# infancy/ky

Hardware: AMD Instinct MI355X
Metric: Msamples/s (paths*spp) (higher is better)
Workload: dtype f32

## Files before the change

include/kyhip.h:

```cpp
#ifndef KYHIP_H
#define KYHIP_H

#ifndef __HIPCC_RTC__
#include <stddef.h>
#include <stdint.h>
#endif

#ifdef __cplusplus
extern "C" {
#endif

#define KYHIP_ABI_VERSION 4


typedef enum ky_shape_kind {
    KY_SHAPE_DISK      = 0,
    KY_SHAPE_TRIANGLE  = 1,
    KY_SHAPE_RECTANGLE = 2,
    KY_SHAPE_SPHERE    = 3
} ky_shape_kind;

typedef struct ky_shape {
    int32_t kind;
    float   p[4][3];
// ... 32 lines not shown
    float   position[3];
    float   direction[3];
    float   world_radius;
} ky_light;

typedef struct ky_surface {
    int32_t shape;
    int32_t material;
    int32_t area_light;
} ky_surface;

typedef struct ky_camera {
    float position[3];
    float front[3];
    float right[3];
    float up[3];
    float resolution[2];
} ky_camera;

typedef struct ky_scene {
    const ky_shape*    shapes;    int32_t shape_count;
    const ky_material* materials; int32_t material_count;
    const ky_light*    lights;    int32_t light_count;
    const ky_surface*  surfaces;  int32_t surface_count;
    int32_t            environment_light;
    ky_camera          camera;
} ky_scene;

#define KYHIP_MAX_SHAPES    256
#define KYHIP_MAX_SURFACES  256
#define KYHIP_MAX_MATERIALS 64
#define KYHIP_MAX_LIGHTS    16


typedef enum ky_integrator_kind {
    KY_INTEGRATOR_POSITION               = 0,
    KY_INTEGRATOR_NORMAL                 = 1,
    KY_INTEGRATOR_BASECOLOR              = 2,
    KY_INTEGRATOR_DIRECT_LIGHTING        = 6,
    KY_INTEGRATOR_SIMPLE_PATH_TRACING_RECURSION   = 8,
    KY_INTEGRATOR_PATH_TRACING_RECURSION          = 9,
    KY_INTEGRATOR_PATH_TRACING_RECURSION_DEFERED  = 10,
    KY_INTEGRATOR_PATH_TRACING_ITERATION = 11
} ky_integrator_kind;

typedef enum ky_direct_sample {
    KY_DIRECT_IDLE      = 0,
    KY_DIRECT_BSDF      = 4,
    KY_DIRECT_LIGHT     = 8,
    KY_DIRECT_BSDF_MIS  = 16,
    KY_DIRECT_LIGHT_MIS = 32,
    KY_DIRECT_BOTH_MIS  = 48
} ky_direct_sample;

typedef enum ky_sampler_kind {
    KY_SAMPLER_DEBUG  = 0,
    KY_SAMPLER_RANDOM = 1
} ky_sampler_kind;

typedef struct ky_render_params {
    int32_t  integrator;
    int32_t  max_path_depth;
    int32_t  direct_sample;
    int32_t  samples_per_pixel;
    int32_t  sampler;
    uint32_t seed;
    int32_t  width, height;
    int32_t  tile_w, tile_h;
    int32_t  tile_first, tile_step;
} ky_render_params;

typedef enum ky_status {
    KY_OK                = 0,
    KY_ERR_INVALID_VALUE = -1,
    KY_ERR_LIMIT         = -2,
    KY_ERR_DEVICE        = -3,
    KY_ERR_NO_DEVICE     = -4
} ky_status;

const char* kyhip_last_error(void);
int         kyhip_set_engine(int engine);
int         kyhip_set_specialisation(int on);
int         kyhip_set_boxes(int on);
int         kyhip_set_shadow_queue(int mode);
int         kyhip_set_jit(int mode);
const char* kyhip_jit_status(void);
int         kyhip_jit_failures(void);
int64_t     kyhip_jit_compile(const char* name_expression);
uint64_t    kyhip_kernel_source_hash(void);
int         kyhip_abi_version(void);
int         kyhip_device_count(void);

int64_t kyhip_shard_tile_count(const ky_render_params* params);
int64_t kyhip_shard_float_count(const ky_render_params* params);
int64_t kyhip_film_term_limit(const ky_render_params* params, int n_lights, int engine, int deferred, float* limit);

int kyhip_render(int device, const ky_scene* scene, const ky_render_params* params,
                 float* film_rgb, size_t film_row_stride_px);

size_t kyhip_workspace_bytes(const ky_render_params* params);
int kyhip_render_tiles_device(int device, const ky_scene* scene, const ky_render_params* params,
                              float* d_tiles, void* d_workspace, size_t workspace_bytes, void* stream);
int kyhip_film_add_tiles_device(int device, const ky_render_params* params, const float* d_tiles,
                                float* d_film_rgb, size_t film_row_stride_px, void* stream);
int kyhip_film_add_gathered_device(int device, const ky_render_params* params, int world, const float* d_gathered,
                                   size_t rank_stride_floats, float* d_film_rgb, size_t film_row_stride_px, void* stream);

void*       kyhip_film_alloc(size_t bytes);
void        kyhip_film_free(void* film);
const char* kyhip_multi_status(int root_device);
int kyhip_seam_threads(void);
int kyhip_render_multi(const int* devices, int n_devices, const ky_scene* scene, const ky_render_params* params,
                       float* film_rgb, size_t film_row_stride_px);

float kyhip_kernel_ms(int device);
const char* kyhip_last_kernel(int device);


int kyhip_kat_intersect(int device, const ky_shape* shape, const float* rays7, int n, float* out8);

int kyhip_kat_camera(int device, const ky_camera* camera, const float* p_film2, int n, float* out6);

int kyhip_kat_bsdf(int device, const ky_material* material, const float* in12, int n, float* out13);

int kyhip_kat_light(int device, const ky_scene* scene, int light, const float* in11, int n, float* out11);

int kyhip_kat_scene_intersect(int device, const ky_scene* scene, const float* rays7, int n, float* out9);
int kyhip_kat_occluded(int device, const ky_scene* scene, const float* in9, int n, float* out1);
int kyhip_kat_any_pair(int device, const ky_scene* scene, const float* in13, int n, float* out2);
int kyhip_kat_occluded_between(int device, const ky_scene* scene, int light, const float* in9, int n, float* out1);
int kyhip_scene_non_occluders(const ky_scene* scene, int light, int* left_out, int n);
int kyhip_scene_boxes(const ky_scene* scene, int* box_face, int n);
int kyhip_scene_facts(const ky_scene* scene);

int kyhip_kat_li(int device, const ky_scene* scene, const ky_render_params* params,
                 int x, int y, int s0, int n, float* out3);

int kyhip_kat_nee(int device, const ky_scene* scene, int direct_sample, int light, const float* in15, int n, float* out6);

int kyhip_kat_li_trace(int device, const ky_scene* scene, const ky_render_params* params, int x, int y, int s,
                       float* rows26, int max_rows, float* li3);

enum ky_smallpt_refl { KY_SP_DIFF = 0, KY_SP_SPEC = 1, KY_SP_REFR = 2 };

typedef struct ky_smallpt_sphere {
    double rad;
    double p[3], e[3], c[3];
    int refl;
    int pad_;
} ky_smallpt_sphere;

enum ky_smallpt_variant { KY_SP_VARIANT_SMALLPT = 0, KY_SP_VARIANT_REWRITE = 1 };

typedef struct ky_smallpt_params {
    int width, height;
    int samps;
    uint32_t seed;
    int max_depth;
    int variant;
} ky_smallpt_params;

int kyhip_smallpt_scene(ky_smallpt_sphere* out);
int kyhip_smallpt_scene_rewrite(ky_smallpt_sphere* out);

int kyhip_smallpt_render(int device, const ky_smallpt_sphere* spheres, int n_spheres, const ky_smallpt_params* params,
                         double* image_rgb);

int kyhip_smallpt_kat_radiance(int device, const ky_smallpt_sphere* spheres, int n_spheres, const ky_smallpt_params* params,
                               int x, int y, int sx, int sy, int s0, int n, double* out3);

#ifdef __cplusplus
}
#endif
#endif
```

ky_amd/_abi.py:

```python
import ctypes as C
import os

_HERE = os.path.dirname(os.path.abspath(__file__))
LIB_DIR = os.path.join(_HERE, "lib")
REPO_ROOT = os.path.dirname(_HERE)

SHAPE_DISK, SHAPE_TRIANGLE, SHAPE_RECTANGLE, SHAPE_SPHERE = 0, 1, 2, 3
MATERIAL_MATTE, MATERIAL_MIRROR, MATERIAL_GLASS, MATERIAL_PLASTIC = 0, 1, 2, 3
LIGHT_POINT, LIGHT_DIRECTION, LIGHT_AREA, LIGHT_ENVIRONMENT = 0, 1, 2, 3
INTEGRATOR_POSITION, INTEGRATOR_NORMAL, INTEGRATOR_BASECOLOR = 0, 1, 2
INTEGRATOR_DIRECT_LIGHTING, INTEGRATOR_PATH_TRACING_ITERATION = 6, 11
INTEGRATOR_SIMPLE_PATH_TRACING_RECURSION, INTEGRATOR_PATH_TRACING_RECURSION, INTEGRATOR_PATH_TRACING_RECURSION_DEFERED = 8, 9, 10
DIRECT_IDLE, DIRECT_BSDF, DIRECT_LIGHT, DIRECT_BSDF_MIS, DIRECT_LIGHT_MIS, DIRECT_BOTH_MIS = 0, 4, 8, 16, 32, 48
SAMPLER_DEBUG, SAMPLER_RANDOM = 0, 1
SP_VARIANT_SMALLPT, SP_VARIANT_REWRITE = 0, 1
KY_OK, KY_ERR_INVALID_VALUE, KY_ERR_LIMIT, KY_ERR_DEVICE, KY_ERR_NO_DEVICE = 0, -1, -2, -3, -4
MAX_SHAPES, MAX_SURFACES, MAX_MATERIALS, MAX_LIGHTS = 256, 256, 64, 16

CB_LIGHT_AREA, CB_LIGHT_DIRECTION, CB_LIGHT_POINT, CB_LIGHT_ENVIRONMENT = 1, 2, 4, 8
CB_LARGE_MIRROR, CB_LARGE_GLASS, CB_SMALL_MIRROR, CB_SMALL_GLASS = 16, 32, 64, 128
CB_BOTH_SMALL_SPHERES = CB_SMALL_MIRROR | CB_SMALL_GLASS
CB_DEFAULT_SCENE = CB_BOTH_SMALL_SPHERES | CB_LIGHT_AREA

f3 = C.c_float * 3


class Shape(C.Structure):
    _fields_ = [("kind", C.c_int32), ("p", (C.c_float * 3) * 4), ("normal", f3), ("radius", C.c_float)]


class Material(C.Structure):
    _fields_ = [("kind", C.c_int32), ("color0", f3), ("color1", f3), ("eta", C.c_float), ("exponent", C.c_float),
                ("diffuse_probability", C.c_float), ("specular_probability", C.c_float)]


class Light(C.Structure):
    _fields_ = [("kind", C.c_int32), ("shape", C.c_int32), ("color", f3), ("position", f3), ("direction", f3),
                ("world_radius", C.c_float)]


class Surface(C.Structure):
    _fields_ = [("shape", C.c_int32), ("material", C.c_int32), ("area_light", C.c_int32)]


class Camera(C.Structure):
    _fields_ = [("position", f3), ("front", f3), ("right", f3), ("up", f3), ("resolution", C.c_float * 2)]


class Scene(C.Structure):
    _fields_ = [("shapes", C.POINTER(Shape)), ("shape_count", C.c_int32),
                ("materials", C.POINTER(Material)), ("material_count", C.c_int32),
                ("lights", C.POINTER(Light)), ("light_count", C.c_int32),
                ("surfaces", C.POINTER(Surface)), ("surface_count", C.c_int32),
                ("environment_light", C.c_int32), ("camera", Camera)]


class RenderParams(C.Structure):
    _fields_ = [("integrator", C.c_int32), ("max_path_depth", C.c_int32), ("direct_sample", C.c_int32),
                ("samples_per_pixel", C.c_int32), ("sampler", C.c_int32), ("seed", C.c_uint32),
                ("width", C.c_int32), ("height", C.c_int32), ("tile_w", C.c_int32), ("tile_h", C.c_int32),
                ("tile_first", C.c_int32), ("tile_step", C.c_int32)]


FP = C.POINTER(C.c_float)
SP = C.POINTER(Scene)
PP = C.POINTER(RenderParams)

class SmallptSphere(C.Structure):
    _fields_ = [("rad", C.c_double), ("p", C.c_double * 3), ("e", C.c_double * 3), ("c", C.c_double * 3), ("refl", C.c_int), ("pad_", C.c_int)]


class SmallptParams(C.Structure):
    _fields_ = [("width", C.c_int), ("height", C.c_int), ("samps", C.c_int), ("seed", C.c_uint32), ("max_depth", C.c_int),
                ("variant", C.c_int)]


SP_DIFF, SP_SPEC, SP_REFR = 0, 1, 2
SSP = C.POINTER(SmallptSphere)
SPP = C.POINTER(SmallptParams)

KYHIP_SYMBOLS = {
    "kyhip_last_error": (C.c_char_p, []),
    "kyhip_set_engine": (C.c_int, [C.c_int]),
    "kyhip_set_specialisation": (C.c_int, [C.c_int]),
    "kyhip_set_boxes": (C.c_int, [C.c_int]),
    "kyhip_set_shadow_queue": (C.c_int, [C.c_int]),
    "kyhip_set_jit": (C.c_int, [C.c_int]),
    "kyhip_jit_status": (C.c_char_p, []),
    "kyhip_jit_failures": (C.c_int, []),
    "kyhip_multi_status": (C.c_char_p, [C.c_int]),
    "kyhip_film_alloc": (C.c_void_p, [C.c_size_t]),
    "kyhip_film_free": (None, [C.c_void_p]),
    "kyhip_seam_threads": (C.c_int, []),
    "kyhip_jit_compile": (C.c_int64, [C.c_char_p]),
    "kyhip_kernel_source_hash": (C.c_uint64, []),
    "kyhip_abi_version": (C.c_int, []),
    "kyhip_device_count": (C.c_int, []),
    "kyhip_shard_tile_count": (C.c_int64, [PP]),
    "kyhip_shard_float_count": (C.c_int64, [PP]),
    "kyhip_film_term_limit": (C.c_int64, [PP, C.c_int, C.c_int, C.c_int, C.POINTER(C.c_float)]),
    "kyhip_render": (C.c_int, [C.c_int, SP, PP, C.c_void_p, C.c_size_t]),
    "kyhip_workspace_bytes": (C.c_size_t, [PP]),
    "kyhip_render_tiles_device": (C.c_int, [C.c_int, SP, PP, C.c_void_p, C.c_void_p, C.c_size_t, C.c_void_p]),
    "kyhip_film_add_tiles_device": (C.c_int, [C.c_int, PP, C.c_void_p, C.c_void_p, C.c_size_t, C.c_void_p]),
    "kyhip_film_add_gathered_device": (C.c_int, [C.c_int, PP, C.c_int, C.c_void_p, C.c_size_t, C.c_void_p, C.c_size_t, C.c_void_p]),
    "kyhip_render_multi": (C.c_int, [C.POINTER(C.c_int), C.c_int, SP, PP, C.c_void_p, C.c_size_t]),
    "kyhip_kernel_ms": (C.c_float, [C.c_int]),
    "kyhip_last_kernel": (C.c_char_p, [C.c_int]),
    "kyhip_kat_nee": (C.c_int, [C.c_int, SP, C.c_int, C.c_int, C.c_void_p, C.c_int, C.c_void_p]),
    "kyhip_kat_li_trace": (C.c_int, [C.c_int, SP, PP, C.c_int, C.c_int, C.c_int, C.c_void_p, C.c_int, C.c_void_p]),
    "kyhip_smallpt_scene": (C.c_int, [SSP]),
    "kyhip_smallpt_scene_rewrite": (C.c_int, [SSP]),
    "kyhip_smallpt_render": (C.c_int, [C.c_int, SSP, C.c_int, SPP, C.c_void_p]),
    "kyhip_smallpt_kat_radiance": (C.c_int, [C.c_int, SSP, C.c_int, SPP, C.c_int, C.c_int, C.c_int, C.c_int, C.c_int, C.c_int, C.c_void_p]),
    "kyhip_kat_intersect": (C.c_int, [C.c_int, C.POINTER(Shape), C.c_void_p, C.c_int, C.c_void_p]),
    "kyhip_kat_camera": (C.c_int, [C.c_int, C.POINTER(Camera), C.c_void_p, C.c_int, C.c_void_p]),
    "kyhip_kat_bsdf": (C.c_int, [C.c_int, C.POINTER(Material), C.c_void_p, C.c_int, C.c_void_p]),
    "kyhip_kat_light": (C.c_int, [C.c_int, SP, C.c_int, C.c_void_p, C.c_int, C.c_void_p]),
    "kyhip_kat_scene_intersect": (C.c_int, [C.c_int, SP, C.c_void_p, C.c_int, C.c_void_p]),
    "kyhip_kat_occluded": (C.c_int, [C.c_int, SP, C.c_void_p, C.c_int, C.c_void_p]),
    "kyhip_kat_any_pair": (C.c_int, [C.c_int, SP, C.c_void_p, C.c_int, C.c_void_p]),
    "kyhip_kat_occluded_between": (C.c_int, [C.c_int, SP, C.c_int, C.c_void_p, C.c_int, C.c_void_p]),
    "kyhip_scene_non_occluders": (C.c_int, [SP, C.c_int, C.c_void_p, C.c_int]),
    "kyhip_scene_boxes": (C.c_int, [SP, C.c_void_p, C.c_int]),
    "kyhip_scene_facts": (C.c_int, [SP]),
    "kyhip_kat_li": (C.c_int, [C.c_int, SP, PP, C.c_int, C.c_int, C.c_int, C.c_int, C.c_void_p]),
}

KYHOST_SYMBOLS = {
    "kyhost_last_error": (C.c_char_p, []),
    "kyhost_scene_create_cornell_box": (C.c_void_p, [C.c_int, C.c_float, C.c_float]),
    "kyhost_scene_create_mis": (C.c_void_p, [C.c_float, C.c_float]),
    "kyhost_scene_destroy": (None, [C.c_void_p]),
    "kyhost_scene_flatten": (SP, [C.c_void_p]),
    "kyhost_render": (C.c_int, [C.c_void_p, C.c_int, C.c_int, C.c_int, C.c_int, C.c_int, C.c_uint, C.c_int, C.c_int,
                                C.c_int, C.c_int, C.c_int, C.c_void_p, C.c_int]),
    "kyhost_debug_area": (C.c_int, [C.c_void_p, C.c_int, C.c_int, C.c_int, C.c_int, C.c_int, C.c_uint, C.c_int, C.c_int,
                                    C.c_void_p, C.c_int, C.c_int, C.c_int, C.c_int, C.c_int]),
    "kyhost_store_image": (C.c_int, [C.c_char_p, C.c_int, C.c_int, C.c_int, C.c_void_p]),
    "kyhost_gamma_encoding": (C.c_int, [C.c_float]),
}


SANITIZE = os.environ.get("KY_SANITIZE")
SAN_DIR = os.path.join(REPO_ROOT, "build", "san")

KYHOSTCHECK_SYMBOLS = {
    "kyhostcheck_pack": (C.c_int, [SP, C.POINTER(C.c_int), C.POINTER(C.c_uint64), C.POINTER(C.c_uint64), C.POINTER(C.c_int), C.POINTER(C.c_int)]),
    "kyhostcheck_chunks": (C.c_int, [C.c_int]),
    "kyhostcheck_shard": (C.c_longlong, [PP]),
    "kyhostcheck_add_rows": (C.c_int, [C.c_int, C.c_int, C.c_int, C.c_int, C.c_int]),
    "kyhostcheck_seam_stress": (C.c_int, [C.c_int]),
    "kyhostcheck_jit_stress": (C.c_int, [C.c_int, C.c_int]),
}


def _bind(lib, table, partial=False):
    for name, (res, args) in table.items():
        try:
            fn = getattr(lib, name)
        except AttributeError:
            if partial:
                continue
            raise
        fn.restype = res
        fn.argtypes = args
    return lib


_kyhip = None
_kyhost = None
_hiprt = None


def load_hip_runtime():
    global _hiprt
    if _hiprt is not None:
        return _hiprt
    candidates = []
    if os.environ.get("KYHIP_HIP_RUNTIME"):
        candidates.append(os.environ["KYHIP_HIP_RUNTIME"])
    else:
        try:
            import torch
            candidates.append(os.path.join(os.path.dirname(torch.__file__), "lib", "libamdhip64.so"))
        except Exception:
            pass
        candidates += ["/opt/rocm/lib/libamdhip64.so", "libamdhip64.so"]
    err = None
    for path in candidates:
        if os.path.isabs(path) and not os.path.exists(path):
            continue
        try:
            _hiprt = C.CDLL(path, mode=C.RTLD_GLOBAL)
            return _hiprt
        except OSError as e:
            err = e
    raise ImportError(f"no HIP runtime (libamdhip64.so) could be loaded: {err}")


def load_kyhip():
    global _kyhip
    if _kyhip is None and SANITIZE:
        path = os.path.join(SAN_DIR, "libkyhip_host_%s.so" % SANITIZE)
        if not os.path.exists(path):
            raise ImportError(f"{path} is missing: `make sanitize-build`")
        _kyhip = _bind(_bind(C.CDLL(path, mode=C.RTLD_GLOBAL), KYHIP_SYMBOLS, partial=True), KYHOSTCHECK_SYMBOLS)
    if _kyhip is None:
# ... 19 lines not shown
```

ky_amd/api.py:

```python
import ctypes as C

import numpy as np

from . import _abi as A


class KyError(RuntimeError):
    pass


def _check(rc, lib=None):
    if rc != A.KY_OK:
        lib = lib or A.load_kyhip()
        raise KyError(f"kyhip error {rc}: {lib.kyhip_last_error().decode()}")


def _fptr(a):
    assert a.dtype == np.float32 and a.flags["C_CONTIGUOUS"]
    return a.ctypes.data_as(C.c_void_p)


class SceneHandle:

    def __init__(self, ptr):
# ... 111 lines not shown

def kernel_ms(device=0):
    return float(A.load_kyhip().kyhip_kernel_ms(device))



def kat_intersect(shape, rays7, device=0):
    lib = A.load_kyhip()
    rays7 = np.ascontiguousarray(rays7, np.float32)
    out = np.zeros((rays7.shape[0], 8), np.float32)
    _check(lib.kyhip_kat_intersect(device, C.byref(shape), _fptr(rays7), rays7.shape[0], _fptr(out)))
    return out


def kat_camera(camera, p_film2, device=0):
    lib = A.load_kyhip()
    p_film2 = np.ascontiguousarray(p_film2, np.float32)
    out = np.zeros((p_film2.shape[0], 6), np.float32)
    _check(lib.kyhip_kat_camera(device, C.byref(camera), _fptr(p_film2), p_film2.shape[0], _fptr(out)))
    return out


def kat_bsdf(material, in12, device=0):
    lib = A.load_kyhip()
    in12 = np.ascontiguousarray(in12, np.float32)
    out = np.zeros((in12.shape[0], 13), np.float32)
    _check(lib.kyhip_kat_bsdf(device, C.byref(material), _fptr(in12), in12.shape[0], _fptr(out)))
    return out


def kat_light(scene, light, in11, device=0):
    lib = A.load_kyhip()
    in11 = np.ascontiguousarray(in11, np.float32)
    out = np.zeros((in11.shape[0], 11), np.float32)
    _check(lib.kyhip_kat_light(device, _scene_ptr(scene), light, _fptr(in11), in11.shape[0], _fptr(out)))
    return out


def kat_scene_intersect(scene, rays7, device=0):
    lib = A.load_kyhip()
    rays7 = np.ascontiguousarray(rays7, np.float32)
    out = np.zeros((rays7.shape[0], 9), np.float32)
    _check(lib.kyhip_kat_scene_intersect(device, _scene_ptr(scene), _fptr(rays7), rays7.shape[0], _fptr(out)))
    return out


def kat_any_pair(scene, in13, device=0):
    lib = A.load_kyhip()
    in13 = np.ascontiguousarray(in13, np.float32)
    out = np.zeros((in13.shape[0], 2), np.float32)
    _check(lib.kyhip_kat_any_pair(device, _scene_ptr(scene), _fptr(in13), in13.shape[0], _fptr(out)))
    return out


def kat_occluded(scene, in9, device=0, table=None):
    lib = A.load_kyhip()
    in9 = np.ascontiguousarray(in9, np.float32)
    out = np.zeros((in9.shape[0],), np.float32)
    if table is None:
        _check(lib.kyhip_kat_occluded(device, _scene_ptr(scene), _fptr(in9), in9.shape[0], _fptr(out)))
    else:
        _check(lib.kyhip_kat_occluded_between(device, _scene_ptr(scene), int(table), _fptr(in9), in9.shape[0], _fptr(out)))
    return out


def scene_non_occluders(scene, light=-1):
    lib = A.load_kyhip()
    n = _scene_ptr(scene).contents.surface_count
    out = np.zeros(max(1, n), np.int32)
    rc = lib.kyhip_scene_non_occluders(_scene_ptr(scene), int(light), out.ctypes.data_as(C.c_void_p), n)
    if rc < 0:
        _check(rc)
    return out[:n].copy()


def scene_facts(scene):
    lib = A.load_kyhip()
    rc = lib.kyhip_scene_facts(_scene_ptr(scene))
    if rc < 0:
        _check(rc)
    return rc


def scene_boxes(scene):
    lib = A.load_kyhip()
    n = _scene_ptr(scene).contents.surface_count
    out = np.zeros(max(1, n), np.int32)
    rc = lib.kyhip_scene_boxes(_scene_ptr(scene), out.ctypes.data_as(C.c_void_p), n)
    if rc < 0:
        _check(rc)
    return rc, out[:n].copy()


def kat_li(scene, params, x, y, s0, n, device=0):
    lib = A.load_kyhip()
    out = np.zeros((n, 3), np.float32)
    _check(lib.kyhip_kat_li(device, _scene_ptr(scene), C.byref(params), x, y, s0, n, _fptr(out)))
    return out


def kat_nee(scene, direct_sample, light, in15, device=0):
    lib = A.load_kyhip()
    in15 = np.ascontiguousarray(in15, np.float32)
    out = np.zeros((in15.shape[0], 6), np.float32)
    _check(lib.kyhip_kat_nee(device, _scene_ptr(scene), direct_sample, light, _fptr(in15), in15.shape[0], _fptr(out)))
    return out


def kat_li_trace(scene, params, x, y, s, max_rows=64, device=0):
    lib = A.load_kyhip()
    rows = np.zeros((max_rows, 26), np.float32)
    li = np.zeros(3, np.float32)
    n = lib.kyhip_kat_li_trace(device, _scene_ptr(scene), C.byref(params), x, y, s, _fptr(rows), max_rows, _fptr(li))
    if n < 0:
        _check(n, lib)
    return rows[:n], li



def smallpt_scene():
    spheres = (A.SmallptSphere * 9)()
    n = A.load_kyhip().kyhip_smallpt_scene(spheres)
    assert n == 9
    return spheres


def smallpt_scene_rewrite():
    spheres = (A.SmallptSphere * 9)()
    n = A.load_kyhip().kyhip_smallpt_scene_rewrite(spheres)
    assert n == 9
    return spheres


def smallpt_params(width, height, samps, seed=1234, max_depth=10, variant=A.SP_VARIANT_SMALLPT):
    return A.SmallptParams(width, height, samps, seed, max_depth, variant)


def smallpt_render(spheres, params, device=0):
    lib = A.load_kyhip()
    img = np.zeros((params.height, params.width, 3), np.float64)
    _check(lib.kyhip_smallpt_render(device, spheres, len(spheres), C.byref(params), img.ctypes.data_as(C.c_void_p)), lib)
    return img


def smallpt_kat_radiance(spheres, params, x, y, sx, sy, s0, n, device=0):
    lib = A.load_kyhip()
    out = np.zeros((n, 3), np.float64)
    _check(lib.kyhip_smallpt_kat_radiance(device, spheres, len(spheres), C.byref(params), x, y, sx, sy, s0, n,
                                          out.ctypes.data_as(C.c_void_p)), lib)
    return out


def store_image(filename, rgb, kind="bmp"):
    host = A.load_kyhost()
    rgb = np.ascontiguousarray(rgb, np.float32)
    k = {"ppm": 0, "bmp": 1, "hdr": 2}[kind]
    if host.kyhost_store_image(filename.encode(), k, rgb.shape[1], rgb.shape[0], _fptr(rgb)) != 0:
        raise KyError("store_image failed: " + host.kyhost_last_error().decode())
```

ky_amd/csrc/ky_device.hpp:

```cpp
#pragma once
#ifndef __HIPCC_RTC__
#include <hip/hip_runtime.h>
#include <stdint.h>
#endif

#include "ky_scene.hpp"

#define KY_DEV __device__ __forceinline__

#if defined(KY_PROFILE_LANES) || defined(KY_PROFILE_CLOCKS) || defined(KY_MARKS)
#include "ky_measure.hpp"
#else
#define KY_PROBE(k) do { } while (0)
#define KY_CLK(k) do { } while (0)
#endif

namespace kyd {

KY_DEV float rcp(float x) { return __builtin_amdgcn_rcpf(x); }
KY_DEV float rsq(float x) { return __builtin_amdgcn_rsqf(x); }
KY_DEV float fsqrt(float x) { return __builtin_amdgcn_sqrtf(x); }
KY_DEV float sin_rev(float x) { return __builtin_amdgcn_sinf(x); }
KY_DEV float cos_rev(float x) { return __builtin_amdgcn_cosf(x); }
KY_DEV float clamp01f(float x) { return __builtin_amdgcn_fmed3f(x, 0.f, 1.f); }
KY_DEV float any_f() { float x; asm volatile("" : "=v"(x)); return x; }
KY_DEV float any_reg() { return any_f(); }
KY_DEV unsigned any_reg_u() { unsigned x; asm volatile("" : "=v"(x)); return x; }
KY_DEV float mul_legacy(float a, float b) { float r; asm("s_nop 0\n\tv_mul_legacy_f32_e64 %0, %1, %2" : "=v"(r) : "v"(a), "v"(b)); return r; }
KY_DEV float pow_nonneg(float x, float n) {
    return __builtin_amdgcn_exp2f(mul_legacy(n, __builtin_amdgcn_logf(x)));
}

struct f3 {
    float x, y, z;
};
KY_DEV f3 mk3(float x, float y, float z) { return f3{x, y, z}; }
KY_DEV f3 any3() { return f3{any_f(), any_f(), any_f()}; }
KY_DEV f3 operator+(f3 a, f3 b) { return {a.x + b.x, a.y + b.y, a.z + b.z}; }
KY_DEV f3 operator-(f3 a, f3 b) { return {a.x - b.x, a.y - b.y, a.z - b.z}; }
KY_DEV f3 operator-(f3 a) { return {-a.x, -a.y, -a.z}; }
KY_DEV f3 operator*(f3 a, float s) { return {a.x * s, a.y * s, a.z * s}; }
KY_DEV f3 operator*(float s, f3 a) { return {a.x * s, a.y * s, a.z * s}; }
KY_DEV f3 operator*(f3 a, f3 b) { return {a.x * b.x, a.y * b.y, a.z * b.z}; }
KY_DEV float dot(f3 a, f3 b) { return a.x * b.x + a.y * b.y + a.z * b.z; }
KY_DEV f3 cross(f3 a, f3 b) { return {a.y * b.z - a.z * b.y, a.z * b.x - a.x * b.z, a.x * b.y - a.y * b.x}; }
KY_DEV float length_sq(f3 a) { return dot(a, a); }
KY_DEV f3 normalize(f3 a) { return a * rsq(dot(a, a)); }
KY_DEV float max3(f3 a) { return fmaxf(a.x, fmaxf(a.y, a.z)); }
KY_DEV bool is_black(f3 c) { return (c.x <= 0) && (c.y <= 0) && (c.z <= 0); }
KY_DEV bool is_black_bits(const float* c) {
    const int* b = (const int*)c;
    return (b[0] <= 0) & (b[1] <= 0) & (b[2] <= 0);
}

KY_DEV unsigned long long fixed_from_float(float a) {
    const float aa = fabsf(a);
    const float hi = __builtin_floorf(aa);
    const float lo = __builtin_rintf((aa - hi) * 4294967296.0f);
    const unsigned long long v = ((unsigned long long)(unsigned)hi << 32) | (unsigned long long)(unsigned)lo;
    return a < 0 ? 0ull - v : v;
}
KY_DEV float film_limit(const unsigned* counter) {
    return __uint_as_float(__hip_atomic_load(counter + 1, __ATOMIC_RELAXED, __HIP_MEMORY_SCOPE_AGENT));
}
KY_DEV float film_limit_for(const float* c, const unsigned* counter) {
    float limit = 1.f;
    if (!(fminf(fminf(c[0], c[1]), c[2]) >= 0.f && c[0] + c[1] + c[2] < 1.f)) limit = film_limit(counter);
    return limit;
}
KY_DEV unsigned long long film_fixed(float a, float limit, int ch, unsigned& flags) {
    const bool nan = a != a, pos = a >= limit, neg = a <= -limit;
    flags |= (nan ? 1u << ch : 0u) | (pos ? 8u << ch : 0u) | (neg ? 64u << ch : 0u);
    const float b = (nan | pos | neg) ? 0.f : a;
    return fixed_from_float(b);
}

constexpr float K_PI = 3.14159265358979323846f;
constexpr float K_INV_PI = 0.318309886183790671538f;
constexpr float K_INV_2PI = K_INV_PI / 2.f;
constexpr float K_SHAPE_EPS = 1e-3f;
constexpr float K_RAY_OFFSET = 1e-2f;
constexpr float K_INF = __builtin_huge_valf();

struct SceneRef {
    const DScene* p;
    bool general;
    int feat;
    bool large;
    __device__ __forceinline__ SceneRef(const DScene* p_) : p(p_), general(true), feat(0), large(true) {}
    __device__ __forceinline__ SceneRef(const DScene* p_, bool general_, int feat_ = 0, bool large_ = false) : p(p_), general(general_), feat(feat_), large(large_) {}
    __device__ __forceinline__ const DScene* operator->() const { return p; }
    __device__ __forceinline__ bool single_area() const { return (feat & KY_FEAT_SINGLE_AREA) != 0; }
    __device__ __forceinline__ bool single_light() const { return (feat & KY_FEAT_SINGLE_LIGHT) != 0; }
    __device__ __forceinline__ bool is_area(int kind) const {
        return (feat & (KY_FEAT_SINGLE_AREA | KY_FEAT_SPHERE_LIGHTS)) ? true : ((feat & (KY_FEAT_SINGLE_DELTA | KY_FEAT_SINGLE_ENV)) ? false : kind == KY_LIGHT_AREA);
    }
    __device__ __forceinline__ bool is_delta(int kind) const {
        return (feat & KY_FEAT_SINGLE_DELTA) ? true : ((feat & (KY_FEAT_SINGLE_AREA | KY_FEAT_SINGLE_ENV | KY_FEAT_SPHERE_LIGHTS)) ? false : (kind == KY_LIGHT_POINT || kind == KY_LIGHT_DIRECTION));
    }
    __device__ __forceinline__ bool is_env(int kind) const {
        return (feat & KY_FEAT_SINGLE_ENV) ? true : ((feat & (KY_FEAT_SINGLE_AREA | KY_FEAT_SINGLE_DELTA | KY_FEAT_SPHERE_LIGHTS)) ? false : kind == KY_LIGHT_ENVIRONMENT);
    }
    __device__ __forceinline__ bool may_have_env() const { return (feat & (KY_FEAT_SINGLE_AREA | KY_FEAT_SINGLE_DELTA | KY_FEAT_SPHERE_LIGHTS)) == 0; }
    __device__ __forceinline__ bool no_carried_light() const { return (feat & (KY_FEAT_SINGLE_DELTA | KY_FEAT_SINGLE_ENV)) != 0; }
    __device__ __forceinline__ bool x_planks() const { return (feat & KY_FEAT_X_PLANKS) != 0; }
    __device__ __forceinline__ bool sphere_lights() const { return (feat & KY_FEAT_SPHERE_LIGHTS) != 0; }
    __device__ __forceinline__ bool boxes() const { return (feat & KY_FEAT_BOXES) != 0; }
    __device__ __forceinline__ bool flat_phong() const { return (feat & KY_FEAT_FLAT_PHONG) != 0; }
    __device__ __forceinline__ bool no_par() const { return (feat & KY_FEAT_AXIS_ALIGNED) != 0; }
    __device__ __forceinline__ bool ipdf() const { return (feat & KY_FEAT_SPHERE_LIGHTS) != 0; }
};

struct LdsScene {
    const DHit* hit;
    const DMat* mat;
    const float (*light_color)[4];
};
template <int NS, int NM>
struct LdsSceneStaticT {
    DHit hit[NS];
    DMat mat[NM];
    float light_color[KYHIP_MAX_LIGHTS][4];
};
using LdsSceneStatic = LdsSceneStaticT<KY_LDS_SURFACES, KY_LDS_MATERIALS>;
extern __shared__ __attribute__((aligned(16))) unsigned char g_lds_scene[];

KY_DEV f3 ld3(const float* p) { return {p[0], p[1], p[2]}; }

template <bool LARGE, bool SMALL = false>
KY_DEV LdsScene stage_scene(SceneRef S) {
    const int tid = threadIdx.x, nt = blockDim.x;
    const int ns = S->n_surfaces, nm = S->n_materials, nl = S->n_lights;
    uint32_t *dst_h, *dst_m;
    float* dst_l;
    if (LARGE) {
        dst_h = reinterpret_cast<uint32_t*>(g_lds_scene);
        dst_m = reinterpret_cast<uint32_t*>(g_lds_scene + lds_scene_mat_offset(ns));
        dst_l = reinterpret_cast<float*>(g_lds_scene + lds_scene_light_offset(ns, nm));
    } else {
        __shared__ LdsSceneStaticT<SMALL ? KY_LDS_SURFACES_SMALL : KY_LDS_SURFACES, SMALL ? KY_LDS_MATERIALS_SMALL : KY_LDS_MATERIALS> L;
        dst_h = reinterpret_cast<uint32_t*>(L.hit);
        dst_m = reinterpret_cast<uint32_t*>(L.mat);
        dst_l = &L.light_color[0][0];
    }
    const uint32_t* src_h = reinterpret_cast<const uint32_t*>(S->hit);
    for (int i = tid; i < ns * (int)(sizeof(DHit) / 4); i += nt) dst_h[i] = src_h[i];
    const uint32_t* src_m = reinterpret_cast<const uint32_t*>(S->mat);
    for (int i = tid; i < nm * (int)(sizeof(DMat) / 4); i += nt) dst_m[i] = src_m[i];
    for (int i = tid; i < nl; i += nt) {
        dst_l[4 * i + 0] = S->light[i].color[0];
        dst_l[4 * i + 1] = S->light[i].color[1];
        dst_l[4 * i + 2] = S->light[i].color[2];
        dst_l[4 * i + 3] = 0.f;
    }
    __syncthreads();
    return LdsScene{reinterpret_cast<const DHit*>(dst_h), reinterpret_cast<const DMat*>(dst_m), reinterpret_cast<const float (*)[4]>(dst_l)};
}

KY_DEV uint32_t mix32(uint32_t x) {
    x ^= x >> 16; x *= 0x21f0aaadu;
    x ^= x >> 15; x *= 0x735a2d97u;
    x ^= x >> 15;
    return x;
}
struct Sampler {
    uint32_t s0, s1;
};
KY_DEV uint32_t sampler_pixel_key(uint32_t seed, uint32_t pixel_index) { return mix32(pixel_index ^ mix32(seed)); }
KY_DEV void sampler_start(Sampler& s, uint32_t h, uint32_t sample_index) {
    s.s0 = mix32(h + sample_index * 0x9E3779B9u);
    s.s1 = (__builtin_amdgcn_alignbit(s.s0, s.s0, 16) ^ h) | 1u;
}
KY_DEV uint32_t rotl32(uint32_t x, int k) { return __builtin_amdgcn_alignbit(x, x, 32 - k); }
// ... 239 lines not shown
}

KY_DEV float vmin(float a, float b) { float r; asm("v_min_f32_e32 %0, %1, %2" : "=v"(r) : "v"(a), "v"(b)); return r; }
KY_DEV float vmax(float a, float b) { float r; asm("v_max_f32_e32 %0, %1, %2" : "=v"(r) : "v"(a), "v"(b)); return r; }
KY_DEV float vmin3(float a, float b, float c) { float r; asm("v_min3_f32 %0, %1, %2, %3" : "=v"(r) : "v"(a), "v"(b), "v"(c)); return r; }
KY_DEV float vmax3(float a, float b, float c) { float r; asm("v_max3_f32 %0, %1, %2, %3" : "=v"(r) : "v"(a), "v"(b), "v"(c)); return r; }
KY_DEV float face_tag(float t, float surface_bits) { return __uint_as_float((__float_as_uint(t) & ~15u) | __float_as_uint(surface_bits)); }
KY_DEV void box_candidate(unsigned long long ex, float t_enter, float t_leave, float t, float& tmax, int& best) {
    unsigned long long tmp;
    const unsigned surface = __float_as_uint(t) & 15u;
    asm volatile(
        "v_cmpx_le_f32_e64 %[tmp], %[te], %[tl]\n\t"
        "v_cmpx_lt_f32_e64 %[tmp], %[eps], %[t]\n\t"
        "v_cmpx_lt_f32_e64 %[tmp], %[t], %[tmax]\n\t"
        "v_cmpx_ne_u32_e64 %[tmp], %[none], %[s]\n\t"
        "v_mov_b32_e32 %[tmax], %[t]\n\t"
        "v_mov_b32_e32 %[best], %[s]\n\t"
        "s_mov_b64 exec, %[ex]"
        : [tmax] "+v"(tmax), [best] "+v"(best), [tmp] "=&s"(tmp)
        : [te] "v"(t_enter), [tl] "v"(t_leave), [t] "v"(t), [s] "v"(surface), [eps] "s"(K_SHAPE_EPS), [none] "n"(KY_BOX_NO_FACE), [ex] "s"(ex));
}
KY_DEV void box_update_nearest(unsigned long long ex, const float4 q0, const float4 q1, const float4 q2, f3 o, f3 inv_c, float& tmax, int& best) {
    const float xl = face_tag((q0.x - o.x) * inv_c.x, q0.w), xh = face_tag((q1.x - o.x) * inv_c.x, q1.w);
    const float yl = face_tag((q0.y - o.y) * inv_c.y, q2.x), yh = face_tag((q1.y - o.y) * inv_c.y, q2.y);
    const float zl = face_tag((q0.z - o.z) * inv_c.z, q2.z), zh = face_tag((q1.z - o.z) * inv_c.z, q2.w);
    const float t_enter = vmax3(vmin(xl, xh), vmin(yl, yh), vmin(zl, zh));
    const float t_leave = vmin3(vmax(xl, xh), vmax(yl, yh), vmax(zl, zh));
    box_candidate(ex, t_enter, t_leave, t_enter, tmax, best);
    box_candidate(ex, t_enter, t_leave, t_leave, tmax, best);
}

KY_DEV void box_candidate_any(unsigned long long ex, float t_enter, float t_leave, float t, float tmax, unsigned& occ) {
    unsigned long long tmp;
    const unsigned surface = __float_as_uint(t) & 15u;
    asm volatile(
        "v_cmpx_le_f32_e64 %[tmp], %[te], %[tl]\n\t"
        "v_cmpx_lt_f32_e64 %[tmp], %[eps], %[t]\n\t"
        "v_cmpx_lt_f32_e64 %[tmp], %[t], %[tmax]\n\t"
        "v_cmpx_ne_u32_e64 %[tmp], %[none], %[s]\n\t"
        "v_mov_b32_e32 %[occ], 1\n\t"
        "s_mov_b64 exec, %[ex]"
        : [occ] "+v"(occ), [tmp] "=&s"(tmp)
        : [te] "v"(t_enter), [tl] "v"(t_leave), [t] "v"(t), [tmax] "v"(tmax), [s] "v"(surface), [eps] "s"(K_SHAPE_EPS), [none] "n"(KY_BOX_NO_FACE), [ex] "s"(ex));
}
KY_DEV void box_update_any(unsigned long long ex, const float4 q0, const float4 q1, const float4 q2, f3 o, f3 inv_c, float tmax, unsigned& occ) {
    const float xl = face_tag((q0.x - o.x) * inv_c.x, q0.w), xh = face_tag((q1.x - o.x) * inv_c.x, q1.w);
    const float yl = face_tag((q0.y - o.y) * inv_c.y, q2.x), yh = face_tag((q1.y - o.y) * inv_c.y, q2.y);
    const float zl = face_tag((q0.z - o.z) * inv_c.z, q2.z), zh = face_tag((q1.z - o.z) * inv_c.z, q2.w);
    const float t_enter = vmax3(vmin(xl, xh), vmin(yl, yh), vmin(zl, zh));
    const float t_leave = vmin3(vmax(xl, xh), vmax(yl, yh), vmax(zl, zh));
    box_candidate_any(ex, t_enter, t_leave, t_enter, tmax, occ);
    box_candidate_any(ex, t_enter, t_leave, t_leave, tmax, occ);
}
KY_DEV void box_candidate_any_unbounded(unsigned long long ex, float t_enter, float t_leave, float t, unsigned& occ) {
    unsigned long long tmp;
    const unsigned surface = __float_as_uint(t) & 15u;
    asm volatile(
        "v_cmpx_le_f32_e64 %[tmp], %[te], %[tl]\n\t"
        "v_cmpx_lt_f32_e64 %[tmp], %[eps], %[t]\n\t"
        "v_cmpx_ne_u32_e64 %[tmp], %[none], %[s]\n\t"
        "v_mov_b32_e32 %[occ], 1\n\t"
        "s_mov_b64 exec, %[ex]"
        : [occ] "+v"(occ), [tmp] "=&s"(tmp)
        : [te] "v"(t_enter), [tl] "v"(t_leave), [t] "v"(t), [s] "v"(surface), [eps] "s"(K_SHAPE_EPS), [none] "n"(KY_BOX_NO_FACE), [ex] "s"(ex));
}
KY_DEV void box_update_any_unbounded(unsigned long long ex, const float4 q0, const float4 q1, const float4 q2, f3 o, f3 inv_c, unsigned& occ) {
    const float xl = face_tag((q0.x - o.x) * inv_c.x, q0.w), xh = face_tag((q1.x - o.x) * inv_c.x, q1.w);
    const float yl = face_tag((q0.y - o.y) * inv_c.y, q2.x), yh = face_tag((q1.y - o.y) * inv_c.y, q2.y);
    const float zl = face_tag((q0.z - o.z) * inv_c.z, q2.z), zh = face_tag((q1.z - o.z) * inv_c.z, q2.w);
    const float t_enter = vmax3(vmin(xl, xh), vmin(yl, yh), vmin(zl, zh));
    const float t_leave = vmin3(vmax(xl, xh), vmax(yl, yh), vmax(zl, zh));
    box_candidate_any_unbounded(ex, t_enter, t_leave, t_enter, occ);
    box_candidate_any_unbounded(ex, t_enter, t_leave, t_leave, occ);
}

KY_DEV bool surf_hit(const DSurf& S, const DShapeFull* __restrict__ full, f3 o, f3 d, float tmax, float& t_out, bool general = true, bool sphere_only = false, bool sparse = true) {
    if (sphere_only) return sph_hit(make_float4(S.f[0], S.f[1], S.f[2], S.f[3]), o, d, tmax, t_out, sparse);
    if (S.kind == TK_PARALLELOGRAM)
        return par_hit(make_float4(S.f[0], S.f[1], S.f[2], S.f[3]), make_float4(S.f[4], S.f[5], S.f[6], S.f[7]), make_float4(S.f[8], S.f[9], S.f[10], S.f[11]), o, d, tmax, t_out);
    if (!general || S.kind == TK_SPHERE) return sph_hit(make_float4(S.f[0], S.f[1], S.f[2], S.f[3]), o, d, tmax, t_out);
    return full_shape_hit(full[S.full], o, d, tmax, t_out);
}

KY_DEV int trace_nearest(SceneRef S, f3 o, f3 d, float& tmax) {
    int best = -1;
    const unsigned t_off = opaque_off((unsigned)__builtin_offsetof(DScene, trav));
    const int4 head = scene_at<int4>(S, t_off), axis = scene_at<int4>(S, t_off + 16u);
    const int n_aar = head.x, n_par = S.no_par() ? 0 : head.y, n_sph = S->n_sph, n_gen = S->n_gen;
    if (S.boxes()) {
        const unsigned b_off = opaque_off((unsigned)__builtin_offsetof(DScene, boxtrav));
        const int4 bhead = scene_at<int4>(S, b_off), baxis = scene_at<int4>(S, b_off + 16u);
        const f3 inv_d = mk3(rcp(d.x), rcp(d.y), rcp(d.z));
        const f3 inv_c = mk3(__builtin_amdgcn_fmed3f(inv_d.x, -1e30f, 1e30f), __builtin_amdgcn_fmed3f(inv_d.y, -1e30f, 1e30f), __builtin_amdgcn_fmed3f(inv_d.z, -1e30f, 1e30f));
        const unsigned long long ex = __builtin_amdgcn_ballot_w64(true);
        unsigned off = b_off + (unsigned)__builtin_offsetof(DBoxTrav, box);
        for (int k = 0; k < bhead.x; ++k) {
            asm volatile("" : "+s"(off));
            const DBox& B = scene_at<DBox>(S, off);
            box_update_nearest(ex, B.q0, B.q1, B.q2, o, inv_c, tmax, best);
            off += (unsigned)sizeof(DBox);
        }
        if (bhead.y > 0) {
            unsigned unused = 0;
            const int n0 = baxis.x, n1 = baxis.y, n2 = baxis.z;
            const unsigned aar_off = b_off + (unsigned)__builtin_offsetof(DBoxTrav, aar);
            aar_scan<0, true>(S, aar_off, 0, n0, o, d, inv_d, tmax, best, unused);
            aar_scan<1, true>(S, aar_off, n0, n1, o, d, inv_d, tmax, best, unused);
            aar_scan<2, true>(S, aar_off, n0 + n1, n2, o, d, inv_d, tmax, best, unused);
        }
    } else
    if (n_aar > 0) {
        const f3 inv_d = mk3(rcp(d.x), rcp(d.y), rcp(d.z));
        unsigned unused = 0;
        const int n0 = axis.x, n1 = axis.y, n2 = axis.z;
        const unsigned aar_off = t_off + (unsigned)__builtin_offsetof(DTrav, aar);
        aar_scan<0, true>(S, aar_off, 0, n0, o, d, inv_d, tmax, best, unused);
        aar_scan<1, true>(S, aar_off, n0, n1, o, d, inv_d, tmax, best, unused);
        aar_scan<2, true>(S, aar_off, n0 + n1, n2, o, d, inv_d, tmax, best, unused);
    }
    if (n_par > 0) {
        unsigned off = t_off + (unsigned)__builtin_offsetof(DTrav, par);
        const unsigned long long ex = __builtin_amdgcn_ballot_w64(true);
        for (int i = 0; i < n_par; ++i) {
            asm volatile("" : "+s"(off));
            const DPar& r = scene_at<DPar>(S, off);
            float t, u, v;
            par_coords(r.q0, r.q1, r.q2, o, d, t, u, v);
            hit_update_nearest(ex, u, 0.5f, v, 0.5f, t, tmax, best, n_aar + i);
            off += (unsigned)sizeof(DPar);
        }
    }
    if (n_sph > 0) {
        unsigned off = scene_off(S, &S->sph[0]);
        const unsigned long long ex = __builtin_amdgcn_ballot_w64(true);
        for (int i = 0; i < n_sph; ++i) {
            asm volatile("" : "+s"(off));
            const float4 c = scene_at<DSph>(S, off).c;
            const f3 oc = mk3(c.x, c.y, c.z) - o;
            const float neg_b = dot(oc, d);
            const float discr = neg_b * neg_b - dot(oc, oc) + c.w;
            if (!S.sphere_lights() || __any(discr >= 0.f)) sph_update_nearest(ex, neg_b, discr, tmax, best, n_aar + n_par + i);
            off += (unsigned)sizeof(DSph);
        }
    }
    for (int i = 0; S.general && i < n_gen; ++i) {
        float t;
        if (full_shape_hit(S->full[S->gen[i].full], o, d, tmax, t)) {
            tmax = t;
            best = n_aar + n_par + n_sph + i;
        }
    }
    return best;
}

KY_DEV bool trace_any_planar(SceneRef S, const DTrav& T, f3 o, f3 d, float tmax) {
    unsigned occ = 0;
    const unsigned t_off = opaque_off(scene_off(S, &T));
    const int4 head = scene_at<int4>(S, t_off), axis = scene_at<int4>(S, t_off + 16u);
    const int n_aar = head.x, n_par = S.no_par() ? 0 : head.y;
    if (n_aar > 0) {
        const f3 inv_d = mk3(rcp(d.x), rcp(d.y), rcp(d.z));
        int unused = -1;
        const int n0 = axis.x, n1 = axis.y, n2 = axis.z;
        const unsigned aar_off = t_off + (unsigned)__builtin_offsetof(DTrav, aar);
        aar_scan<0, false>(S, aar_off, 0, n0, o, d, inv_d, tmax, unused, occ);
        aar_scan<1, false>(S, aar_off, n0, n1, o, d, inv_d, tmax, unused, occ);
        aar_scan<2, false>(S, aar_off, n0 + n1, n2, o, d, inv_d, tmax, unused, occ);
    }
    if (n_par > 0) {
        unsigned off = t_off + (unsigned)__builtin_offsetof(DTrav, par);
        const unsigned long long ex = __builtin_amdgcn_ballot_w64(true);
        for (int i = 0; i < n_par; ++i) {
            asm volatile("" : "+s"(off));
            const DPar& r = scene_at<DPar>(S, off);
            float t, u, v;
            par_coords(r.q0, r.q1, r.q2, o, d, t, u, v, S.x_planks());
            hit_update_any(ex, u, 0.5f, v, 0.5f, t, tmax, occ);
            off += (unsigned)sizeof(DPar);
        }
    }
    return occ != 0;
}
KY_DEV bool trace_any_round(SceneRef S, bool occ, f3 o, f3 d, float tmax) {
    const int n_sph = S->n_sph, n_gen = S->n_gen;
    float t;
    if (n_sph > 0) {
        unsigned off = scene_off(S, &S->sph[0]);
        const unsigned long long ex = __builtin_amdgcn_ballot_w64(true);
        unsigned occ_v = 0;
        for (int i = 0; i < n_sph; ++i) {
            asm volatile("" : "+s"(off));
            const float4 c = scene_at<DSph>(S, off).c;
            const f3 oc = mk3(c.x, c.y, c.z) - o;
            const float neg_b = dot(oc, d);
            const float discr = neg_b * neg_b - dot(oc, oc) + c.w;
            const float e = neg_b - tmax;
            if (!S.sphere_lights() || __any((discr >= 0.f) & ((e < 0.f) | (e * e < discr)))) sph_update_any(ex, neg_b, discr, tmax, occ_v);
            off += (unsigned)sizeof(DSph);
        }
        occ = occ | (occ_v != 0);
    }
    for (int i = 0; S.general && i < n_gen; ++i) occ = occ || full_shape_hit(S->full[S->gen[i].full], o, d, tmax, t);
    return occ;
}
KY_DEV bool trace_any(SceneRef S, const DTrav& T, f3 o, f3 d, float tmax) {
    return trace_any_round(S, trace_any_planar(S, T, o, d, tmax), o, d, tmax);
}
struct AnyRay {
    f3 o, d;
    float tmax;
};
template <int AXIS>
KY_DEV void aar_scan_any_pair(SceneRef S, unsigned long long ex, unsigned aar_off, int first, int n, const AnyRay& A, f3 iA, unsigned& occA, const AnyRay& B, f3 iB, unsigned& occB) {
    if (n <= 0) return;
    unsigned off = aar_off + (unsigned)first * (unsigned)sizeof(DAar);
    const float oaA = AXIS == 0 ? A.o.x : (AXIS == 1 ? A.o.y : A.o.z), iaA = AXIS == 0 ? iA.x : (AXIS == 1 ? iA.y : iA.z);
    const float ouA = AXIS == 0 ? A.o.y : (AXIS == 1 ? A.o.z : A.o.x), duA = AXIS == 0 ? A.d.y : (AXIS == 1 ? A.d.z : A.d.x);
    const float ovA = AXIS == 0 ? A.o.z : (AXIS == 1 ? A.o.x : A.o.y), dvA = AXIS == 0 ? A.d.z : (AXIS == 1 ? A.d.x : A.d.y);
    const float oaB = AXIS == 0 ? B.o.x : (AXIS == 1 ? B.o.y : B.o.z), iaB = AXIS == 0 ? iB.x : (AXIS == 1 ? iB.y : iB.z);
    const float ouB = AXIS == 0 ? B.o.y : (AXIS == 1 ? B.o.z : B.o.x), duB = AXIS == 0 ? B.d.y : (AXIS == 1 ? B.d.z : B.d.x);
    const float ovB = AXIS == 0 ? B.o.z : (AXIS == 1 ? B.o.x : B.o.y), dvB = AXIS == 0 ? B.d.z : (AXIS == 1 ? B.d.x : B.d.y);
    for (int i = 0; i < n; ++i) {
        asm volatile("" : "+s"(off));
        const DAar& r = scene_at<DAar>(S, off);
        const float4 q0 = r.q0;
        const float rv = r.q1.x;
        const float tA = (q0.x - oaA) * iaA, tB = (q0.x - oaB) * iaB;
        const float uA = (ouA + tA * duA) - q0.y, uB = (ouB + tB * duB) - q0.y;
        const float vA = (ovA + tA * dvA) - q0.w, vB = (ovB + tB * dvB) - q0.w;
        hit_update_any_unbounded(ex, uA, q0.z, vA, rv, tA, occA);
        hit_update_any(ex, uB, q0.z, vB, rv, tB, B.tmax, occB);
        off += (unsigned)sizeof(DAar);
    }
}
KY_DEV void trace_any_pair(SceneRef S, const AnyRay& A, const AnyRay& B, bool& occ_a, bool& occ_b) {
    unsigned occA = 0, occB = 0;
    const f3 iA = mk3(__builtin_amdgcn_fmed3f(rcp(A.d.x), -1e30f, 1e30f), __builtin_amdgcn_fmed3f(rcp(A.d.y), -1e30f, 1e30f), __builtin_amdgcn_fmed3f(rcp(A.d.z), -1e30f, 1e30f));
    const f3 iB = mk3(__builtin_amdgcn_fmed3f(rcp(B.d.x), -1e30f, 1e30f), __builtin_amdgcn_fmed3f(rcp(B.d.y), -1e30f, 1e30f), __builtin_amdgcn_fmed3f(rcp(B.d.z), -1e30f, 1e30f));
    const unsigned long long ex = __builtin_amdgcn_ballot_w64(true);
    const unsigned t_off = opaque_off((unsigned)__builtin_offsetof(DScene, trav));
    if (S.boxes()) {
        const unsigned b_off = opaque_off((unsigned)__builtin_offsetof(DScene, boxtrav));
        const int4 bhead = scene_at<int4>(S, b_off), baxis = scene_at<int4>(S, b_off + 16u);
        unsigned off = b_off + (unsigned)__builtin_offsetof(DBoxTrav, box);
        for (int k = 0; k < bhead.x; ++k) {
            asm volatile("" : "+s"(off));
            const DBox& Bx = scene_at<DBox>(S, off);
            const float4 q0 = Bx.q0, q1 = Bx.q1, q2 = Bx.q2;
            box_update_any_unbounded(ex, q0, q1, q2, A.o, iA, occA);
            box_update_any(ex, q0, q1, q2, B.o, iB, B.tmax, occB);
            off += (unsigned)sizeof(DBox);
        }
        if (bhead.y > 0) {
            const unsigned aar_off = b_off + (unsigned)__builtin_offsetof(DBoxTrav, aar);
            aar_scan_any_pair<0>(S, ex, aar_off, 0, baxis.x, A, iA, occA, B, iB, occB);
            aar_scan_any_pair<1>(S, ex, aar_off, baxis.x, baxis.y, A, iA, occA, B, iB, occB);
            aar_scan_any_pair<2>(S, ex, aar_off, baxis.x + baxis.y, baxis.z, A, iA, occA, B, iB, occB);
        }
    } else {
        const int4 head = scene_at<int4>(S, t_off), axis = scene_at<int4>(S, t_off + 16u);
        if (head.x > 0) {
            const unsigned aar_off = t_off + (unsigned)__builtin_offsetof(DTrav, aar);
            aar_scan_any_pair<0>(S, ex, aar_off, 0, axis.x, A, iA, occA, B, iB, occB);
            aar_scan_any_pair<1>(S, ex, aar_off, axis.x, axis.y, A, iA, occA, B, iB, occB);
            aar_scan_any_pair<2>(S, ex, aar_off, axis.x + axis.y, axis.z, A, iA, occA, B, iB, occB);
        }
    }
    const int n_par = S.no_par() ? 0 : S->trav.n_par;
    if (n_par > 0) {
        unsigned off = t_off + (unsigned)__builtin_offsetof(DTrav, par);
        for (int i = 0; i < n_par; ++i) {
            asm volatile("" : "+s"(off));
            const DPar& r = scene_at<DPar>(S, off);
            float t, u, v;
            par_coords(r.q0, r.q1, r.q2, A.o, A.d, t, u, v, S.x_planks());
            hit_update_any_unbounded(ex, u, 0.5f, v, 0.5f, t, occA);
            par_coords(r.q0, r.q1, r.q2, B.o, B.d, t, u, v, S.x_planks());
            hit_update_any(ex, u, 0.5f, v, 0.5f, t, B.tmax, occB);
            off += (unsigned)sizeof(DPar);
        }
    }
    const int n_sph = S->n_sph, n_gen = S->n_gen;
    if (n_sph > 0) {
        unsigned off = scene_off(S, &S->sph[0]);
        for (int i = 0; i < n_sph; ++i) {
            asm volatile("" : "+s"(off));
            const float4 c = scene_at<DSph>(S, off).c;
            const f3 ocA = mk3(c.x, c.y, c.z) - A.o, ocB = mk3(c.x, c.y, c.z) - B.o;
            const float nbA = dot(ocA, A.d), nbB = dot(ocB, B.d);
            sph_update_any_unbounded(ex, nbA, nbA * nbA - dot(ocA, ocA) + c.w, occA);
            sph_update_any(ex, nbB, nbB * nbB - dot(ocB, ocB) + c.w, B.tmax, occB);
            off += (unsigned)sizeof(DSph);
        }
    }
    occ_a = occA != 0;
    occ_b = occB != 0;
    float t;
    for (int i = 0; S.general && i < n_gen; ++i) {
        occ_a = occ_a || full_shape_hit(S->full[S->gen[i].full], A.o, A.d, A.tmax, t);
        occ_b = occ_b || full_shape_hit(S->full[S->gen[i].full], B.o, B.d, B.tmax, t);
    }
}

KY_DEV f3 hit_normal(const DHit& H, f3 position, f3 d) {
    const f3 n = ld3(H.n);
    if (H.kind == KY_SHAPE_SPHERE) return normalize(position - n);
    if (H.kind == KY_SHAPE_RECTANGLE) {
        const unsigned flip = dot(n, d) <= 0 ? 0u : 0x80000000u;
        return mk3(__uint_as_float(__float_as_uint(n.x) ^ flip), __uint_as_float(__float_as_uint(n.y) ^ flip), __uint_as_float(__float_as_uint(n.z) ^ flip));
    }
    return n;
}

struct Frame {
    f3 s, t, n;
};
KY_DEV Frame make_frame(f3 n) {
    Frame f;
// ... 676 lines not shown
    const float c[3] = {r.c.x, r.c.y, r.c.z};
    const int pix = (int)(r.tag >> 6), owner = (int)((threadIdx.x & ~63u) | (r.tag & 63u));
    const bool local = q.c_pix[owner] == pix;
    unsigned fl = 0;
    const float limit = film_limit_for(c, q.counter);
#pragma unroll
    for (int ch = 0; ch < 3; ++ch) {
        const unsigned long long fx = film_fixed(c[ch], limit, ch, fl);
        if (fx != 0) {
            if (local) atomicAdd(&q.c_def[ch * 256 + owner], fx);
            else atomicAdd(&q.accum[(size_t)pix * 3 + ch], fx);
        }
    }
    if (fl) atomicOr(&q.flags[pix], fl);
}
KY_DEV void sq_push(SceneRef S, ShadowQueue& q, bool push, SqRay r) {
    const unsigned long long m = __ballot(push);
    if (!m) return;
    const int k = __popcll(m);
    const int rank = (int)__builtin_amdgcn_mbcnt_hi((unsigned)(m >> 32), __builtin_amdgcn_mbcnt_lo((unsigned)m, 0u));
    if (q.n + k < KY_SQ_FLUSH_AT) {
        if (push) sq_store(KY_SQ_SLOT(q, q.n + rank), r);
        q.n += k;
        return;
    }
    asm volatile("" ::: "memory");
    const unsigned long long idle = ~m;
    const int idx = (int)__builtin_amdgcn_mbcnt_hi((unsigned)(idle >> 32), __builtin_amdgcn_mbcnt_lo((unsigned)idle, 0u));
    const bool pop = !push && idx < q.n;
    if (pop) r = sq_load(KY_SQ_SLOT(q, q.n - 1 - idx));
    q.n -= min(q.n, 64 - k);
    if (KY_SQ_FLUSH_AT == 64 || push || pop) sq_trace(S, q, r);
}
KY_DEV void sq_push_bsdf_query(SceneRef S, ShadowQueue& q, bool push, f3 o, f3 d, float tmax, f3 c, unsigned tag) {
    sq_push(S, q, push, SqRay{o, d, c, tmax, tag});
}
KY_DEV void sq_drain(SceneRef S, ShadowQueue& q) {
    const int lane = (int)__lane_id();
    __builtin_amdgcn_fence(__ATOMIC_ACQ_REL, "wavefront");
    if (lane < q.n) sq_trace(S, q, sq_load(KY_SQ_SLOT(q, lane)));
    q.n = 0;
}

template <bool MIS>
KY_DEV void estimate_by_emitter_deferred(SceneRef S, const Vertex& v, f3 wo, int li, float u0, float u1, bool active, f3 beta, float weight,
                                         unsigned tag, ShadowQueue& q) {
    const DLight& L = scene_light(S, li);
    bool push = false;
    SqRay r{any3(), any3(), any3(), any_f(), tag};
    if (active) {
        const bool ip = S.ipdf();
        const LightSample ls = light_sample_Li(L, v.position, v.normal, u0, u1, S.feat, ip);
        if (S.is_area(L.kind)) {
            r.d = ls.dir;
            r.tmax = ls.dist - 2e-3f;
        } else {
            const f3 to = ls.position - v.position;
            const float d2 = length_sq(to);
            const float inv_d = rsq(d2);
            r.d = to * inv_d;
            r.tmax = d2 * inv_d - 2e-3f;
        }
        r.o = offset_ray_origin(v.position, v.normal, r.d);
        f3 col;
        float scale, bsdf_pdf, abs_cos_i;
        bsdf_eval_parts(v, wo, S.is_area(L.kind) ? r.d : ls.wi, col, scale, bsdf_pdf, abs_cos_i);
        const bool delta_light = S.is_delta(L.kind);
        const float fc = scale * abs_cos_i;
        const float k = fc * (ip ? ((!MIS || delta_light) ? ls.pdf : (2.f * ls.pdf) * rcp(1.f + bsdf_pdf * ls.pdf))
                                 : ((!MIS || delta_light) ? rcp(ls.pdf) : 2.f * rcp(ls.pdf + bsdf_pdf))) * weight;
        const bool area = S.is_area(L.kind);
        const f3 Li = area ? ld3(L.color) : ls.Li;
        r.c = ((col * Li) * beta) * k;
        push = (area ? ls.lit : !is_black(ls.Li)) && (ip || !(MIS ? ls.pdf <= 0 : ls.pdf == 0)) && !(fc <= 0.f) && !is_black(col);
        if (S.is_area(L.kind) && L.sampled_is_surface) {
            float t;
            if (surf_hit(L.isect, S->full, r.o, r.d, r.tmax, t, S.general, S.sphere_lights(), false)) push = false;
        }
    }
    sq_push(S, q, push, r);
}

KY_DEV bool light_sample_occluded(SceneRef S, int li, f3 o, f3 dir, float tmax) {
    const unsigned tab = (unsigned)scene_light(S, li).shadow_table;
    const bool two = (tab & 1u) != 0;
    bool occ = trace_any(S, scene_at<DTrav>(S, tab & ~1u), o, dir, tmax);
    if (two) {
        const float4 plane = scene_at<float4>(S, opaque_off((unsigned)__builtin_offsetof(DScene, ts_plane)));
        const f3 pn = mk3(plane.x, plane.y, plane.z);
        const f3 e = o + dir * tmax;
        const bool need = !occ && (fminf(dot(pn, e), dot(pn, o)) <= plane.w);
        if (__any(need)) {
            if (need) occ = trace_any_planar(S, S->occ_behind, o, dir, tmax);
        }
    }
    return occ;
}

template <bool MIS>
KY_DEV void estimate_by_emitter(SceneRef S, const LdsScene& Lds, const Vertex& v, f3 wo, int li, float u0, float u1, f3& acc, f3 w) {
    const DLight& L = scene_light(S, li);
    KY_PROBE(3);
    const bool ip = S.ipdf();
    const LightSample ls = light_sample_Li(L, v.position, v.normal, u0, u1, S.feat, ip);
    const bool area = S.is_area(L.kind);
    const bool dead = (area ? !ls.lit : is_black(ls.Li)) || (!(ip || area) && (MIS ? (ls.pdf <= 0) : (ls.pdf == 0)));
    KY_CLK(5);
    if (!dead) {
        f3 dir;
        float dist;
        if (area) {
            dir = ls.dir;
            dist = ls.dist;
        } else {
            const f3 to = ls.position - v.position;
            const float d2 = length_sq(to);
            const float inv_d = rsq(d2);
            dir = to * inv_d;
            dist = d2 * inv_d;
        }
        const f3 o = offset_ray_origin(v.position, v.normal, dir);
        KY_PROBE(4);
        const bool occ = light_sample_occluded(S, li, o, dir, dist - 2e-3f);
        KY_CLK(6);
        if (!occ) {
            KY_PROBE(5);
            f3 col;
            float scale, bsdf_pdf, abs_cos_i;
            bsdf_eval_parts(v, wo, area ? dir : ls.wi, col, scale, bsdf_pdf, abs_cos_i);
            const float fc = scale * abs_cos_i;
            if (!(fc <= 0.f) && !is_black(col)) {
                const bool delta_light = S.is_delta(L.kind);
                const float k = fc * (ip ? ((!MIS || delta_light) ? ls.pdf : (2.f * ls.pdf) * rcp(1.f + bsdf_pdf * ls.pdf))
                                         : ((!MIS || delta_light) ? rcp(ls.pdf) : 2.f * rcp(ls.pdf + bsdf_pdf)));
                acc = acc + ((col * (area ? ld3(L.color) : ls.Li)) * w) * k;
            }
            KY_CLK(7);
        }
    }
}

template <bool MIS>
KY_DEV void estimate_by_emitter_ride(SceneRef S, const LdsScene& Lds, const Vertex& v, f3 wo, int li, float u0, float u1, bool active, RideAlong& ra, f3& acc, f3 w) {
    const DLight& L = scene_light(S, li);
    LightSample ls{any3(), any3(), any3(), any_f(), false, any3(), any_f()};
    const bool area = S.is_area(L.kind);
    bool dead = true;
    if (active) {
        ls = light_sample_Li(L, v.position, v.normal, u0, u1, S.feat);
        dead = (area ? !ls.lit : is_black(ls.Li)) || (MIS ? (ls.pdf <= 0) : (ls.pdf == 0));
    }
    f3 o = any3(), dir = any3();
    float tmax = any_f();
    if (!dead) {
        if (area) {
            dir = ls.dir;
            tmax = ls.dist - 2e-3f;
        } else {
            const f3 to = ls.position - v.position;
            const float d2 = length_sq(to);
            const float inv_d = rsq(d2);
            dir = to * inv_d;
            tmax = d2 * inv_d - 2e-3f;
        }
        o = offset_ray_origin(v.position, v.normal, dir);
    }
// ... 332 lines not shown
```

ky_amd/csrc/ky_host.hpp:

```cpp
#pragma once
#include <cstddef>
#include <cstdint>
#include <condition_variable>
#include <functional>
#include <mutex>
#include <string>
#include <utility>
#include <vector>
#include <sys/types.h>

#include "ky_shard.hpp"

namespace kyh {
using namespace kyd;

int fail(int code, const char* fmt, ...) __attribute__((format(printf, 2, 3)));
const std::string& last_error();

bool valid_params(const ky_render_params* p);
bool shard_in_range(const ky_render_params* p);
ShardConst make_shard(const ky_render_params* p);
RenderConst make_rc(const ky_render_params* p);
long long film_term_count(const ky_render_params* p, int n_lights, bool queue_engine, bool deferred);
float film_term_limit(long long n_terms);
bool film_in_range(const ky_render_params* p, int n_lights);
int film_range_check(const ky_render_params* p, const ky_scene* scene);
inline size_t workspace_bytes_for(const ShardConst& s) { return (size_t)s.n_pix * (3 * sizeof(unsigned long long) + sizeof(unsigned)); }

void cp3(float* d, const float* s);
void pack_shape(const ky_shape& sh, int full_index, DSurf* surf, DShapeFull* full);
void pack_material(const ky_material& m, DMat* d);
bool shape_normal_ok(const ky_shape& sh);
struct NonOccluders {
    std::vector<char> wall;
    std::vector<char> light_ok;
    bool deferred_ok = false;
    int ts_light = -1;
    double ts_plane[4] = {0, 0, 0, 0};
    std::vector<char> ts_behind;
};
void find_non_occluders(const ky_scene* in, NonOccluders& R);
struct Boxes {
    struct Box { float lo[3], hi[3]; int face[6]; };
    std::vector<Box> box;
    std::vector<int> box_of;
};
void find_boxes(const ky_scene* in, Boxes& B);
int pack_scene(const ky_scene* in, DScene* out);
uint64_t scene_hash(const DScene& s);
bool scene_input(const ky_scene* in, std::vector<unsigned char>& out, uint64_t& hash);

constexpr int KY_SP_MAX_SPHERES = 32;
int smallpt_check(const ky_smallpt_sphere* spheres, int n, const ky_smallpt_params* p);

bool specialisation_enabled();
bool boxes_enabled();
int shadow_queue_mode();
bool shadow_queue_wanted(const ky_scene* scene);
int blocks_per_cu_cap();
enum { KY_ENGINE_LANE = 0, KY_ENGINE_QUEUE = 1 };
int current_engine();

int cpus_granted();
int seam_threads();
void host_add_rows(float* __restrict__ film, size_t stride_px, const float* __restrict__ src, int width, int y0, int y1);
class HostPool {
public:
    void run(int n, const std::function<void(int)>& fn);
private:
    void loop(int id);
    std::mutex job_m_, m_;
    std::condition_variable cv_, done_;
    const std::function<void(int)>* fn_ = nullptr;
    int n_ = 0, pending_ = 0, n_threads_ = 0;
    pid_t pid_ = 0;
    unsigned long long generation_ = 0;
};
HostPool& host_pool();
std::vector<std::unique_lock<std::mutex>> lock_seams(std::vector<std::pair<int, std::mutex*>> by_device);
}

namespace kyjit {
struct Code {
    std::vector<char> object;
    bool failed = false;
};
extern const char k_entry[];
int mode();
const Code* get_code(const std::string& args, bool wait = true, bool* pending = nullptr);
uint64_t source_hash();
int set_mode(int m);
bool mode_by_default();
std::string status();
int failures();
void frame_begin();
void frame_end();
}
```

ky_amd/csrc/ky_launch.hip:

```cpp
#include <hip/hip_runtime.h>

#include <algorithm>
#include <cstdio>
#include <cstring>

#include "ky_ctx.hpp"
#include "ky_render.hpp"
#include "ky_smallpt.hpp"

using namespace kyh;
static_assert(kyh::KY_SP_MAX_SPHERES == kysp::SP_MAX_SPHERES, "smallpt_check (ky_pack.cpp) and the kernels' LDS table");

#include "ky_queue.hpp"

__global__ void resolve_kernel(unsigned long long* __restrict__ accum, unsigned* __restrict__ flags, float* __restrict__ tiles, int n_pix, unsigned* __restrict__ counter) {
    const int i = blockIdx.x * blockDim.x + threadIdx.x;
    if (i == 0) *counter = 0u;
    if (i >= n_pix) return;
    const unsigned fl = flags[i];
    flags[i] = 0u;
#pragma unroll
    for (int ch = 0; ch < 3; ++ch) {
        float v = (float)((double)(long long)accum[3 * (size_t)i + ch] * (1.0 / KY_FIX_SCALE));
        accum[3 * (size_t)i + ch] = 0ull;
// ... 113 lines not shown
            if (sl.valid && sl.input_hash == input_hash && sl.input == input) pick = &sl;
    uint64_t hash = 0;
    if (!pick) {
        const int rc = pack_scene(scene, &scratch);
        if (rc != KY_OK) return rc;
        hash = scene_hash(scratch);
        for (SceneSlot& sl : c->scenes)
            if (sl.valid && sl.hash == hash && std::memcmp(&scratch, sl.h, sizeof(DScene)) == 0) pick = &sl;
        if (pick && keyed) { pick->input = input; pick->input_hash = input_hash; }
    }
    if (pick) {
        if (pick->upload_stream != stream) HIP_TRY(hipStreamWaitEvent(stream, pick->ready, 0));
    } else {
        for (SceneSlot& sl : c->scenes)
            if (!sl.valid && !pick) pick = &sl;
        if (!pick) {
            pick = &c->scenes[0];
            for (SceneSlot& sl : c->scenes)
                if (sl.last_use < pick->last_use) pick = &sl;
            for (int i = 0; i < KY_STREAM_STATES; ++i)
                if ((pick->readers >> i & 1u) && c->ss[i].done) HIP_TRY(hipEventSynchronize(c->ss[i].done));
            HIP_TRY(hipEventSynchronize(pick->ready));
            pick->valid = false;
        }
        if (!pick->d) {
            HIP_TRY(hipMalloc(&pick->d, sizeof(DScene)));
            HIP_TRY(hipHostMalloc(&pick->h, sizeof(DScene)));
            HIP_TRY(hipEventCreateWithFlags(&pick->ready, hipEventDisableTiming));
        }
        std::memcpy(pick->h, &scratch, sizeof(DScene));
        HIP_TRY(hipMemcpyAsync(pick->d, pick->h, sizeof(DScene), hipMemcpyHostToDevice, stream));
        HIP_TRY(hipEventRecord(pick->ready, stream));
        pick->upload_stream = stream;
        pick->hash = hash;
        if (keyed) { pick->input = input; pick->input_hash = input_hash; } else { pick->input.clear(); pick->input_hash = 0; }
        pick->readers = 0;
        pick->valid = true;
    }
    pick->last_use = ++c->clock;
    *out = pick;
    return KY_OK;
}
}

extern "C" {

#ifdef KY_PROFILE_LANES
int kyhip_debug_lane_probe(unsigned long long* out32) {
    unsigned long long zero[32] = {0};
    if (hipMemcpyFromSymbol(out32, HIP_SYMBOL(g_lane_probe), sizeof zero) != hipSuccess) return KY_ERR_DEVICE;
    if (hipMemcpyToSymbol(HIP_SYMBOL(g_lane_probe), zero, sizeof zero) != hipSuccess) return KY_ERR_DEVICE;
    return KY_OK;
}
#endif
#ifdef KY_PROFILE_CLOCKS
int kyhip_debug_clocks(unsigned long long* out16, int reset) {
    if (hipMemcpyFromSymbol(out16, HIP_SYMBOL(g_clk), 16 * sizeof(unsigned long long)) != hipSuccess) return -1;
    if (reset) { unsigned long long z[16] = {}; if (hipMemcpyToSymbol(HIP_SYMBOL(g_clk), z, sizeof(z)) != hipSuccess) return -1; }
    return 0;
}
#endif
#ifdef KY_QE_STATS
int kyhip_debug_stats(unsigned long long* out32, int reset) {
    if (hipMemcpyFromSymbol(out32, HIP_SYMBOL(kyd::g_qe_stats), 32 * sizeof(unsigned long long)) != hipSuccess) return -1;
    if (reset) { unsigned long long z[32] = {}; if (hipMemcpyToSymbol(HIP_SYMBOL(kyd::g_qe_stats), z, sizeof(z)) != hipSuccess) return -1; }
    return 0;
}
#endif

int kyhip_device_count(void) {
    int n = 0;
    if (hipGetDeviceCount(&n) != hipSuccess) return 0;
    return n;
}

using RenderFn = void (*)(const DScene*, RenderConst, ShardConst, unsigned*, unsigned long long*, unsigned*, float4*);
struct Variant {
    bool dbg;
    int strategy;
    bool queue, general;
    int feat, integrator;
    bool large;
    RenderFn fn;
};
#define KY_VARIANT(D, S, Q, G, F, I) Variant{D, S, Q, G, F, I, false, render_kernel<D, S, Q, G, F, I>}
#define KY_VARIANT_LARGE(D, S, Q, G, F, I) Variant{D, S, Q, G, F, I, true, render_kernel<D, S, Q, G, F, I, true>}
constexpr int IT = KY_INTEGRATOR_PATH_TRACING_ITERATION;
static const Variant g_variants[] = {
#ifdef KY_FEW_VARIANTS
    KY_VARIANT(false, KY_DIRECT_BOTH_MIS, false, false, KY_FEAT_CORNELL | KY_FEAT_SMALL_TABLES | KY_FEAT_BOXES | KY_FEAT_AXIS_ALIGNED | KY_FEAT_FLAT_PHONG, IT),
    KY_VARIANT(false, KY_DIRECT_BOTH_MIS, false, false, KY_FEAT_CORNELL | KY_FEAT_SMALL_TABLES | KY_FEAT_BOXES, IT),
    KY_VARIANT(false, KY_DIRECT_BOTH_MIS, false, false, KY_FEAT_CORNELL | KY_FEAT_SMALL_TABLES, IT),
#ifndef KY_NO_XPLANK_ROW
    KY_VARIANT(false, KY_DIRECT_BOTH_MIS, true, false, KY_FEAT_VEACH | KY_FEAT_FLAT_PHONG | KY_FEAT_X_PLANKS, IT),
#endif
    KY_VARIANT(false, KY_DIRECT_BOTH_MIS, true, false, KY_FEAT_VEACH | KY_FEAT_FLAT_PHONG, IT),
    KY_VARIANT(false, KY_DIRECT_BOTH_MIS, false, false, KY_FEAT_SINGLE_ENV | KY_FEAT_SMALL_TABLES | KY_FEAT_BOXES | KY_FEAT_AXIS_ALIGNED | KY_FEAT_FLAT_PHONG, IT),
    KY_VARIANT(false, KY_DIRECT_BOTH_MIS, false, false, KY_FEAT_SINGLE_ENV | KY_FEAT_SMALL_TABLES | KY_FEAT_AXIS_ALIGNED | KY_FEAT_FLAT_PHONG, IT),
    KY_VARIANT(false, KY_DIRECT_BOTH_MIS, false, false, KY_FEAT_SINGLE_ENV, IT),
    KY_VARIANT(false, -1, false, false, 0, IT),
#else
    KY_VARIANT(false, KY_DIRECT_BOTH_MIS, false, false, KY_FEAT_CORNELL | KY_FEAT_SMALL_TABLES | KY_FEAT_BOXES | KY_FEAT_AXIS_ALIGNED | KY_FEAT_FLAT_PHONG, IT),
    KY_VARIANT(false, KY_DIRECT_BOTH_MIS, false, false, KY_FEAT_CORNELL | KY_FEAT_SMALL_TABLES | KY_FEAT_BOXES, IT),
    KY_VARIANT(false, KY_DIRECT_BOTH_MIS, false, false, KY_FEAT_CORNELL | KY_FEAT_SMALL_TABLES | KY_FEAT_AXIS_ALIGNED, IT),
    KY_VARIANT(false, KY_DIRECT_BOTH_MIS, false, false, KY_FEAT_CORNELL | KY_FEAT_SMALL_TABLES, IT),
    KY_VARIANT(false, KY_DIRECT_BOTH_MIS, false, false, KY_FEAT_CORNELL, IT),
    KY_VARIANT(false, KY_DIRECT_BOTH_MIS, false, false, KY_FEAT_SINGLE_DELTA | KY_FEAT_BOXES | KY_FEAT_AXIS_ALIGNED | KY_FEAT_FLAT_PHONG, IT),
    KY_VARIANT(false, KY_DIRECT_BOTH_MIS, false, false, KY_FEAT_SINGLE_DELTA, IT),
    KY_VARIANT(false, KY_DIRECT_BOTH_MIS, false, false, KY_FEAT_SINGLE_ENV | KY_FEAT_SMALL_TABLES | KY_FEAT_BOXES | KY_FEAT_AXIS_ALIGNED | KY_FEAT_FLAT_PHONG, IT),
    KY_VARIANT(false, KY_DIRECT_BOTH_MIS, false, false, KY_FEAT_SINGLE_ENV | KY_FEAT_SMALL_TABLES | KY_FEAT_AXIS_ALIGNED | KY_FEAT_FLAT_PHONG, IT),
    KY_VARIANT(false, KY_DIRECT_BOTH_MIS, false, false, KY_FEAT_SINGLE_ENV, IT),
    KY_VARIANT(false, KY_DIRECT_BOTH_MIS, true, false, KY_FEAT_VEACH | KY_FEAT_FLAT_PHONG | KY_FEAT_X_PLANKS, IT),
    KY_VARIANT(false, KY_DIRECT_BOTH_MIS, true, false, KY_FEAT_VEACH | KY_FEAT_FLAT_PHONG, IT),
    KY_VARIANT(false, KY_DIRECT_BOTH_MIS, true, false, KY_FEAT_VEACH, IT),
    KY_VARIANT(false, KY_DIRECT_BOTH_MIS, true, false, 0, IT),
    KY_VARIANT(false, KY_DIRECT_BOTH_MIS, false, false, 0, IT),
    KY_VARIANT(false, KY_DIRECT_BSDF, false, false, KY_FEAT_VEACH, IT),
    KY_VARIANT(false, KY_DIRECT_LIGHT, true, false, KY_FEAT_VEACH, IT),
    KY_VARIANT(false, KY_DIRECT_LIGHT, false, false, KY_FEAT_VEACH, IT),
    KY_VARIANT(false, KY_DIRECT_BSDF_MIS, false, false, KY_FEAT_VEACH, IT),
    KY_VARIANT(false, KY_DIRECT_LIGHT_MIS, true, false, KY_FEAT_VEACH, IT),
    KY_VARIANT(false, KY_DIRECT_LIGHT_MIS, false, false, KY_FEAT_VEACH, IT),
    KY_VARIANT(false, KY_DIRECT_BSDF, false, false, KY_FEAT_CORNELL, IT),
    KY_VARIANT(false, KY_DIRECT_BSDF_MIS, false, false, KY_FEAT_CORNELL, IT),
    KY_VARIANT(false, KY_DIRECT_IDLE, false, false, 0, IT),
    KY_VARIANT(false, KY_DIRECT_BSDF, false, false, 0, IT),
    KY_VARIANT(false, KY_DIRECT_LIGHT, true, false, 0, IT),
    KY_VARIANT(false, KY_DIRECT_LIGHT_MIS, true, false, 0, IT),
    KY_VARIANT(false, KY_DIRECT_LIGHT, false, false, 0, IT),
    KY_VARIANT(false, KY_DIRECT_BSDF_MIS, false, false, 0, IT),
    KY_VARIANT(false, KY_DIRECT_LIGHT_MIS, false, false, 0, IT),
    KY_VARIANT(false, KY_DIRECT_BOTH_MIS, false, false, KY_FEAT_CORNELL, KY_INTEGRATOR_PATH_TRACING_RECURSION),
    KY_VARIANT(false, KY_DIRECT_BOTH_MIS, false, false, KY_FEAT_SINGLE_ENV, KY_INTEGRATOR_PATH_TRACING_RECURSION),
    KY_VARIANT(false, KY_DIRECT_BOTH_MIS, false, false, KY_FEAT_CORNELL, KY_INTEGRATOR_PATH_TRACING_RECURSION_DEFERED),
    KY_VARIANT(false, KY_DIRECT_BOTH_MIS, false, false, KY_FEAT_SINGLE_ENV, KY_INTEGRATOR_PATH_TRACING_RECURSION_DEFERED),
    KY_VARIANT(false, KY_DIRECT_BOTH_MIS, false, false, KY_FEAT_SINGLE_DELTA, KY_INTEGRATOR_PATH_TRACING_RECURSION),
    KY_VARIANT(false, KY_DIRECT_BOTH_MIS, false, false, KY_FEAT_SINGLE_DELTA, KY_INTEGRATOR_PATH_TRACING_RECURSION_DEFERED),
    KY_VARIANT(false, KY_DIRECT_BOTH_MIS, false, false, KY_FEAT_CORNELL, KY_INTEGRATOR_DIRECT_LIGHTING),
    KY_VARIANT(false, KY_DIRECT_BOTH_MIS, false, false, KY_FEAT_SINGLE_DELTA, KY_INTEGRATOR_DIRECT_LIGHTING),
    KY_VARIANT(false, KY_DIRECT_BOTH_MIS, false, false, KY_FEAT_SINGLE_ENV, KY_INTEGRATOR_DIRECT_LIGHTING),
    KY_VARIANT(false, KY_DIRECT_BOTH_MIS, false, false, 0, KY_INTEGRATOR_DIRECT_LIGHTING),
    KY_VARIANT(false, KY_DIRECT_BOTH_MIS, false, false, 0, KY_INTEGRATOR_SIMPLE_PATH_TRACING_RECURSION),
    KY_VARIANT(false, KY_DIRECT_BOTH_MIS, false, false, 0, KY_INTEGRATOR_PATH_TRACING_RECURSION),
    KY_VARIANT(false, KY_DIRECT_BOTH_MIS, false, false, 0, KY_INTEGRATOR_PATH_TRACING_RECURSION_DEFERED),
    KY_VARIANT(false, KY_DIRECT_BOTH_MIS, false, true, 0, IT),
    KY_VARIANT(false, -1, false, false, 0, IT),
    KY_VARIANT(true, -1, false, false, 0, IT),
    KY_VARIANT(false, -1, false, true, 0, IT),
    KY_VARIANT(true, -1, false, true, 0, IT),
    KY_VARIANT_LARGE(false, -1, false, true, 0, IT),
    KY_VARIANT_LARGE(true, -1, false, true, 0, IT),
#endif
};
constexpr int KY_N_VARIANTS = (int)(sizeof g_variants / sizeof g_variants[0]);
static_assert(KY_N_VARIANTS <= 64, "DeviceCtx::variant_blocks");

static const Variant* pick_variant(const ky_render_params* p, const DScene* packed, bool deferred_rays, int n_pix) {
    const bool dbg = p->sampler == KY_SAMPLER_DEBUG;
    const bool general = packed->general != 0;
    const bool large = packed->n_surfaces > KY_LDS_SURFACES || packed->n_materials > KY_LDS_MATERIALS;
    for (const Variant& v : g_variants) {
        if (v.dbg != dbg || v.large != large) continue;
        if (general && !v.general) continue;
        if (v.strategy >= 0) {
            if (!specialisation_enabled() && !(v.strategy == KY_DIRECT_BOTH_MIS && v.feat == 0 && v.integrator == IT)) continue;
            if (v.strategy != p->direct_sample || v.integrator != p->integrator) continue;
        }
        if ((v.feat & packed->feat) != v.feat) continue;
        if (v.queue && !(n_pix < (1 << 26) && deferred_rays)) continue;
        return &v;
    }
    return nullptr;
}

}
static int set_film_limit(StreamState* st, long long n_terms, hipStream_t stream) {
    const float t = film_term_limit(n_terms);
    if (t == 0.f) return fail(KY_ERR_DEVICE, "internal: %lld film terms per pixel passed film_in_range", n_terms);
    uint32_t bits;
    std::memcpy(&bits, &t, sizeof bits);
    if (st->counter_limit_bits != bits) {
        HIP_TRY(hipMemsetD32Async((hipDeviceptr_t)(st->d_counter + 1), (int)bits, 1, stream));
        st->counter_limit_bits = bits;
    }
    return KY_OK;
}
int kyh::render_replay_feat(const ky_scene* scene, const ky_render_params* p, const DScene* packed) {
    const Variant* v = pick_variant(p, packed, shadow_queue_wanted(scene), p->width * p->height);
    return v != nullptr ? (v->feat & (KY_FEAT_BOXES | KY_FEAT_SINGLE_ENV)) : 0;
}
bool kyh::render_uses_boxes(const ky_scene* scene, const ky_render_params* p, const DScene* packed) { return (render_replay_feat(scene, p, packed) & KY_FEAT_BOXES) != 0; }
extern "C" {

int kyhip_render_tiles_device(int device, const ky_scene* scene, const ky_render_params* p, float* d_tiles, void* d_workspace,
                              size_t workspace_bytes, void* stream_) {
    if (!valid_params(p)) return fail(KY_ERR_INVALID_VALUE, "invalid render params (integrator %d, direct_sample %d)", p ? p->integrator : -1, p ? p->direct_sample : -1);
    if (!shard_in_range(p)) return fail(KY_ERR_LIMIT, "frame too large for the device's 32-bit work-item and pixel indices (%d x %d, %d spp)", p->width, p->height, p->samples_per_pixel);
    if (film_range_check(p, scene) != KY_OK) return KY_ERR_LIMIT;
    if (!d_tiles) return fail(KY_ERR_INVALID_VALUE, "d_tiles is NULL");
    DeviceCtx* c;
    int rcode = get_ctx(device, &c);
    if (rcode != KY_OK) return rcode;
    std::lock_guard<std::mutex> lock(c->m);
    hipStream_t stream = (hipStream_t)stream_;
    SceneSlot* sc;
    rcode = upload_scene(c, scene, stream, &sc);
    if (rcode != KY_OK) return rcode;

    const ShardConst sh = make_shard(p);
    if (sh.n_tiles == 0) return KY_OK;
    const RenderConst rc = make_rc(p);
    StreamState* st;
    rcode = get_stream_state(c, stream, &st);
    if (rcode != KY_OK) return rcode;

    const size_t need = workspace_bytes_for(sh);
    void* ws = d_workspace;
    if (!(d_workspace && workspace_bytes >= need)) {
        if (st->ws_bytes < need) {
            HIP_TRY(hipStreamSynchronize(stream));
            if (st->ws) HIP_TRY(hipFree(st->ws));
            st->ws = nullptr; st->ws_bytes = 0;
            HIP_TRY(hipMalloc(&st->ws, need));
            st->ws_bytes = need;
            st->ws_clean = false;
        }
        ws = st->ws;
    }
    unsigned long long* accum = (unsigned long long*)ws;
    unsigned* flags = (unsigned*)(accum + (size_t)sh.n_pix * 3);
    const bool large_scene = scene->surface_count > KY_LDS_SURFACES || scene->material_count > KY_LDS_MATERIALS;
    const size_t lds_bytes = large_scene ? (size_t)lds_scene_bytes(scene->surface_count, scene->material_count, scene->light_count) : 0;
    const bool own_ws = ws == st->ws;
    if (!(own_ws && st->ws_clean)) {
        HIP_TRY(hipMemsetAsync(ws, 0, own_ws ? st->ws_bytes : need, stream));
        HIP_TRY(hipMemsetAsync(st->d_counter, 0, sizeof(unsigned), stream));
    }
    st->ws_clean = false;

    if (current_engine() == KY_ENGINE_QUEUE && p->integrator == KY_INTEGRATOR_PATH_TRACING_ITERATION && !large_scene) {
        const int variant = p->sampler == KY_SAMPLER_DEBUG ? 2 : (p->direct_sample == KY_DIRECT_BOTH_MIS ? 0 : 1);
        const int per_cu = c->q_blocks_per_cu[variant] > 0 ? c->q_blocks_per_cu[variant] : 1;
        unsigned grid = (unsigned)(c->cus * per_cu);
        const unsigned need_blocks = (unsigned)(((unsigned long long)sh.n_items * 64u + QE_SLOTS - 1) / QE_SLOTS);
        if (grid > need_blocks) grid = need_blocks;
        if (grid < 1) grid = 1;
        rcode = set_film_limit(st, film_term_count(p, sc->h->n_lights, true, false), stream);
        if (rcode != KY_OK) return rcode;
        HIP_TRY(hipEventRecord(st->ev0, stream));
        if (variant == 0) hipLaunchKernelGGL((render_kernel_q<false, KY_DIRECT_BOTH_MIS>), dim3(grid), dim3(QE_THREADS), 0, stream, sc->d, rc, sh, st->d_counter, accum, flags);
        else if (variant == 1) hipLaunchKernelGGL((render_kernel_q<false, -1>), dim3(grid), dim3(QE_THREADS), 0, stream, sc->d, rc, sh, st->d_counter, accum, flags);
        else hipLaunchKernelGGL((render_kernel_q<true, -1>), dim3(grid), dim3(QE_THREADS), 0, stream, sc->d, rc, sh, st->d_counter, accum, flags);
        c->last_variant = -2;
    } else {
        const Variant* v = pick_variant(p, sc->h, shadow_queue_wanted(scene), sh.n_pix);
        if (!v) return fail(KY_ERR_DEVICE, "internal: no render kernel for these parameters");
        const int vi = (int)(v - g_variants);
        DeviceCtx::JitKernel* jk = nullptr;
        bool queue = v->queue;
        const int jit_mode = kyjit::mode();
        c->last_note.clear();
        if (v->strategy < 0 && jit_mode == 0) c->last_note = " [the run-time-dispatched kernel: no row of the table holds this launch's strategy / integrator / shapes; kyhip_set_jit(1 / 2) instantiates its own]";
        const bool jit_wanted = jit_mode != 0 && (!kyjit::mode_by_default() || v->feat == 0 || v->strategy < 0);
        if (jit_wanted && specialisation_enabled() && p->integrator >= KY_INTEGRATOR_DIRECT_LIGHTING) {
            const bool dbg = p->sampler == KY_SAMPLER_DEBUG, general = sc->h->general != 0;
            int feat = (dbg || general) ? 0 : sc->h->feat;
            const bool env_pair = (feat & KY_FEAT_SINGLE_ENV) && p->direct_sample == KY_DIRECT_BOTH_MIS && p->integrator != KY_INTEGRATOR_PATH_TRACING_RECURSION;
            if (!((feat & (KY_FEAT_SINGLE_AREA | KY_FEAT_SINGLE_DELTA)) || env_pair)) feat &= ~KY_FEAT_BOXES;
            const bool want_queue = (p->direct_sample == KY_DIRECT_BOTH_MIS || p->direct_sample == KY_DIRECT_LIGHT_MIS || p->direct_sample == KY_DIRECT_LIGHT) &&
                                    p->integrator == KY_INTEGRATOR_PATH_TRACING_ITERATION && sh.n_pix < (1 << 26) && !general && shadow_queue_wanted(scene);
            const bool same = v->dbg == dbg && v->strategy == p->direct_sample && v->queue == want_queue && v->general == general && v->feat == feat &&
                              v->integrator == p->integrator && v->large == large_scene;
            if (!same) {
                char expr[192];
                snprintf(expr, sizeof expr, "%s, %d, %s, %s, %d, %d, %s", dbg ? "true" : "false", p->direct_sample, want_queue ? "true" : "false",
                         general ? "true" : "false", feat, p->integrator, large_scene ? "true" : "false");
                DeviceCtx::JitKernel& k = c->jit[expr];
                if (!k.fn && !k.failed) {
                    bool pending = false;
                    const kyjit::Code* code = kyjit::get_code(expr, jit_mode == 1, &pending);
                    if (code) {
                        if (!(hipModuleLoadData(&k.module, code->object.data()) == hipSuccess && hipModuleGetFunction(&k.fn, k.module, kyjit::k_entry) == hipSuccess)) {
                            (void)hipGetLastError();
                            k.fn = nullptr;
                            k.failed = true;
                        }
                    } else if (!pending) {
                        k.failed = true;
                    }
                    if (pending) c->last_note = " [its own instantiation render_kernel<" + std::string(expr) + "> is being compiled (kyhip_set_jit mode 2): this frame ran on the table's kernel]";
                }
                if (k.failed) c->last_note = " [its own instantiation is unavailable: " + kyjit::status() + "]";
                if (k.fn) {
                    if (k.lds != lds_bytes) {
                        int per_cu = 0;
                        HIP_TRY(hipModuleOccupancyMaxActiveBlocksPerMultiprocessor(&per_cu, k.fn, 256, lds_bytes));
                        k.per_cu = per_cu > 0 ? per_cu : 1;
                        k.lds = lds_bytes;
                    }
                    jk = &k;
                    queue = want_queue;
                    char desc[224];
                    snprintf(desc, sizeof desc, "render_kernel<%sstrategy %d%s%s%s, feat %d, integrator %d> = render_kernel<", dbg ? "debug sampler, " : "", p->direct_sample,
                             want_queue ? ", deferred shadow rays" : "", general ? ", general shapes" : "", large_scene ? ", scene-sized LDS block" : "", feat, p->integrator);
                    c->last_jit = std::string(desc) + expr + ">";
                }
            }
        }
        if (!jk && (c->variant_blocks[vi] == 0 || c->variant_lds[vi] != lds_bytes)) {
            int per_cu = 0;
            HIP_TRY(hipOccupancyMaxActiveBlocksPerMultiprocessor(&per_cu, v->fn, 256, lds_bytes));
            c->variant_blocks[vi] = per_cu > 0 ? per_cu : 1;
            c->variant_lds[vi] = lds_bytes;
        }
        const int per_cu = jk ? jk->per_cu : c->variant_blocks[vi];
        unsigned grid = (unsigned)(c->cus * per_cu);
        const int cap = blocks_per_cu_cap();
        if (cap > 0 && cap < per_cu) grid = (unsigned)(c->cus * cap);
        const unsigned need_blocks = sh.n_items / 4 + 1;
        if (grid > need_blocks) grid = need_blocks;
        if (grid < 1) grid = 1;
        if (queue && st->sq_blocks < (size_t)c->cus * per_cu) {
            if (st->d_shadow_queue) {
                HIP_TRY(hipStreamSynchronize(stream));
                HIP_TRY(hipFree(st->d_shadow_queue));
                st->d_shadow_queue = nullptr; st->sq_blocks = 0;
            }
            const size_t blocks = (size_t)c->cus * per_cu;
            HIP_TRY(hipMalloc(&st->d_shadow_queue, blocks * 4 * KY_SQ_ENTRY * KY_SQ_CAP * sizeof(float4)));
            st->sq_blocks = blocks;
        }
        rcode = set_film_limit(st, film_term_count(p, sc->h->n_lights, false, queue), stream);
        if (rcode != KY_OK) return rcode;
        HIP_TRY(hipEventRecord(st->ev0, stream));
        float4* queue_mem = queue ? st->d_shadow_queue : (float4*)nullptr;
        if (jk) {
            const DScene* a_scene = sc->d;
            RenderConst a_rc = rc;
            ShardConst a_sh = sh;
            unsigned* a_counter = st->d_counter;
            void* args[] = {&a_scene, &a_rc, &a_sh, &a_counter, &accum, &flags, &queue_mem};
            HIP_TRY(hipModuleLaunchKernel(jk->fn, grid, 1, 1, 256, 1, 1, (unsigned)lds_bytes, stream, args, nullptr));
            c->last_variant = -3;
        } else {
            hipLaunchKernelGGL(v->fn, dim3(grid), dim3(256), lds_bytes, stream, (const DScene*)sc->d, rc, sh, st->d_counter, accum, flags, queue_mem);
            c->last_variant = vi;
        }
    }
    HIP_TRY(hipGetLastError());
    HIP_TRY(hipEventRecord(st->ev1, stream));
    st->timing_valid = true;
    c->last_launch = st;
    hipLaunchKernelGGL(resolve_kernel, dim3((sh.n_pix + 255) / 256), dim3(256), 0, stream, accum, flags, d_tiles, sh.n_pix, st->d_counter);
    HIP_TRY(hipGetLastError());
    st->ws_clean = own_ws;
    HIP_TRY(hipEventRecord(st->done, stream));
    sc->readers |= 1u << (unsigned)(st - c->ss);
    return KY_OK;
}

float kyhip_kernel_ms(int device) {
    DeviceCtx* c = find_ctx(device);
    if (!c) return -1.f;
    std::lock_guard<std::mutex> lock(c->m);
    if (!c->last_launch || !c->last_launch->timing_valid) return -1.f;
    float ms = -1.f;
    if (hipEventElapsedTime(&ms, c->last_launch->ev0, c->last_launch->ev1) != hipSuccess) return -1.f;
    return ms;
}

const char* kyhip_last_kernel(int device) {
    static thread_local std::string name;
    name.clear();
    DeviceCtx* c = find_ctx(device);
    if (!c) return name.c_str();
    std::lock_guard<std::mutex> lock(c->m);
    if (c->last_variant == -2) name = "render_kernel_q (queue engine)";
    else if (c->last_variant == -3) name = c->last_jit + " (run-time instantiation; template arguments: DEBUG_SAMPLER, STRATEGY, QUEUE, GENERAL, FEAT, INTEGRATOR, LARGE)";
    else if (c->last_variant >= 0) {
        const Variant& v = g_variants[c->last_variant];
        char buf[160];
        snprintf(buf, sizeof buf, "render_kernel<%sstrategy %d%s%s%s, feat %d, integrator %d>", v.dbg ? "debug sampler, " : "", v.strategy, v.queue ? ", deferred shadow rays" : "",
                 v.general ? ", general shapes" : "", v.large ? ", scene-sized LDS block" : "", v.feat, v.integrator);
        name = buf;
    }
    name += c->last_note;
    return name.c_str();
}

int kyhip_film_add_tiles_device(int device, const ky_render_params* p, const float* d_tiles, float* d_film, size_t stride_px, void* stream_) {
    if (!valid_params(p) || !shard_in_range(p)) return fail(KY_ERR_INVALID_VALUE, "invalid render params");
    if (!d_tiles || !d_film || stride_px < (size_t)p->width) return fail(KY_ERR_INVALID_VALUE, "bad film arguments");
    DeviceCtx* c;
    int rcode = get_ctx(device, &c);
    if (rcode != KY_OK) return rcode;
    std::lock_guard<std::mutex> lock(c->m);
    const ShardConst sh = make_shard(p);
    if (sh.n_pix == 0) return KY_OK;
    hipLaunchKernelGGL(film_add_kernel, dim3((sh.n_pix + 255) / 256), dim3(256), 0, (hipStream_t)stream_, d_tiles, d_film, stride_px, sh, p->width, p->height);
    HIP_TRY(hipGetLastError());
    return KY_OK;
}

int kyhip_film_add_gathered_device(int device, const ky_render_params* p, int world, const float* d_gathered, size_t rank_stride_floats,
                                   float* d_film, size_t stride_px, void* stream_) {
    if (!valid_params(p) || !shard_in_range(p)) return fail(KY_ERR_INVALID_VALUE, "invalid render params");
    if (world < 1 || (long long)p->tile_step * world > 0x7fffffffLL) return fail(KY_ERR_INVALID_VALUE, "bad shard count %d", world);
    if (!d_gathered || !d_film || stride_px < (size_t)p->width) return fail(KY_ERR_INVALID_VALUE, "bad film arguments");
    ky_render_params q = *p;
    q.tile_step = p->tile_step * world;
    if (rank_stride_floats < (size_t)make_shard(&q).n_pix * 3) return fail(KY_ERR_INVALID_VALUE, "rank_stride_floats is smaller than a shard's tile buffer");
    DeviceCtx* c;
    int rcode = get_ctx(device, &c);
    if (rcode != KY_OK) return rcode;
    std::lock_guard<std::mutex> lock(c->m);
    const int n = p->width * p->height, tiles_x = (p->width + p->tile_w - 1) / p->tile_w;
    hipLaunchKernelGGL(film_add_gathered_kernel, dim3((n + 255) / 256), dim3(256), 0, (hipStream_t)stream_, d_gathered, rank_stride_floats, world, d_film, stride_px,
                       p->tile_w, p->tile_h, p->tile_first, p->tile_step, tiles_x, p->width, p->height);
    HIP_TRY(hipGetLastError());
    return KY_OK;
}

int kyhip_smallpt_render(int device, const ky_smallpt_sphere* spheres, int n, const ky_smallpt_params* p, double* image_rgb) {
    int rcode = kyh::smallpt_check(spheres, n, p);
    if (rcode != KY_OK) return rcode;
    if (!image_rgb) return fail(KY_ERR_INVALID_VALUE, "null image");
    DeviceCtx* c = nullptr;
    rcode = get_ctx(device, &c);
    if (rcode != KY_OK) return rcode;
    std::lock_guard<std::mutex> lock(c->m);
    kysp::SpSphere packed[kysp::SP_MAX_SPHERES];
    kysp::sp_pack(spheres, n, packed);
    kysp::SpConst k;
    kysp::sp_make_const(p, n, k);
    const size_t n_px = (size_t)p->width * p->height;
    DevBuf d_sph, d_sub, d_img;
    HIP_TRY(d_sph.alloc(sizeof(packed)));
    HIP_TRY(d_sub.alloc(n_px * 12 * sizeof(double)));
    HIP_TRY(d_img.alloc(n_px * 3 * sizeof(double)));
    HIP_TRY(hipMemcpy(d_sph.p, packed, sizeof(packed), hipMemcpyHostToDevice));
    const int blocks = ((p->width + 7) / 8) * ((p->height + 7) / 8);
    StreamState* st;
    rcode = get_stream_state(c, 0, &st);
    if (rcode != KY_OK) return rcode;
    HIP_TRY(hipEventRecord(st->ev0, 0));
    hipLaunchKernelGGL(kysp::smallpt_kernel, dim3(blocks), dim3(256), 0, 0, d_sph.as<kysp::SpSphere>(), k, d_sub.as<double>());
    HIP_TRY(hipGetLastError());
    HIP_TRY(hipEventRecord(st->ev1, 0));
    st->timing_valid = true;
    c->last_launch = st;
    hipLaunchKernelGGL(kysp::smallpt_resolve_kernel, dim3((unsigned)((n_px + 255) / 256)), dim3(256), 0, 0, d_sub.as<double>(), d_img.as<double>(), p->width, p->height, p->variant);
    HIP_TRY(hipGetLastError());
    HIP_TRY(hipMemcpy(image_rgb, d_img.p, n_px * 3 * sizeof(double), hipMemcpyDeviceToHost));
    return KY_OK;
}

int kyhip_smallpt_kat_radiance(int device, const ky_smallpt_sphere* spheres, int n_spheres, const ky_smallpt_params* p,
                               int x, int y, int sx, int sy, int s0, int n, double* out3) {
    int rcode = kyh::smallpt_check(spheres, n_spheres, p);
    if (rcode != KY_OK) return rcode;
    if (!out3 || n <= 0 || s0 < 0 || x < 0 || y < 0 || x >= p->width || y >= p->height || (sx | sy) < 0 || sx > 1 || sy > 1)
        return fail(KY_ERR_INVALID_VALUE, "bad KAT arguments");
    if (p->variant == KY_SP_VARIANT_REWRITE && (sx | sy) != 0) return fail(KY_ERR_INVALID_VALUE, "variant 1 has no subpixels: sx = sy = 0");
    DeviceCtx* c = nullptr;
    rcode = get_ctx(device, &c);
    if (rcode != KY_OK) return rcode;
    std::lock_guard<std::mutex> lock(c->m);
// ... 16 lines not shown
```

ky_amd/csrc/ky_pack.cpp:

```cpp
#include <algorithm>
#include <cmath>
#include <cstdarg>
#include <cstdio>
#include <cstdlib>
#include <cstring>
#include <limits>
#include <thread>
#include <sched.h>
#include <unistd.h>

#include "ky_host.hpp"

namespace kyh {

static thread_local std::string g_error;

int fail(int code, const char* fmt, ...) {
    char buf[512];
    va_list ap;
    va_start(ap, fmt);
    vsnprintf(buf, sizeof buf, fmt, ap);
    va_end(ap);
    g_error = buf;
    return code;
// ... 333 lines not shown
        for (int j = 0; j < 3; ++j) n[j] /= len;
        const double k = n[0] * sh.p[1][0] + n[1] * sh.p[1][1] + n[2] * sh.p[1][2];
        double lo = inf, hi = -inf;
        for (int j = 0; j < ns; ++j) shape_extent(shape_of(j), n, lo, hi);
        for (int l = 0; l < nl; ++l) {
            const ky_light& L = in->lights[l];
            if (L.kind == KY_LIGHT_AREA) shape_extent(in->shapes[L.shape], n, lo, hi);
            if (L.kind == KY_LIGHT_POINT) { const double c = n[0] * L.position[0] + n[1] * L.position[1] + n[2] * L.position[2]; lo = std::min(lo, c); hi = std::max(hi, c); }
        }
        const int side = lo >= k ? 1 : (hi <= k ? -1 : 0);
        if (side == 0) continue;
        bool ok = true;
        for (int y = 0; y < ns && ok; ++y) {
            if (y == i) continue;
            double lo_y = inf, hi_y = -inf;
            shape_extent(shape_of(y), n, lo_y, hi_y);
            ok = offset_safe(y, n, k, side, lo_y, hi_y);
        }
        if (!ok) continue;
        R.wall[i] = 1;
        for (int l = 0; l < nl; ++l) {
            const ky_light& L = in->lights[l];
            if (L.kind == KY_LIGHT_DIRECTION || L.kind == KY_LIGHT_ENVIRONMENT) continue;
            double lo_l = inf, hi_l = -inf;
            if (L.kind == KY_LIGHT_AREA) shape_extent(in->shapes[L.shape], n, lo_l, hi_l);
            else lo_l = hi_l = n[0] * L.position[0] + n[1] * L.position[1] + n[2] * L.position[2];
            const double nearest = side > 0 ? lo_l - k : k - hi_l;
            if (!(nearest > 1.01 * K_HOST_RAY_OFFSET)) R.light_ok[l] = 0;
        }
    }
    R.deferred_ok = true;
    for (int l = 0; l < nl; ++l) R.deferred_ok = R.deferred_ok && R.light_ok[l];
    R.ts_behind.assign(ns, 0);
    for (int l = 0; l < nl && R.ts_light < 0; ++l) {
        const ky_light& L = in->lights[l];
        if (L.kind != KY_LIGHT_AREA || !R.light_ok[l]) continue;
        const ky_shape& ls = in->shapes[L.shape];
        if (ls.kind == KY_SHAPE_SPHERE) continue;
        const double n[3] = {ls.normal[0], ls.normal[1], ls.normal[2]};
        double k_min = inf, k_max = -inf;
        if (ls.kind == KY_SHAPE_DISK) {
            k_min = k_max = n[0] * ls.p[0][0] + n[1] * ls.p[0][1] + n[2] * ls.p[0][2];
        } else if (ls.kind == KY_SHAPE_TRIANGLE) {
            shape_extent(ls, n, k_min, k_max);
        } else {
            const double c0 = n[0] * ls.p[0][0] + n[1] * ls.p[0][1] + n[2] * ls.p[0][2], c1 = n[0] * ls.p[1][0] + n[1] * ls.p[1][1] + n[2] * ls.p[1][2],
                         c2 = n[0] * ls.p[2][0] + n[1] * ls.p[2][1] + n[2] * ls.p[2][2];
            k_min = std::min(std::min(c0, c1), std::min(c2, c0 + c2 - c1));
        }
        int count = 0;
        std::vector<char> behind(ns, 0);
        for (int y = 0; y < ns; ++y) {
            const ky_shape& sh = shape_of(y);
            if (sh.kind != KY_SHAPE_RECTANGLE || R.wall[y] || in->surfaces[y].shape == L.shape) continue;
            double lo_y = inf, hi_y = -inf;
            shape_extent(sh, n, lo_y, hi_y);
            if (hi_y <= k_min) { behind[y] = 1; ++count; }
        }
        if (count == 0) continue;
        R.ts_light = l;
        R.ts_behind = behind;
        R.ts_plane[0] = n[0]; R.ts_plane[1] = n[1]; R.ts_plane[2] = n[2]; R.ts_plane[3] = k_min;
    }
}

static int g_specialise = -1;
bool specialisation_enabled() {
    if (g_specialise < 0) {
        const char* e = std::getenv("KYHIP_SPECIALISE");
        g_specialise = (e && std::atoi(e) == 0) ? 0 : 1;
    }
    return g_specialise != 0;
}

static int g_boxes = -1;
bool boxes_enabled() {
    if (g_boxes < 0) {
        const char* e = std::getenv("KYHIP_BOXES");
        g_boxes = (e && std::atoi(e) == 0) ? 0 : 1;
    }
    return g_boxes != 0;
}

int pack_scene(const ky_scene* in, DScene* out) {
    if (!in) return fail(KY_ERR_INVALID_VALUE, "scene is NULL");
    if (in->surface_count < 0 || in->shape_count < 0 || in->material_count < 0 || in->light_count < 0)
        return fail(KY_ERR_INVALID_VALUE, "negative count in scene");
    if (in->surface_count > KYHIP_MAX_SURFACES || in->shape_count > KYHIP_MAX_SHAPES || in->material_count > KYHIP_MAX_MATERIALS ||
        in->light_count > KYHIP_MAX_LIGHTS)
        return fail(KY_ERR_LIMIT, "scene exceeds device limits (%d surfaces, %d shapes, %d materials, %d lights)", in->surface_count,
                    in->shape_count, in->material_count, in->light_count);
    if (in->environment_light < -1 || in->environment_light >= in->light_count) return fail(KY_ERR_INVALID_VALUE, "environment_light out of range");
    std::memset(out, 0, sizeof *out);
    out->n_surfaces = in->surface_count; out->n_lights = in->light_count; out->n_materials = in->material_count;
    out->env_light = in->environment_light;
    cp3(out->cam_position, in->camera.position); cp3(out->cam_front, in->camera.front); cp3(out->cam_right, in->camera.right);
    cp3(out->cam_up, in->camera.up);
    out->cam_inv_w = 1.f / in->camera.resolution[0]; out->cam_inv_h = 1.f / in->camera.resolution[1];
    std::vector<DSurf> recs(in->surface_count);
    std::vector<DShapeFull> fulls(in->surface_count);
    for (int i = 0; i < in->surface_count; ++i) {
        const ky_surface& sf = in->surfaces[i];
        if (sf.shape < 0 || sf.shape >= in->shape_count || sf.material < 0 || sf.material >= in->material_count || sf.area_light < -1 ||
            sf.area_light >= in->light_count)
            return fail(KY_ERR_INVALID_VALUE, "surface %d has an index out of range", i);
        const ky_shape& sh = in->shapes[sf.shape];
        if (sh.kind < KY_SHAPE_DISK || sh.kind > KY_SHAPE_SPHERE) return fail(KY_ERR_INVALID_VALUE, "shape %d has an unknown kind", sf.shape);
        if (!shape_normal_ok(sh)) return fail(KY_ERR_INVALID_VALUE, "shape %d: the stored normal must be unit length", sf.shape);
        if (sf.area_light >= 0 && in->lights[sf.area_light].kind != KY_LIGHT_AREA)
            return fail(KY_ERR_INVALID_VALUE, "surface %d: area_light must refer to an area light", i);
        pack_shape(sh, 0, &recs[i], &fulls[i]);
    }
    for (int i = 0; i < in->light_count; ++i)
        if (in->lights[i].kind == KY_LIGHT_AREA && (in->lights[i].shape < 0 || in->lights[i].shape >= in->shape_count))
            return fail(KY_ERR_INVALID_VALUE, "area light %d: shape out of range", i);
    for (int i = 0; i < in->surface_count; ++i)
        if (in->surfaces[i].shape < 0 || in->surfaces[i].shape >= in->shape_count || in->surfaces[i].material < 0 || in->surfaces[i].material >= in->material_count)
            return fail(KY_ERR_INVALID_VALUE, "surface %d has an index out of range", i);
    NonOccluders non;
    find_non_occluders(in, non);
    int j = 0;
    struct PlanarEntry { int surface, axis; DAar aar; DPar par; };
    std::vector<PlanarEntry> planar;
    for (int pass = -3; pass < 3; ++pass) {
        for (int i = 0; i < in->surface_count; ++i) {
            const ky_surface& sf = in->surfaces[i];
            const ky_shape& sh = in->shapes[sf.shape];
            DAar aar{};
            const int axis = recs[i].kind == TK_PARALLELOGRAM ? axis_aligned_rectangle(sh, &aar) : -1;
            const int group = axis >= 0 ? axis - 3 : (recs[i].kind == TK_PARALLELOGRAM ? 0 : (recs[i].kind == TK_SPHERE ? 1 : 2));
            if (group != pass) continue;
            if (pass < 0) {
                const int32_t sorted_index = j;
                std::memcpy(&aar.q1.y, &sorted_index, 4);
                planar.push_back(PlanarEntry{i, axis, aar, DPar{}});
            } else if (pass == 0) {
                PlanarEntry e{i, -1, DAar{}, DPar{}};
                std::memcpy(&e.par.q0, &recs[i].f[0], 16); std::memcpy(&e.par.q1, &recs[i].f[4], 16); std::memcpy(&e.par.q2, &recs[i].f[8], 16);
                planar.push_back(e);
            } else if (pass == 1) {
                std::memcpy(&out->sph[out->n_sph++].c, &recs[i].f[0], 16);
                out->sph[out->n_sph] = out->sph[out->n_sph - 1];
            } else {
                DSurf& d = out->gen[out->n_gen++];
                d = recs[i];
                d.full = j;
            }
            out->full[j] = fulls[i];
            out->all[j] = recs[i];
            out->all[j].full = j;
            DHit& h = out->hit[j];
            cp3(h.n, sh.kind == KY_SHAPE_SPHERE ? sh.p[0] : sh.normal);
            h.kind = sh.kind; h.material = sf.material; h.area_light = sf.area_light;
            if (sh.kind != KY_SHAPE_SPHERE) host_frame(sh.normal, h.fs, h.ft);
            out->orig[j] = i;
            ++j;
        }
    }
    auto build_trav = [&](DTrav& T, auto&& skip) {
        std::memset(&T, 0, sizeof T);
        for (const PlanarEntry& e : planar) {
            if (skip(e.surface)) continue;
            if (e.axis >= 0) { T.n_aar_axis[e.axis]++; T.aar[T.n_aar++] = e.aar; }
            else T.par[T.n_par++] = e.par;
        }
        if (T.n_aar > 0) T.aar[T.n_aar] = T.aar[T.n_aar - 1];
// ... 57 lines not shown
            if (in->materials[in->surfaces[i].material].kind == KY_MATERIAL_PLASTIC && in->shapes[in->surfaces[i].shape].kind != KY_SHAPE_RECTANGLE) flat_phong = false;
        if (flat_phong) out->feat |= KY_FEAT_FLAT_PHONG;
        if (out->trav.n_aar > 0 && out->trav.n_par == 0 && out->n_gen == 0) out->feat |= KY_FEAT_AXIS_ALIGNED;
        bool x_planks = out->trav.n_par > 0;
        for (int i = 0; i < out->trav.n_par; ++i) {
            const DPar& r = out->trav.par[i];
            if (!(r.q0.x == 0.f && r.q1.x == 0.f && r.q2.y == 0.f && r.q2.z == 0.f)) x_planks = false;
        }
        if (x_planks) out->feat |= KY_FEAT_X_PLANKS;
    }
    if (non.ts_light >= 0) {
        build_trav(out->occ_front, [&](int i) { return non.wall[i] != 0 || non.ts_behind[i] != 0; });
        build_trav(out->occ_behind, [&](int i) { return non.ts_behind[i] == 0; });
        double size = 0;
        for (int i = 0; i < in->surface_count; ++i)
            for (int q = 0; q < 4; ++q)
                for (int c = 0; c < 3; ++c) size = std::max(size, std::fabs((double)in->shapes[in->surfaces[i].shape].p[q][c]));
        for (int c = 0; c < 3; ++c) out->ts_plane[c] = (float)non.ts_plane[c];
        out->ts_plane[3] = (float)(non.ts_plane[3] + 1e-5 * (1.0 + size));
    }
    for (int i = 0; i < in->material_count; ++i) {
        const ky_material& m = in->materials[i];
        if (m.kind < KY_MATERIAL_MATTE || m.kind > KY_MATERIAL_PLASTIC) return fail(KY_ERR_INVALID_VALUE, "material %d has an unknown kind", i);
        pack_material(m, &out->mat[i]);
    }
    for (int i = 0; i < in->light_count; ++i) {
        const ky_light& l = in->lights[i];
        if (l.kind < KY_LIGHT_POINT || l.kind > KY_LIGHT_ENVIRONMENT) return fail(KY_ERR_INVALID_VALUE, "light %d has an unknown kind", i);
        DLight& d = out->light[i];
        cp3(d.color, l.color); cp3(d.position, l.position); cp3(d.direction, l.direction);
        for (int j = 0; j < 3; ++j)
            if (d.color[j] != d.color[j]) d.color[j] = std::numeric_limits<float>::quiet_NaN();
        d.kind = l.kind; d.world_radius = l.world_radius; d.shape_kind = -1;
        d.occ_ok = non.light_ok[i];
        d.shadow_table = (i == non.ts_light) ? ((int32_t)__builtin_offsetof(DScene, occ_front) | 1)
                                             : (int32_t)(non.light_ok[i] ? __builtin_offsetof(DScene, occ) : __builtin_offsetof(DScene, trav));
        if (l.kind == KY_LIGHT_AREA) {
            if (l.shape < 0 || l.shape >= in->shape_count) return fail(KY_ERR_INVALID_VALUE, "area light %d: shape out of range", i);
            const ky_shape& sh = in->shapes[l.shape];
            if (sh.kind < KY_SHAPE_DISK || sh.kind > KY_SHAPE_SPHERE) return fail(KY_ERR_INVALID_VALUE, "shape %d has an unknown kind", l.shape);
            if (!shape_normal_ok(sh)) return fail(KY_ERR_INVALID_VALUE, "shape %d: the stored normal must be unit length", l.shape);
            d.shape_kind = sh.kind; d.radius = sh.radius; d.area = host_shape_area(sh); d.inv_area = 1 / d.area;
            cp3(d.n, sh.normal);
            d.aar_axis = -1;
            if (sh.kind == KY_SHAPE_RECTANGLE) {
                DAar a{};
                d.aar_axis = axis_aligned_rectangle(sh, &a);
                if (d.aar_axis >= 0) { d.aar[0] = a.q0.x; d.aar[1] = a.q0.y; d.aar[2] = a.q0.z; d.aar[3] = a.q0.w; d.aar[4] = a.q1.x; }
            }
            if (sh.kind == KY_SHAPE_RECTANGLE) {
                cp3(d.p1, sh.p[1]);
                for (int j = 0; j < 3; ++j) { d.e0[j] = sh.p[0][j] - sh.p[1][j]; d.e1[j] = sh.p[2][j] - sh.p[1][j]; }
            } else if (sh.kind == KY_SHAPE_TRIANGLE) {
                cp3(d.p1, sh.p[0]); cp3(d.e0, sh.p[1]); cp3(d.e1, sh.p[2]);
            } else {
                cp3(d.p1, sh.p[0]);
                if (sh.kind == KY_SHAPE_SPHERE) d.e0[0] = 1.f / sh.radius;
            }
            pack_shape(sh, KYHIP_MAX_SURFACES + i, &d.isect, &out->full[KYHIP_MAX_SURFACES + i]);
            if (d.isect.kind != TK_PARALLELOGRAM && d.isect.kind != TK_SPHERE) out->general = 1;
            d.sampled_is_surface = 0;
            for (int j2 = 0; j2 < in->surface_count; ++j2) d.sampled_is_surface |= in->surfaces[j2].shape == l.shape;
            d.n_carriers = 0;
            for (int j2 = 0; j2 < out->n_surfaces; ++j2) {
                if (out->hit[j2].area_light != i) continue;
                if (d.n_carriers >= 0 && d.n_carriers < KY_MAX_CARRIERS) d.carrier[d.n_carriers++] = j2;
                else d.n_carriers = -1;
            }
            d.pdf_from_carrier = (d.n_carriers == 1 && d.isect.kind == TK_PARALLELOGRAM && in->surfaces[out->orig[d.carrier[0]]].shape == l.shape) ? 1 : 0;
            if (d.aar_axis < 0 && d.n_carriers >= 1 && out->all[d.carrier[0]].kind == TK_SPHERE) std::memcpy(d.aar, out->all[d.carrier[0]].f, 16);
        }
    }
    if (out->n_gen > 0) out->general = 1;
    if (specialisation_enabled() && !out->general) {
        bool carriers = true;
        for (int i = 0; i < in->light_count; ++i)
            if (in->lights[i].kind == KY_LIGHT_AREA && out->light[i].n_carriers < 0) carriers = false;
        if (carriers) out->feat |= KY_FEAT_CARRIERS;
        bool own = true, any_area = false;
        for (int i = 0; i < in->light_count; ++i)
            if (in->lights[i].kind == KY_LIGHT_AREA) { any_area = true; own = own && out->light[i].pdf_from_carrier != 0; }
        if (carriers && any_area && own) out->feat |= KY_FEAT_OWN_CARRIER;
    }
    return KY_OK;
}

#ifndef KY_SQ_MIN_SPHERE_MARGIN
#define KY_SQ_MIN_SPHERE_MARGIN 5
#endif
static int g_shadow_queue = -2;
int shadow_queue_mode() {
    if (g_shadow_queue == -2) {
        const char* e = std::getenv("KYHIP_SHADOW_QUEUE");
        g_shadow_queue = e ? (std::atoi(e) != 0 ? 1 : 0) : -1;
    }
    return g_shadow_queue;
}
bool shadow_queue_wanted(const ky_scene* scene) {
    const int mode = shadow_queue_mode();
    if (mode >= 0) return mode == 1 && scene->light_count > 0;
    int spheres = 0, deltas = 0;
    for (int i = 0; i < scene->light_count; ++i) {
        const ky_light& l = scene->lights[i];
        if (l.kind == KY_LIGHT_AREA && l.shape >= 0 && l.shape < scene->shape_count && scene->shapes[l.shape].kind == KY_SHAPE_SPHERE) ++spheres;
        if (l.kind == KY_LIGHT_POINT || l.kind == KY_LIGHT_DIRECTION) ++deltas;
    }
    return spheres - deltas >= KY_SQ_MIN_SPHERE_MARGIN;
}

int blocks_per_cu_cap() {
    static const int cap = [] { const char* e = std::getenv("KYHIP_BLOCKS_PER_CU"); return e ? std::atoi(e) : 0; }();
    return cap;
}

static int g_engine = -1;
int current_engine() {
    if (g_engine < 0) {
        const char* e = std::getenv("KYHIP_ENGINE");
        g_engine = (e && (!std::strcmp(e, "queue") || !std::strcmp(e, "1"))) ? KY_ENGINE_QUEUE : KY_ENGINE_LANE;
    }
    return g_engine;
}

uint64_t scene_hash(const DScene& s) {
    static_assert(sizeof(DScene) % 8 == 0, "hashed in 64-bit words");
    const uint64_t* w = reinterpret_cast<const uint64_t*>(&s);
    uint64_t h0 = 0x9E3779B97F4A7C15ull, h1 = 0xC2B2AE3D27D4EB4Full;
    for (size_t i = 0; i + 1 < sizeof(DScene) / 8; i += 2) {
        h0 = (h0 ^ w[i]) * 0xff51afd7ed558ccdull; h0 ^= h0 >> 29;
        h1 = (h1 ^ w[i + 1]) * 0xc4ceb9fe1a85ec53ull; h1 ^= h1 >> 31;
    }
    if ((sizeof(DScene) / 8) & 1) h0 = (h0 ^ w[sizeof(DScene) / 8 - 1]) * 0xff51afd7ed558ccdull;
    return h0 ^ (h1 * 0x9E3779B97F4A7C15ull);
}

bool scene_input(const ky_scene* in, std::vector<unsigned char>& out, uint64_t& hash) {
    out.clear();
    if (!in || in->surface_count < 0 || in->shape_count < 0 || in->material_count < 0 || in->light_count < 0 || in->surface_count > KYHIP_MAX_SURFACES ||
        in->shape_count > KYHIP_MAX_SHAPES || in->material_count > KYHIP_MAX_MATERIALS || in->light_count > KYHIP_MAX_LIGHTS)
        return false;
    auto put = [&](const void* p, size_t n) { const unsigned char* b = (const unsigned char*)p; out.insert(out.end(), b, b + n); };
    const int32_t head[6] = {in->shape_count, in->material_count, in->light_count, in->surface_count, in->environment_light, (specialisation_enabled() ? 1 : 0) | (boxes_enabled() ? 2 : 0)};
    put(head, sizeof head);
    put(&in->camera, sizeof in->camera);
    if (in->shape_count) put(in->shapes, sizeof(ky_shape) * (size_t)in->shape_count);
    if (in->material_count) put(in->materials, sizeof(ky_material) * (size_t)in->material_count);
    if (in->light_count) put(in->lights, sizeof(ky_light) * (size_t)in->light_count);
    if (in->surface_count) put(in->surfaces, sizeof(ky_surface) * (size_t)in->surface_count);
    out.resize((out.size() + 7) & ~(size_t)7, 0);
    uint64_t h = 0x9E3779B97F4A7C15ull;
    for (size_t i = 0; i < out.size(); i += 8) {
        uint64_t w;
        std::memcpy(&w, &out[i], 8);
        h = (h ^ w) * 0xff51afd7ed558ccdull;
        h ^= h >> 29;
    }
    hash = h;
    return true;
}

int cpus_granted() {
    static const int n = [] {
        int cpus = (int)std::thread::hardware_concurrency();
        cpu_set_t mask;
        if (sched_getaffinity(0, sizeof mask, &mask) == 0 && CPU_COUNT(&mask) > 0) cpus = CPU_COUNT(&mask);
        if (cpus < 1) cpus = 1;
        if (FILE* f = std::fopen("/sys/fs/cgroup/cpu.max", "r")) {
            char quota[32] = {0};
            long period = 0;
            if (std::fscanf(f, "%31s %ld", quota, &period) == 2 && std::strcmp(quota, "max") != 0 && period > 0) {
                const long q = (std::atol(quota) + period / 2) / period;
                if (q >= 1 && q < cpus) cpus = (int)q;
            }
            std::fclose(f);
        }
        return cpus;
    }();
    return n;
}

int seam_threads() {
    static const int n = [] {
        if (const char* e = std::getenv("KYHIP_SEAM_THREADS")) { const int v = std::atoi(e); if (v >= 1 && v <= 16) return v; }
        const int cpus = cpus_granted();
        return std::max(1, std::min(cpus, 4));
    }();
    return n;
}

void host_add_rows(float* __restrict__ film, size_t stride_px, const float* __restrict__ src, int width, int y0, int y1) {
    const size_t n = (size_t)width * 3;
    for (int y = y0; y < y1; ++y) {
        float* __restrict__ dst = film + (size_t)y * stride_px * 3;
        const float* __restrict__ row = src + (size_t)y * n;
        for (size_t i = 0; i < n; ++i) dst[i] += row[i];
    }
}
void HostPool::run(int n, const std::function<void(int)>& fn) {
    std::lock_guard<std::mutex> one(job_m_);
    if (n <= 1) { if (n == 1) fn(0); return; }
    {
        std::lock_guard<std::mutex> lock(m_);
        if (pid_ != getpid()) { pid_ = getpid(); n_threads_ = 0; }
        while (n_threads_ < n - 1) { const int id = ++n_threads_; std::thread([this, id] { loop(id); }).detach(); }
        fn_ = &fn; n_ = n; pending_ = n - 1; ++generation_;
    }
    cv_.notify_all();
    fn(0);
    std::unique_lock<std::mutex> lock(m_);
    done_.wait(lock, [this] { return pending_ == 0; });
    fn_ = nullptr;
}
void HostPool::loop(int id) {
    unsigned long long seen = 0;
    for (;;) {
        const std::function<void(int)>* fn = nullptr;
        {
            std::unique_lock<std::mutex> lock(m_);
            cv_.wait(lock, [&] { return generation_ != seen && id < n_; });
            seen = generation_;
            fn = fn_;
        }
        (*fn)(id);
        std::lock_guard<std::mutex> lock(m_);
        if (--pending_ == 0) done_.notify_one();
    }
}
std::vector<std::unique_lock<std::mutex>> lock_seams(std::vector<std::pair<int, std::mutex*>> by_device) {
    std::sort(by_device.begin(), by_device.end(), [](const std::pair<int, std::mutex*>& a, const std::pair<int, std::mutex*>& b) { return a.first < b.first; });
    by_device.erase(std::unique(by_device.begin(), by_device.end(), [](const std::pair<int, std::mutex*>& a, const std::pair<int, std::mutex*>& b) { return a.first == b.first; }), by_device.end());
    std::vector<std::unique_lock<std::mutex>> locks;
    locks.reserve(by_device.size());
    for (auto& d : by_device) locks.emplace_back(*d.second);
    return locks;
}
HostPool& host_pool() { static HostPool* pool = new HostPool; return *pool; }

int smallpt_check(const ky_smallpt_sphere* spheres, int n, const ky_smallpt_params* p) {
    if (!spheres || !p) return fail(KY_ERR_INVALID_VALUE, "null argument");
    if (p->variant != KY_SP_VARIANT_SMALLPT && p->variant != KY_SP_VARIANT_REWRITE) return fail(KY_ERR_INVALID_VALUE, "unknown smallpt variant %d", p->variant);
    if (n <= 0 || n > KY_SP_MAX_SPHERES) return fail(KY_ERR_INVALID_VALUE, "1..%d spheres", KY_SP_MAX_SPHERES);
    if (p->width <= 0 || p->height <= 0 || p->width > 16384 || p->height > 16384 || p->samps <= 0 || p->max_depth < 0)
        return fail(KY_ERR_INVALID_VALUE, "invalid smallpt params");
    for (int i = 0; i < n; ++i)
        if (spheres[i].refl < KY_SP_DIFF || spheres[i].refl > KY_SP_REFR || !(spheres[i].rad > 0)) return fail(KY_ERR_INVALID_VALUE, "sphere %d is invalid", i);
    return KY_OK;
}

void set_engine_raw(int v) { g_engine = v; }
void set_specialise_raw(int v) { g_specialise = v; }
void set_boxes_raw(int v) { g_boxes = v; }
void set_shadow_queue_raw(int v) { g_shadow_queue = v; }
}

using namespace kyh;

extern "C" {

const char* kyhip_last_error(void) { return kyh::last_error().c_str(); }
int kyhip_seam_threads(void) { return kyh::seam_threads(); }
int kyhip_abi_version(void) { return KYHIP_ABI_VERSION; }


int kyhip_set_engine(int engine) {
    const int prev = current_engine();
    if (engine == KY_ENGINE_LANE || engine == KY_ENGINE_QUEUE) kyh::set_engine_raw(engine);
    return prev;
}
int kyhip_set_specialisation(int on) {
    const int prev = specialisation_enabled() ? 1 : 0;
    if (on == 0 || on == 1) kyh::set_specialise_raw(on);
    return prev;
}
int kyhip_set_boxes(int on) {
    const int prev = boxes_enabled() ? 1 : 0;
    if (on == 0 || on == 1) kyh::set_boxes_raw(on);
    return prev;
}
int kyhip_set_shadow_queue(int mode) {
    const int prev = shadow_queue_mode();
    if (mode >= -1 && mode <= 1) kyh::set_shadow_queue_raw(mode);
    return prev;
}

int64_t kyhip_shard_tile_count(const ky_render_params* p) {
    if (!valid_params(p)) return fail(KY_ERR_INVALID_VALUE, "invalid render params");
    return make_shard(p).n_tiles;
}
int64_t kyhip_film_term_limit(const ky_render_params* p, int n_lights, int engine, int deferred, float* limit) {
    if (!valid_params(p) || n_lights < 0 || n_lights > KYHIP_MAX_LIGHTS || (engine != 0 && engine != 1)) return fail(KY_ERR_INVALID_VALUE, "invalid render params");
    const long long n = film_term_count(p, n_lights, engine == 1, deferred != 0);
    const float t = film_term_limit(n);
    if (limit) *limit = t;
    return t > 0.f ? n : fail(KY_ERR_LIMIT, "%lld terms per pixel: no term limit >= 1 keeps their sum inside the 32.32 accumulator", n);
}
int64_t kyhip_shard_float_count(const ky_render_params* p) {
    if (!valid_params(p)) return fail(KY_ERR_INVALID_VALUE, "invalid render params");
    return (int64_t)make_shard(p).n_pix * 3;
}

size_t kyhip_workspace_bytes(const ky_render_params* p) {
    if (!valid_params(p)) return 0;
    return workspace_bytes_for(make_shard(p));
}


int kyhip_scene_non_occluders(const ky_scene* scene, int light, int* left_out, int n) {
    if (!scene || !left_out || n < 0) return fail(KY_ERR_INVALID_VALUE, "bad arguments");
    std::vector<DScene> packed(1);
    const int rc = pack_scene(scene, &packed[0]);
    if (rc != KY_OK) return rc;
    if (n < scene->surface_count) return fail(KY_ERR_INVALID_VALUE, "left_out holds %d entries, the scene has %d surfaces", n, scene->surface_count);
    if (light < -1 || light >= scene->light_count) return fail(KY_ERR_INVALID_VALUE, "light %d out of range", light);
    NonOccluders non;
    find_non_occluders(scene, non);
    const DScene& P = packed[0];
    int count = 0;
    for (int j = 0; j < P.n_surfaces; ++j) {
        const int i = P.orig[j];
        const bool planar = P.all[j].kind == TK_PARALLELOGRAM;
        left_out[i] = (planar && non.wall[i] && (light < 0 || non.light_ok[light])) ? 1 : 0;
        if (planar && light >= 0 && light == non.ts_light && non.ts_behind[i]) left_out[i] = 2;
        count += left_out[i] == 1;
    }
    const DTrav& T = (light < 0 || non.light_ok[light]) ? P.occ : P.trav;
    if (count != P.trav.n_aar + P.trav.n_par - T.n_aar - T.n_par) return fail(KY_ERR_DEVICE, "internal: occluder table and classification disagree");
    return count;
}

int kyhip_scene_facts(const ky_scene* scene) {
    if (!scene) return fail(KY_ERR_INVALID_VALUE, "bad arguments");
    std::vector<DScene> packed(1);
    const int rc = pack_scene(scene, &packed[0]);
    return rc != KY_OK ? rc : packed[0].feat;
}

int kyhip_scene_boxes(const ky_scene* scene, int* box_face, int n) {
    if (!scene || !box_face || n < 0) return fail(KY_ERR_INVALID_VALUE, "bad arguments");
    std::vector<DScene> packed(1);
    const int rc = pack_scene(scene, &packed[0]);
    if (rc != KY_OK) return rc;
    if (n < scene->surface_count) return fail(KY_ERR_INVALID_VALUE, "box_face holds %d entries, the scene has %d surfaces", n, scene->surface_count);
    for (int i = 0; i < scene->surface_count; ++i) box_face[i] = -1;
    const DScene& P = packed[0];
    for (int b = 0; b < P.boxtrav.n_box; ++b) {
        const DBox& d = P.boxtrav.box[b];
        const float* src[6] = {&d.q0.w, &d.q1.w, &d.q2.x, &d.q2.y, &d.q2.z, &d.q2.w};
        for (int f = 0; f < 6; ++f) {
            uint32_t sidx;
            std::memcpy(&sidx, src[f], 4);
            if (sidx != (uint32_t)KY_BOX_NO_FACE) box_face[P.orig[sidx]] = 8 * b + f;
        }
    }
    return P.boxtrav.n_box;
}

int kyhip_smallpt_scene(ky_smallpt_sphere* out) {
    if (!out) return fail(KY_ERR_INVALID_VALUE, "null output");
    struct Row { double rad, p[3], e[3], c[3]; int refl; };
    static const Row rows[9] = {
        {1e5, {1e5 + 1, 40.8, 81.6}, {0, 0, 0}, {.75, .25, .25}, KY_SP_DIFF},
        {1e5, {-1e5 + 99, 40.8, 81.6}, {0, 0, 0}, {.25, .25, .75}, KY_SP_DIFF},
        {1e5, {50, 40.8, 1e5}, {0, 0, 0}, {.75, .75, .75}, KY_SP_DIFF},
        {1e5, {50, 40.8, -1e5 + 170}, {0, 0, 0}, {0, 0, 0}, KY_SP_DIFF},
        {1e5, {50, 1e5, 81.6}, {0, 0, 0}, {.75, .75, .75}, KY_SP_DIFF},
        {1e5, {50, -1e5 + 81.6, 81.6}, {0, 0, 0}, {.75, .75, .75}, KY_SP_DIFF},
        {16.5, {27, 16.5, 47}, {0, 0, 0}, {1 * .999, 1 * .999, 1 * .999}, KY_SP_SPEC},
        {16.5, {73, 16.5, 78}, {0, 0, 0}, {1 * .999, 1 * .999, 1 * .999}, KY_SP_REFR},
        {600, {50, 681.6 - .27, 81.6}, {12, 12, 12}, {0, 0, 0}, KY_SP_DIFF}};
    for (int i = 0; i < 9; ++i) {
        out[i].rad = rows[i].rad;
        for (int j = 0; j < 3; ++j) { out[i].p[j] = rows[i].p[j]; out[i].e[j] = rows[i].e[j]; out[i].c[j] = rows[i].c[j]; }
        out[i].refl = rows[i].refl;
        out[i].pad_ = 0;
    }
    return 9;
}

int kyhip_smallpt_scene_rewrite(ky_smallpt_sphere* out) {
    const int n = kyhip_smallpt_scene(out);
    if (n < 0) return n;
    static const double z[9] = {-81.6, -81.6, -1e5, 1e5 - 170, -81.6, -81.6, -47, -78, -81.6};
    for (int i = 0; i < n; ++i) out[i].p[2] = z[i];
    return n;
}

}
```

ky_amd/csrc/ky_render.hpp:

```cpp
#pragma once
#include "ky_device.hpp"
#include "ky_shard.hpp"

using namespace kyd;

#ifndef KY_MAX_RETRACE
#define KY_MAX_RETRACE 1
#endif
#ifndef KY_REFILL_BATCH
#define KY_REFILL_BATCH 6
#endif
#ifndef KY_REFILL_WAIT
#define KY_REFILL_WAIT 4
#endif
#ifndef KY_RETRACE_THRESHOLD
#define KY_RETRACE_THRESHOLD 80
#endif
#ifndef KY_WAVES_PER_EU
#define KY_WAVES_PER_EU 7
#endif
#ifndef KY_WAVES_PER_EU_QUEUE
#define KY_WAVES_PER_EU_QUEUE 6
#endif
#ifndef KY_WAVES_PER_EU_QUEUE_FEAT
#define KY_WAVES_PER_EU_QUEUE_FEAT 7
#endif
#ifndef KY_WAVES_PER_EU_HOT
#define KY_WAVES_PER_EU_HOT 8
#endif
#ifndef KY_WAVES_PER_EU_ENV
#define KY_WAVES_PER_EU_ENV 7
#endif
#ifndef KY_WAVES_PER_EU_NO_FACTS
#define KY_WAVES_PER_EU_NO_FACTS 7
#endif
#ifndef KY_WAVES_PER_EU_NO_FACTS_GENERAL
#define KY_WAVES_PER_EU_NO_FACTS_GENERAL 6
#endif
#ifndef KY_WAVES_PER_EU_GENERIC
#define KY_WAVES_PER_EU_GENERIC 5
#endif

constexpr int KY_FEAT_CORNELL = KY_FEAT_SINGLE_AREA | KY_FEAT_RECT_LIGHTS | KY_FEAT_CARRIERS | KY_FEAT_OWN_CARRIER;
constexpr int KY_FEAT_VEACH = KY_FEAT_SPHERE_LIGHTS | KY_FEAT_CARRIERS | KY_FEAT_NO_DELTA | KY_FEAT_SMALL_TABLES;

struct ItemSlot {
    int x0, y0, pix0, s_begin, s_end;
};

template <bool DEBUG_SAMPLER, int STRATEGY, bool QUEUE, bool GENERAL, int FEAT, int INTEGRATOR, bool LARGE>
constexpr int ky_waves_per_eu() {
    return STRATEGY >= 0 ? (QUEUE ? (FEAT ? KY_WAVES_PER_EU_QUEUE_FEAT : KY_WAVES_PER_EU_QUEUE)
                                  : ((FEAT == 0 && STRATEGY == KY_DIRECT_BOTH_MIS) ? ((GENERAL || INTEGRATOR == KY_INTEGRATOR_PATH_TRACING_RECURSION) ? KY_WAVES_PER_EU_NO_FACTS_GENERAL : KY_WAVES_PER_EU_NO_FACTS)
                                     : ((FEAT != 0 && STRATEGY == KY_DIRECT_BOTH_MIS && INTEGRATOR == KY_INTEGRATOR_PATH_TRACING_ITERATION) ? ((FEAT & KY_FEAT_SINGLE_ENV) ? KY_WAVES_PER_EU_ENV : KY_WAVES_PER_EU_HOT) : KY_WAVES_PER_EU)))
                         : KY_WAVES_PER_EU_GENERIC;
}

template <bool DEBUG_SAMPLER, int STRATEGY, bool QUEUE = false, bool GENERAL = false, int FEAT = 0, int INTEGRATOR = KY_INTEGRATOR_PATH_TRACING_ITERATION, bool LARGE = false>
KY_DEV void render_kernel_body(const DScene* __restrict__ S_, RenderConst rc, ShardConst sh, unsigned* __restrict__ counter, unsigned long long* __restrict__ accum,
                               unsigned* __restrict__ flags, float4* __restrict__ queue_mem) {
    static_assert(!QUEUE || ((STRATEGY == KY_DIRECT_BOTH_MIS || STRATEGY == KY_DIRECT_LIGHT_MIS || STRATEGY == KY_DIRECT_LIGHT) && INTEGRATOR == KY_INTEGRATOR_PATH_TRACING_ITERATION),
                  "the deferred shadow rays belong to the iterative integrator's strategies with a light-sampling half");
    static_assert(FEAT == 0 || (STRATEGY >= 0 && !GENERAL && !DEBUG_SAMPLER), "scene facts are instantiated for kernels with a fixed strategy only");
    static_assert(STRATEGY >= 0 || INTEGRATOR == KY_INTEGRATOR_PATH_TRACING_ITERATION, "the run-time-dispatched kernel reads the integrator from rc");
    const SceneRef S{S_, GENERAL, FEAT, LARGE};
    __shared__ ItemSlot ring[4][KY_RING];
    __shared__ int c_xy[256], c_pix[256];
    __shared__ unsigned c_se[256];
    __shared__ uint32_t c_key[QUEUE ? 1 : 256];
    __shared__ unsigned long long c_def[QUEUE ? 3 * 256 : 1];
    const int tid = threadIdx.x;
    const LdsScene Lds = stage_scene<LARGE, (FEAT & KY_FEAT_SMALL_TABLES) != 0>(S);
    if (STRATEGY >= 0) { rc.strategy = STRATEGY; rc.integrator = INTEGRATOR; }
    const int nee_weight = (rc.strategy == KY_DIRECT_IDLE || rc.integrator < KY_INTEGRATOR_DIRECT_LIGHTING ||
                            rc.integrator == KY_INTEGRATOR_SIMPLE_PATH_TRACING_RECURSION) ? 0 : S->n_lights;

    const int lane = threadIdx.x & 63;
    ItemSlot* my_ring = ring[threadIdx.x >> 6];

    int fetched = 0;
    int cursor = 0;
    bool exhausted = false;
    c_pix[tid] = -1;
    ShadowQueue sq{nullptr, 0, c_pix, c_def, accum, flags, counter};
    if (QUEUE) {
        c_def[tid] = 0; c_def[256 + tid] = 0; c_def[512 + tid] = 0;
        sq.base = queue_mem + (size_t)(blockIdx.x * 4 + (threadIdx.x >> 6)) * (KY_SQ_ENTRY * KY_SQ_CAP);
    }
    bool open = false;
    bool has_item = false, done = false, alive = false;
    int waited = 0;
    PathState ps;
    ps.Lo = mk3(0, 0, 0);

    KY_CLK(-1);
    for (;;) {
        KY_CLK(9);
        const bool need = !alive && !done && !open;
        const unsigned long long need_mask = __ballot(need);
        bool refill = need_mask != 0;
        if (refill && __popcll(need_mask) < KY_REFILL_BATCH && waited < KY_REFILL_WAIT && __any(alive || (open && !done))) { refill = false; ++waited; }
        if (refill) {
            waited = 0;
            if (need && has_item) {
                const float v[3] = {ps.Lo.x * rc.inv_spp, ps.Lo.y * rc.inv_spp, ps.Lo.z * rc.inv_spp};
                ps.Lo = mk3(0, 0, 0);
                const int pix = c_pix[tid];
                c_pix[tid] = -1;
                const bool plain = fminf(fminf(v[0], v[1]), v[2]) >= 0.f && (v[0] + v[1] + v[2]) < 1.0f;
                if (__all(plain)) {
#pragma unroll
                    for (int ch = 0; ch < 3; ++ch) {
                        const float hi = __builtin_floorf(v[ch]);
                        const float lo = __builtin_rintf((v[ch] - hi) * 4294967296.0f);
                        unsigned long long fx = ((unsigned long long)(unsigned)hi << 32) | (unsigned long long)(unsigned)lo;
                        if (QUEUE) { fx += c_def[ch * 256 + tid]; c_def[ch * 256 + tid] = 0; }
                        atomicAdd(&accum[(size_t)pix * 3 + ch], fx);
                    }
                } else
                {
                    unsigned fl = 0;
                    const float limit = film_limit(counter);
#pragma unroll
                    for (int ch = 0; ch < 3; ++ch) {
                        unsigned long long fx = film_fixed(v[ch], limit, ch, fl);
                        if (QUEUE) { fx += c_def[ch * 256 + tid]; c_def[ch * 256 + tid] = 0; }
                        if (fx != 0) atomicAdd(&accum[(size_t)pix * 3 + ch], fx);
                    }
                    if (fl) atomicOr(&flags[pix], fl);
                }
                has_item = false;
            }
            const int n_need = __popcll(need_mask);
            while (!exhausted && cursor + n_need > fetched * 64) {
                unsigned id = blockIdx.x * 4u + (threadIdx.x >> 6);
                if (fetched > 0 && lane == 0) id = atomicAdd(counter, 1u) + gridDim.x * 4u;
                id = __builtin_amdgcn_readfirstlane(id);
                if (id >= sh.n_items) { exhausted = true; break; }
                const int c = (int)(id / (unsigned)sh.n_blocks), b = (int)(id % (unsigned)sh.n_blocks);
                const int k = b / sh.blocks_per_tile, inner = b % sh.blocks_per_tile;
                const int bx = inner % sh.blocks_w, by = inner / sh.blocks_w;
                const int tile = sh.tile_first + k * sh.tile_step;
                if (lane == 0) {
                    ItemSlot it;
                    const int trow = tile / sh.tiles_x, tcol = (tile % sh.tiles_x + trow) % sh.tiles_x;
                    it.x0 = tcol * sh.tile_w + bx * 8;
                    it.y0 = trow * sh.tile_h + by * 8;
                    it.pix0 = (k * sh.tile_h + by * 8) * sh.tile_w + bx * 8;
// ... 3 lines not shown
#endif
                    my_ring[fetched % KY_RING] = it;
                }
                ++fetched;
            }
            __builtin_amdgcn_fence(__ATOMIC_ACQ_REL, "wavefront");
            if (need) {
                const int mine = cursor + (int)__builtin_amdgcn_mbcnt_hi((unsigned)(need_mask >> 32), __builtin_amdgcn_mbcnt_lo((unsigned)need_mask, 0u));
                if (mine < fetched * 64) {
                    const ItemSlot it = my_ring[(mine >> 6) % KY_RING];
#ifdef KY_EXP_TRANSPOSE
                    const int px = 0, py = 0;
#else
                    const int px = mine & 7, py = (mine >> 3) & 7;
#endif
                    const int x = it.x0 + px, y = it.y0 + py;
                    const bool in_range = x < rc.width && y < rc.height;
                    c_xy[tid] = x | (y << 16);
                    c_pix[tid] = it.pix0 + py * sh.tile_w + px;
                    if (!QUEUE) c_key[tid] = sampler_pixel_key(rc.seed, (uint32_t)(y * rc.width + x));
#ifdef KY_EXP_TRANSPOSE
                    c_se[tid] = ((unsigned)((mine & 63) * 16) << 7) | 16u;
                    open = in_range;
#else
                    c_se[tid] = ((unsigned)it.s_begin << 7) | (unsigned)(it.s_end - it.s_begin);
                    open = in_range && it.s_begin < it.s_end;
#endif
                    has_item = in_range;
                } else {
                    done = true;
                }
            }
            cursor = min(cursor + n_need, fetched * 64);
        }
        KY_CLK(0);
        Vertex v;
        v.in_lds = true;
        bool have_vertex = false;
        for (int attempt = 0;; ++attempt) {
            if (!alive && !done && open) {
                const int xy = c_xy[tid];
                const unsigned se = c_se[tid];
                const uint32_t key = QUEUE ? sampler_pixel_key(rc.seed, (uint32_t)((xy >> 16) * rc.width + (xy & 0xffff))) : c_key[tid];
                path_begin<DEBUG_SAMPLER, true>(ps, S, key, xy & 0xffff, xy >> 16, (int)(se >> 7));
                c_se[tid] = se + 127;
                open = (se & 127) > 1;
                alive = true;
            }
            const bool tracing = alive && !have_vertex;
            if (!__any(tracing)) break;
            if (tracing) {
                const bool ended = !path_intersect<DEBUG_SAMPLER>(ps, v, S, Lds, rc);
                if (!ended) have_vertex = true;
                if (ended) {
                    alive = false;
                }
            }
            if (attempt >= ((FEAT & KY_FEAT_SINGLE_LIGHT) ? 0 : KY_MAX_RETRACE)) break;
            const int idle = __popcll(__ballot(!alive && !done && open));
            if (idle * (2 * nee_weight + 1) < KY_RETRACE_THRESHOLD) break;
        }
        KY_CLK(1);
        if (!__any(alive)) {
            if (__all(done)) break;
            path_state_dead(ps);
            continue;
        }
        unsigned tag = 0;
        if (QUEUE) tag = ((unsigned)c_pix[tid] << 6) | (unsigned)lane;
        {
            const bool cont = path_shade<DEBUG_SAMPLER>(ps, v, S, Lds, rc, have_vertex, -1, nullptr, QUEUE ? &sq : nullptr, tag,
                                                        STRATEGY >= 0 && INTEGRATOR == KY_INTEGRATOR_PATH_TRACING_RECURSION, true);
            if (have_vertex && !cont) {
                alive = false;
            }
        }
    }
    if (QUEUE) {
        sq_drain(S, sq);
    }
    KY_CLK(-2);
}

template <bool DEBUG_SAMPLER, int STRATEGY, bool QUEUE = false, bool GENERAL = false, int FEAT = 0, int INTEGRATOR = KY_INTEGRATOR_PATH_TRACING_ITERATION, bool LARGE = false>
__global__ __launch_bounds__(256, (ky_waves_per_eu<DEBUG_SAMPLER, STRATEGY, QUEUE, GENERAL, FEAT, INTEGRATOR, LARGE>())) void render_kernel(
    const DScene* __restrict__ S_, RenderConst rc, ShardConst sh, unsigned* __restrict__ counter, unsigned long long* __restrict__ accum, unsigned* __restrict__ flags,
    float4* __restrict__ queue_mem) {
    render_kernel_body<DEBUG_SAMPLER, STRATEGY, QUEUE, GENERAL, FEAT, INTEGRATOR, LARGE>(S_, rc, sh, counter, accum, flags, queue_mem);
}
```

ky_amd/csrc/ky_scene.hpp:

```cpp
#pragma once
#ifndef __HIPCC_RTC__
#include <hip/hip_vector_types.h>
#include <stdint.h>
#endif

#include "../../include/kyhip.h"

#if defined(__HIPCC__) || defined(__HIPCC_RTC__)
#define KY_HD __host__ __device__
#else
#define KY_HD
#endif

namespace kyd {

enum : int {
    TK_DISK = KY_SHAPE_DISK,
    TK_TRIANGLE = KY_SHAPE_TRIANGLE,
    TK_QUAD = KY_SHAPE_RECTANGLE,
    TK_SPHERE = KY_SHAPE_SPHERE,
    TK_PARALLELOGRAM = 4
};

struct DSurf {
// ... 17 lines not shown
    int32_t kind;
    int32_t material;
    int32_t area_light;
    float fs[3], ft[3];
    int32_t pad_h[4];
};
static_assert(sizeof(DHit) == 64, "DHit");

struct DMat {
    float c0[3];
    int32_t kind;
    float c1[3];
    float eta;
    float exponent, phong_pdf_norm, p_specular;
    int32_t exp_flags;
    float cs[3];
    float inv_eta;
};

struct DLight {
    float color[3];
    int32_t kind;
    float position[3];
    float world_radius;
    float direction[3];
    int32_t shape_kind;
    float p1[3];
    float radius;
    float e0[3];
    float area;
    float e1[3];
    float inv_area;
    float n[3];
    int32_t n_carriers;
    int32_t carrier[4];
    int32_t sampled_is_surface;
    int32_t occ_ok;
    int32_t pdf_from_carrier;
    int32_t shadow_table;
    float aar[5];
    int32_t aar_axis;
    int32_t pad_a[2];
    DSurf isect;
};
constexpr int KY_MAX_CARRIERS = 4;
static_assert(sizeof(DLight) % 16 == 0 && __builtin_offsetof(DLight, p1) % 16 == 0 && __builtin_offsetof(DLight, n) % 16 == 0, "DLight is read in 16-byte groups (shape_sample_position)");

struct DPar {
    float4 q0, q1, q2;
};
struct DSph {
    float4 c;
};
struct DAar {
    float4 q0, q1;
};

struct DBox {
    float4 q0, q1, q2;
};
constexpr int KY_MAX_BOXES = 4, KY_BOX_MIN_FACES = 4, KY_BOX_NO_FACE = 15;
struct DBoxTrav {
    int32_t n_box, n_aar, pad_b0, pad_b1;
    int32_t n_aar_axis[3], pad_b2;
    DBox box[KY_MAX_BOXES];
    DAar aar[KYHIP_MAX_SURFACES + 1];
};

struct DTrav {
    int32_t n_aar, n_par, pad_t0, pad_t1;
    int32_t n_aar_axis[3], pad_t2;
    DAar aar[KYHIP_MAX_SURFACES + 1];
    DPar par[KYHIP_MAX_SURFACES + 1];
};
struct DScene {
    int32_t n_surfaces, n_lights, n_materials, env_light;
    int32_t n_sph, n_gen, general, occ_deferred_ok;
    float cam_position[3], cam_inv_w;
    float cam_front[3], cam_inv_h;
    float cam_right[3], pad0;
    float cam_up[3], pad1;
    DTrav trav;
    DTrav occ;
    int32_t ts_light, feat, ts_pad[2];
    float ts_plane[4];
    DTrav occ_front, occ_behind;
    DBoxTrav boxtrav;
    DSph sph[KYHIP_MAX_SURFACES + 1];
    DSurf gen[KYHIP_MAX_SURFACES];
    DSurf all[KYHIP_MAX_SURFACES];
    DShapeFull full[KYHIP_MAX_SURFACES + KYHIP_MAX_LIGHTS];
    DHit hit[KYHIP_MAX_SURFACES];
    int32_t orig[KYHIP_MAX_SURFACES];
    DMat mat[KYHIP_MAX_MATERIALS];
    DLight light[KYHIP_MAX_LIGHTS];
};
static_assert(__builtin_offsetof(DScene, light) % 16 == 0 && __builtin_offsetof(DScene, trav) % 16 == 0 && __builtin_offsetof(DScene, boxtrav) % 16 == 0 &&
              __builtin_offsetof(DBoxTrav, box) % 16 == 0, "16-byte scalar loads of light, table and box records");


enum : int {
    KY_FEAT_SINGLE_AREA = 1,
    KY_FEAT_RECT_LIGHTS = 2,
    KY_FEAT_CARRIERS = 4,
    KY_FEAT_SINGLE_DELTA = 8,
    KY_FEAT_SINGLE_ENV = 16,
    KY_FEAT_SPHERE_LIGHTS = 32,
    KY_FEAT_NO_DELTA = 64,
    KY_FEAT_OWN_CARRIER = 256,
    KY_FEAT_BOXES = 512,
    KY_FEAT_AXIS_ALIGNED = 1024,
    KY_FEAT_FLAT_PHONG = 2048,
    KY_FEAT_X_PLANKS = 4096,
    KY_FEAT_SMALL_TABLES = 128
};
constexpr int KY_FEAT_SINGLE_LIGHT = KY_FEAT_SINGLE_AREA | KY_FEAT_SINGLE_DELTA | KY_FEAT_SINGLE_ENV;

constexpr int KY_LDS_SURFACES = 64, KY_LDS_MATERIALS = 32;
constexpr int KY_LDS_SURFACES_SMALL = 16, KY_LDS_MATERIALS_SMALL = 8;
KY_HD inline int lds_scene_mat_offset(int n_surfaces) { return (n_surfaces * (int)sizeof(DHit) + 15) & ~15; }
KY_HD inline int lds_scene_light_offset(int n_surfaces, int n_materials) { return lds_scene_mat_offset(n_surfaces) + n_materials * (int)sizeof(DMat); }
KY_HD inline int lds_scene_bytes(int n_surfaces, int n_materials, int n_lights) { return lds_scene_light_offset(n_surfaces, n_materials) + n_lights * 16; }

struct RenderConst {
    int integrator, max_path_depth, strategy;
    uint32_t seed;
    int width, height, spp;
    float inv_spp;
};

}
```

Baseline: 22230.

## Specialise render kernels on compile-time per-scene shape counts

Packs per-axis counts of boxes, axis-aligned rectangles, spheres and shadow-table entries into a 64-bit scene code. New kernel variants take this code as a template parameter, so traversal and shadow loops run fixed-count, fully unrolled scans instead of reading counts and table headers from scene memory at run time. The aim is to drop loop overhead, header loads and the indirect shadow-table lookup on known scenes. The cost is more kernel instantiations and code size, plus extra register pressure from unrolling, and it only applies when the scene matches a compiled shape code.

```diff
diff --git a/include/kyhip.h b/include/kyhip.h
--- a/include/kyhip.h
+++ b/include/kyhip.h
@@ -138,6 +138,7 @@
 int         kyhip_set_engine(int engine);
 int         kyhip_set_specialisation(int on);
 int         kyhip_set_boxes(int on);
+int         kyhip_set_shape_counts(int on);
 int         kyhip_set_shadow_queue(int mode);
 int         kyhip_set_jit(int mode);
 const char* kyhip_jit_status(void);
@@ -188,6 +189,7 @@
 int kyhip_scene_non_occluders(const ky_scene* scene, int light, int* left_out, int n);
 int kyhip_scene_boxes(const ky_scene* scene, int* box_face, int n);
 int kyhip_scene_facts(const ky_scene* scene);
+int64_t kyhip_scene_shapes(const ky_scene* scene);
 
 int kyhip_kat_li(int device, const ky_scene* scene, const ky_render_params* params,
                  int x, int y, int s0, int n, float* out3);
diff --git a/ky_amd/_abi.py b/ky_amd/_abi.py
--- a/ky_amd/_abi.py
+++ b/ky_amd/_abi.py
@@ -84,6 +84,7 @@
     "kyhip_set_engine": (C.c_int, [C.c_int]),
     "kyhip_set_specialisation": (C.c_int, [C.c_int]),
     "kyhip_set_boxes": (C.c_int, [C.c_int]),
+    "kyhip_set_shape_counts": (C.c_int, [C.c_int]),
     "kyhip_set_shadow_queue": (C.c_int, [C.c_int]),
     "kyhip_set_jit": (C.c_int, [C.c_int]),
     "kyhip_jit_status": (C.c_char_p, []),
@@ -124,6 +125,7 @@
     "kyhip_scene_non_occluders": (C.c_int, [SP, C.c_int, C.c_void_p, C.c_int]),
     "kyhip_scene_boxes": (C.c_int, [SP, C.c_void_p, C.c_int]),
     "kyhip_scene_facts": (C.c_int, [SP]),
+    "kyhip_scene_shapes": (C.c_int64, [SP]),
     "kyhip_kat_li": (C.c_int, [C.c_int, SP, PP, C.c_int, C.c_int, C.c_int, C.c_int, C.c_void_p]),
 }
 
diff --git a/ky_amd/api.py b/ky_amd/api.py
--- a/ky_amd/api.py
+++ b/ky_amd/api.py
@@ -217,6 +217,20 @@
     return rc
 
 
+def scene_shapes(scene):
+    lib = A.load_kyhip()
+    rc = lib.kyhip_scene_shapes(_scene_ptr(scene))
+    if rc < 0:
+        _check(rc)
+    return rc
+
+
+def scene_shape_counts(code):
+    f = [(code >> (3 * i)) & 7 for i in range(17)]
+    return {"boxes": f[0], "box_aar": tuple(f[1:4]), "trav": tuple(f[4:7]), "sph": f[7], "occ": tuple(f[8:11]), "front": tuple(f[11:14]),
+            "behind": tuple(f[14:17]), "table": (code >> 51) & 3, "two_stage": bool((code >> 53) & 1)}
+
+
 def scene_boxes(scene):
     lib = A.load_kyhip()
     n = _scene_ptr(scene).contents.surface_count
diff --git a/ky_amd/csrc/ky_device.hpp b/ky_amd/csrc/ky_device.hpp
--- a/ky_amd/csrc/ky_device.hpp
+++ b/ky_amd/csrc/ky_device.hpp
@@ -87,8 +87,12 @@
     bool general;
     int feat;
     bool large;
-    __device__ __forceinline__ SceneRef(const DScene* p_) : p(p_), general(true), feat(0), large(true) {}
-    __device__ __forceinline__ SceneRef(const DScene* p_, bool general_, int feat_ = 0, bool large_ = false) : p(p_), general(general_), feat(feat_), large(large_) {}
+    unsigned long long shapes;
+    __device__ __forceinline__ SceneRef(const DScene* p_) : p(p_), general(true), feat(0), large(true), shapes(0) {}
+    __device__ __forceinline__ SceneRef(const DScene* p_, bool general_, int feat_ = 0, bool large_ = false, unsigned long long shapes_ = 0)
+        : p(p_), general(general_), feat(feat_), large(large_), shapes(shapes_) {}
+    __device__ __forceinline__ bool known() const { return shapes != 0; }
+    __device__ __forceinline__ int count(int field) const { return shape_count(shapes, field); }
     __device__ __forceinline__ const DScene* operator->() const { return p; }
     __device__ __forceinline__ bool single_area() const { return (feat & KY_FEAT_SINGLE_AREA) != 0; }
     __device__ __forceinline__ bool single_light() const { return (feat & KY_FEAT_SINGLE_LIGHT) != 0; }
@@ -494,7 +498,101 @@
     return full_shape_hit(full[S.full], o, d, tmax, t_out);
 }
 
+template <int AXIS, bool NEAREST>
+KY_DEV void aar_scan_known(SceneRef S, unsigned aar_off, int first, int n, f3 o, f3 d, f3 inv_d, float& tmax, int& best, unsigned& occ_v) {
+    if (n <= 0) return;
+    const unsigned long long ex = __builtin_amdgcn_ballot_w64(true);
+    const float oa = AXIS == 0 ? o.x : (AXIS == 1 ? o.y : o.z), ia = AXIS == 0 ? inv_d.x : (AXIS == 1 ? inv_d.y : inv_d.z);
+    const float ou_ = AXIS == 0 ? o.y : (AXIS == 1 ? o.z : o.x), du_ = AXIS == 0 ? d.y : (AXIS == 1 ? d.z : d.x);
+    const float ov_ = AXIS == 0 ? o.z : (AXIS == 1 ? o.x : o.y), dv_ = AXIS == 0 ? d.z : (AXIS == 1 ? d.x : d.y);
+#pragma unroll
+    for (int i = 0; i < n; ++i) {
+        const DAar& r = scene_at<DAar>(S, aar_off + (unsigned)(first + i) * (unsigned)sizeof(DAar));
+        const float4 q0 = r.q0;
+        const float rv = r.q1.x;
+        const float t = (q0.x - oa) * ia;
+        const float u = (ou_ + t * du_) - q0.y;
+        const float v = (ov_ + t * dv_) - q0.w;
+        if (NEAREST) hit_update_nearest(ex, u, q0.z, v, rv, t, tmax, best, __float_as_int(r.q1.y));
+        else hit_update_any(ex, u, q0.z, v, rv, t, tmax, occ_v);
+    }
+}
+template <bool NEAREST>
+KY_DEV void aar_scans_known(SceneRef S, int field, unsigned aar_off, f3 o, f3 d, f3 inv_d, float& tmax, int& best, unsigned& occ_v) {
+    const int n0 = S.count(field), n1 = S.count(field + 1), n2 = S.count(field + 2);
+    aar_scan_known<0, NEAREST>(S, aar_off, 0, n0, o, d, inv_d, tmax, best, occ_v);
+    aar_scan_known<1, NEAREST>(S, aar_off, n0, n1, o, d, inv_d, tmax, best, occ_v);
+    aar_scan_known<2, NEAREST>(S, aar_off, n0 + n1, n2, o, d, inv_d, tmax, best, occ_v);
+}
+KY_DEV int aar_total(SceneRef S, int field) { return S.count(field) + S.count(field + 1) + S.count(field + 2); }
+KY_DEV int trace_nearest_known(SceneRef S, f3 o, f3 d, float& tmax) {
+    int best = -1;
+    const int n_aar = aar_total(S, KY_SH_TRAV), n_sph = S.count(KY_SH_SPH);
+    if (S.boxes()) {
+        const unsigned b_off = opaque_off((unsigned)__builtin_offsetof(DScene, boxtrav));
+        const f3 inv_d = mk3(rcp(d.x), rcp(d.y), rcp(d.z));
+        const f3 inv_c = mk3(__builtin_amdgcn_fmed3f(inv_d.x, -1e30f, 1e30f), __builtin_amdgcn_fmed3f(inv_d.y, -1e30f, 1e30f), __builtin_amdgcn_fmed3f(inv_d.z, -1e30f, 1e30f));
+        const unsigned long long ex = __builtin_amdgcn_ballot_w64(true);
+#pragma unroll
+        for (int k = 0; k < S.count(KY_SH_BOX); ++k) {
+            const DBox& B = scene_at<DBox>(S, b_off + (unsigned)__builtin_offsetof(DBoxTrav, box) + (unsigned)k * (unsigned)sizeof(DBox));
+            box_update_nearest(ex, B.q0, B.q1, B.q2, o, inv_c, tmax, best);
+        }
+        if (aar_total(S, KY_SH_BOX_AAR) > 0) {
+            unsigned unused = 0;
+            aar_scans_known<true>(S, KY_SH_BOX_AAR, b_off + (unsigned)__builtin_offsetof(DBoxTrav, aar), o, d, inv_d, tmax, best, unused);
+        }
+    } else if (n_aar > 0) {
+        const f3 inv_d = mk3(rcp(d.x), rcp(d.y), rcp(d.z));
+        unsigned unused = 0;
+        const unsigned t_off = opaque_off((unsigned)__builtin_offsetof(DScene, trav));
+        aar_scans_known<true>(S, KY_SH_TRAV, t_off + (unsigned)__builtin_offsetof(DTrav, aar), o, d, inv_d, tmax, best, unused);
+    }
+    if (n_sph > 0) {
+        const unsigned off = opaque_off((unsigned)__builtin_offsetof(DScene, sph));
+        const unsigned long long ex = __builtin_amdgcn_ballot_w64(true);
+#pragma unroll
+        for (int i = 0; i < n_sph; ++i) {
+            const float4 c = scene_at<DSph>(S, off + (unsigned)i * (unsigned)sizeof(DSph)).c;
+            const f3 oc = mk3(c.x, c.y, c.z) - o;
+            const float neg_b = dot(oc, d);
+            const float discr = neg_b * neg_b - dot(oc, oc) + c.w;
+            if (!S.sphere_lights() || __any(discr >= 0.f)) sph_update_nearest(ex, neg_b, discr, tmax, best, n_aar + i);
+        }
+    }
+    return best;
+}
+KY_DEV bool trace_any_planar_known(SceneRef S, int field, unsigned t_off, f3 o, f3 d, float tmax) {
+    unsigned occ = 0;
+    if (aar_total(S, field) > 0) {
+        const f3 inv_d = mk3(rcp(d.x), rcp(d.y), rcp(d.z));
+        int unused = -1;
+        aar_scans_known<false>(S, field, t_off + (unsigned)__builtin_offsetof(DTrav, aar), o, d, inv_d, tmax, unused, occ);
+    }
+    return occ != 0;
+}
+KY_DEV bool trace_any_round_known(SceneRef S, bool occ, f3 o, f3 d, float tmax) {
+    const int n_sph = S.count(KY_SH_SPH);
+    if (n_sph > 0) {
+        const unsigned off = opaque_off((unsigned)__builtin_offsetof(DScene, sph));
+        const unsigned long long ex = __builtin_amdgcn_ballot_w64(true);
+        unsigned occ_v = 0;
+#pragma unroll
+        for (int i = 0; i < n_sph; ++i) {
+            const float4 c = scene_at<DSph>(S, off + (unsigned)i * (unsigned)sizeof(DSph)).c;
+            const f3 oc = mk3(c.x, c.y, c.z) - o;
+            const float neg_b = dot(oc, d);
+            const float discr = neg_b * neg_b - dot(oc, oc) + c.w;
+            const float e = neg_b - tmax;
+            if (!S.sphere_lights() || __any((discr >= 0.f) & ((e < 0.f) | (e * e < discr)))) sph_update_any(ex, neg_b, discr, tmax, occ_v);
+        }
+        occ = occ | (occ_v != 0);
+    }
+    return occ;
+}
+
 KY_DEV int trace_nearest(SceneRef S, f3 o, f3 d, float& tmax) {
+    if (S.known()) return trace_nearest_known(S, o, d, tmax);
     int best = -1;
     const unsigned t_off = opaque_off((unsigned)__builtin_offsetof(DScene, trav));
     const int4 head = scene_at<int4>(S, t_off), axis = scene_at<int4>(S, t_off + 16u);
@@ -594,6 +692,7 @@
     return occ != 0;
 }
 KY_DEV bool trace_any_round(SceneRef S, bool occ, f3 o, f3 d, float tmax) {
+    if (S.known()) return trace_any_round_known(S, occ, o, d, tmax);
     const int n_sph = S->n_sph, n_gen = S->n_gen;
     float t;
     if (n_sph > 0) {
@@ -645,7 +744,70 @@
         off += (unsigned)sizeof(DAar);
     }
 }
+template <int AXIS>
+KY_DEV void aar_scan_any_pair_known(SceneRef S, unsigned long long ex, unsigned aar_off, int first, int n, const AnyRay& A, f3 iA, unsigned& occA, const AnyRay& B, f3 iB, unsigned& occB) {
+    if (n <= 0) return;
+    const float oaA = AXIS == 0 ? A.o.x : (AXIS == 1 ? A.o.y : A.o.z), iaA = AXIS == 0 ? iA.x : (AXIS == 1 ? iA.y : iA.z);
+    const float ouA = AXIS == 0 ? A.o.y : (AXIS == 1 ? A.o.z : A.o.x), duA = AXIS == 0 ? A.d.y : (AXIS == 1 ? A.d.z : A.d.x);
+    const float ovA = AXIS == 0 ? A.o.z : (AXIS == 1 ? A.o.x : A.o.y), dvA = AXIS == 0 ? A.d.z : (AXIS == 1 ? A.d.x : A.d.y);
+    const float oaB = AXIS == 0 ? B.o.x : (AXIS == 1 ? B.o.y : B.o.z), iaB = AXIS == 0 ? iB.x : (AXIS == 1 ? iB.y : iB.z);
+    const float ouB = AXIS == 0 ? B.o.y : (AXIS == 1 ? B.o.z : B.o.x), duB = AXIS == 0 ? B.d.y : (AXIS == 1 ? B.d.z : B.d.x);
+    const float ovB = AXIS == 0 ? B.o.z : (AXIS == 1 ? B.o.x : B.o.y), dvB = AXIS == 0 ? B.d.z : (AXIS == 1 ? B.d.x : B.d.y);
+#pragma unroll
+    for (int i = 0; i < n; ++i) {
+        const DAar& r = scene_at<DAar>(S, aar_off + (unsigned)(first + i) * (unsigned)sizeof(DAar));
+        const float4 q0 = r.q0;
+        const float rv = r.q1.x;
+        const float tA = (q0.x - oaA) * iaA, tB = (q0.x - oaB) * iaB;
+        const float uA = (ouA + tA * duA) - q0.y, uB = (ouB + tB * duB) - q0.y;
+        const float vA = (ovA + tA * dvA) - q0.w, vB = (ovB + tB * dvB) - q0.w;
+        hit_update_any_unbounded(ex, uA, q0.z, vA, rv, tA, occA);
+        hit_update_any(ex, uB, q0.z, vB, rv, tB, B.tmax, occB);
+    }
+}
+KY_DEV void aar_scans_any_pair_known(SceneRef S, int field, unsigned long long ex, unsigned aar_off, const AnyRay& A, f3 iA, unsigned& occA, const AnyRay& B, f3 iB, unsigned& occB) {
+    const int n0 = S.count(field), n1 = S.count(field + 1), n2 = S.count(field + 2);
+    aar_scan_any_pair_known<0>(S, ex, aar_off, 0, n0, A, iA, occA, B, iB, occB);
+    aar_scan_any_pair_known<1>(S, ex, aar_off, n0, n1, A, iA, occA, B, iB, occB);
+    aar_scan_any_pair_known<2>(S, ex, aar_off, n0 + n1, n2, A, iA, occA, B, iB, occB);
+}
+KY_DEV void trace_any_pair_known(SceneRef S, const AnyRay& A, const AnyRay& B, bool& occ_a, bool& occ_b) {
+    unsigned occA = 0, occB = 0;
+    const f3 iA = mk3(__builtin_amdgcn_fmed3f(rcp(A.d.x), -1e30f, 1e30f), __builtin_amdgcn_fmed3f(rcp(A.d.y), -1e30f, 1e30f), __builtin_amdgcn_fmed3f(rcp(A.d.z), -1e30f, 1e30f));
+    const f3 iB = mk3(__builtin_amdgcn_fmed3f(rcp(B.d.x), -1e30f, 1e30f), __builtin_amdgcn_fmed3f(rcp(B.d.y), -1e30f, 1e30f), __builtin_amdgcn_fmed3f(rcp(B.d.z), -1e30f, 1e30f));
+    const unsigned long long ex = __builtin_amdgcn_ballot_w64(true);
+    if (S.boxes()) {
+        const unsigned b_off = opaque_off((unsigned)__builtin_offsetof(DScene, boxtrav));
+#pragma unroll
+        for (int k = 0; k < S.count(KY_SH_BOX); ++k) {
+            const DBox& Bx = scene_at<DBox>(S, b_off + (unsigned)__builtin_offsetof(DBoxTrav, box) + (unsigned)k * (unsigned)sizeof(DBox));
+            const float4 q0 = Bx.q0, q1 = Bx.q1, q2 = Bx.q2;
+            box_update_any_unbounded(ex, q0, q1, q2, A.o, iA, occA);
+            box_update_any(ex, q0, q1, q2, B.o, iB, B.tmax, occB);
+        }
+        if (aar_total(S, KY_SH_BOX_AAR) > 0)
+            aar_scans_any_pair_known(S, KY_SH_BOX_AAR, ex, b_off + (unsigned)__builtin_offsetof(DBoxTrav, aar), A, iA, occA, B, iB, occB);
+    } else if (aar_total(S, KY_SH_TRAV) > 0) {
+        const unsigned t_off = opaque_off((unsigned)__builtin_offsetof(DScene, trav));
+        aar_scans_any_pair_known(S, KY_SH_TRAV, ex, t_off + (unsigned)__builtin_offsetof(DTrav, aar), A, iA, occA, B, iB, occB);
+    }
+    const int n_sph = S.count(KY_SH_SPH);
+    if (n_sph > 0) {
+        const unsigned off = opaque_off((unsigned)__builtin_offsetof(DScene, sph));
+#pragma unroll
+        for (int i = 0; i < n_sph; ++i) {
+            const float4 c = scene_at<DSph>(S, off + (unsigned)i * (unsigned)sizeof(DSph)).c;
+            const f3 ocA = mk3(c.x, c.y, c.z) - A.o, ocB = mk3(c.x, c.y, c.z) - B.o;
+            const float nbA = dot(ocA, A.d), nbB = dot(ocB, B.d);
+            sph_update_any_unbounded(ex, nbA, nbA * nbA - dot(ocA, ocA) + c.w, occA);
+            sph_update_any(ex, nbB, nbB * nbB - dot(ocB, ocB) + c.w, B.tmax, occB);
+        }
+    }
+    occ_a = occA != 0;
+    occ_b = occB != 0;
+}
 KY_DEV void trace_any_pair(SceneRef S, const AnyRay& A, const AnyRay& B, bool& occ_a, bool& occ_b) {
+    if (S.known()) { trace_any_pair_known(S, A, B, occ_a, occ_b); return; }
     unsigned occA = 0, occB = 0;
     const f3 iA = mk3(__builtin_amdgcn_fmed3f(rcp(A.d.x), -1e30f, 1e30f), __builtin_amdgcn_fmed3f(rcp(A.d.y), -1e30f, 1e30f), __builtin_amdgcn_fmed3f(rcp(A.d.z), -1e30f, 1e30f));
     const f3 iB = mk3(__builtin_amdgcn_fmed3f(rcp(B.d.x), -1e30f, 1e30f), __builtin_amdgcn_fmed3f(rcp(B.d.y), -1e30f, 1e30f), __builtin_amdgcn_fmed3f(rcp(B.d.z), -1e30f, 1e30f));
@@ -1488,6 +1650,23 @@
 }
 
 KY_DEV bool light_sample_occluded(SceneRef S, int li, f3 o, f3 dir, float tmax) {
+    const int known_tab = S.known() ? shape_table(S.shapes) : 0;
+    if (known_tab != 0) {
+        const unsigned t_off = known_tab == KY_SH_TABLE_FRONT ? (unsigned)__builtin_offsetof(DScene, occ_front)
+                             : (known_tab == KY_SH_TABLE_OCC ? (unsigned)__builtin_offsetof(DScene, occ) : (unsigned)__builtin_offsetof(DScene, trav));
+        const int field = known_tab == KY_SH_TABLE_FRONT ? KY_SH_FRONT : (known_tab == KY_SH_TABLE_OCC ? KY_SH_OCC : KY_SH_TRAV);
+        bool occ = trace_any_round(S, trace_any_planar_known(S, field, opaque_off(t_off), o, dir, tmax), o, dir, tmax);
+        if (S.shapes & KY_SH_TWO_STAGE) {
+            const float4 plane = scene_at<float4>(S, opaque_off((unsigned)__builtin_offsetof(DScene, ts_plane)));
+            const f3 pn = mk3(plane.x, plane.y, plane.z);
+            const f3 e = o + dir * tmax;
+            const bool need = !occ && (fminf(dot(pn, e), dot(pn, o)) <= plane.w);
+            if (__any(need)) {
+                if (need) occ = trace_any_planar_known(S, KY_SH_BEHIND, opaque_off((unsigned)__builtin_offsetof(DScene, occ_behind)), o, dir, tmax);
+            }
+        }
+        return occ;
+    }
     const unsigned tab = (unsigned)scene_light(S, li).shadow_table;
     const bool two = (tab & 1u) != 0;
     bool occ = trace_any(S, scene_at<DTrav>(S, tab & ~1u), o, dir, tmax);
diff --git a/ky_amd/csrc/ky_host.hpp b/ky_amd/csrc/ky_host.hpp
--- a/ky_amd/csrc/ky_host.hpp
+++ b/ky_amd/csrc/ky_host.hpp
@@ -55,6 +55,7 @@
 
 bool specialisation_enabled();
 bool boxes_enabled();
+bool shape_counts_enabled();
 int shadow_queue_mode();
 bool shadow_queue_wanted(const ky_scene* scene);
 int blocks_per_cu_cap();
diff --git a/ky_amd/csrc/ky_launch.hip b/ky_amd/csrc/ky_launch.hip
--- a/ky_amd/csrc/ky_launch.hip
+++ b/ky_amd/csrc/ky_launch.hip
@@ -219,12 +219,18 @@
     int feat, integrator;
     bool large;
     RenderFn fn;
+    unsigned long long shapes;
 };
-#define KY_VARIANT(D, S, Q, G, F, I) Variant{D, S, Q, G, F, I, false, render_kernel<D, S, Q, G, F, I>}
-#define KY_VARIANT_LARGE(D, S, Q, G, F, I) Variant{D, S, Q, G, F, I, true, render_kernel<D, S, Q, G, F, I, true>}
+#define KY_VARIANT(D, S, Q, G, F, I) Variant{D, S, Q, G, F, I, false, render_kernel<D, S, Q, G, F, I>, 0ull}
+#define KY_VARIANT_LARGE(D, S, Q, G, F, I) Variant{D, S, Q, G, F, I, true, render_kernel<D, S, Q, G, F, I, true>, 0ull}
+#define KY_VARIANT_SHAPES(D, S, Q, G, F, I, SH) Variant{D, S, Q, G, F, I, false, render_kernel<D, S, Q, G, F, I, false, SH>, SH}
 constexpr int IT = KY_INTEGRATOR_PATH_TRACING_ITERATION;
+constexpr unsigned long long KY_SH_CORNELL_LAMP = shape_code(2, 0, 0, 0, 4, 3, 3, 2, 2, 2, 1, 0, 0, 1, 2, 2, 0, KY_SH_TABLE_FRONT, true);
+constexpr unsigned long long KY_SH_CORNELL_POINT = shape_code(1, 0, 0, 0, 2, 1, 2, 2, 0, 0, 0, 0, 0, 0, 0, 0, 0, KY_SH_TABLE_OCC, false);
+constexpr unsigned long long KY_SH_CORNELL_DIRECTION = shape_code(1, 0, 0, 0, 2, 1, 2, 2, 0, 0, 0, 0, 0, 0, 0, 0, 0, KY_SH_TABLE_TRAV, false);
 static const Variant g_variants[] = {
 #ifdef KY_FEW_VARIANTS
+    KY_VARIANT_SHAPES(false, KY_DIRECT_BOTH_MIS, false, false, KY_FEAT_CORNELL | KY_FEAT_SMALL_TABLES | KY_FEAT_BOXES | KY_FEAT_AXIS_ALIGNED | KY_FEAT_FLAT_PHONG, IT, KY_SH_CORNELL_LAMP),
     KY_VARIANT(false, KY_DIRECT_BOTH_MIS, false, false, KY_FEAT_CORNELL | KY_FEAT_SMALL_TABLES | KY_FEAT_BOXES | KY_FEAT_AXIS_ALIGNED | KY_FEAT_FLAT_PHONG, IT),
     KY_VARIANT(false, KY_DIRECT_BOTH_MIS, false, false, KY_FEAT_CORNELL | KY_FEAT_SMALL_TABLES | KY_FEAT_BOXES, IT),
     KY_VARIANT(false, KY_DIRECT_BOTH_MIS, false, false, KY_FEAT_CORNELL | KY_FEAT_SMALL_TABLES, IT),
@@ -232,18 +238,23 @@
     KY_VARIANT(false, KY_DIRECT_BOTH_MIS, true, false, KY_FEAT_VEACH | KY_FEAT_FLAT_PHONG | KY_FEAT_X_PLANKS, IT),
 #endif
     KY_VARIANT(false, KY_DIRECT_BOTH_MIS, true, false, KY_FEAT_VEACH | KY_FEAT_FLAT_PHONG, IT),
+    KY_VARIANT_SHAPES(false, KY_DIRECT_BOTH_MIS, false, false, KY_FEAT_SINGLE_ENV | KY_FEAT_SMALL_TABLES | KY_FEAT_BOXES | KY_FEAT_AXIS_ALIGNED | KY_FEAT_FLAT_PHONG, IT, KY_SH_CORNELL_DIRECTION),
     KY_VARIANT(false, KY_DIRECT_BOTH_MIS, false, false, KY_FEAT_SINGLE_ENV | KY_FEAT_SMALL_TABLES | KY_FEAT_BOXES | KY_FEAT_AXIS_ALIGNED | KY_FEAT_FLAT_PHONG, IT),
     KY_VARIANT(false, KY_DIRECT_BOTH_MIS, false, false, KY_FEAT_SINGLE_ENV | KY_FEAT_SMALL_TABLES | KY_FEAT_AXIS_ALIGNED | KY_FEAT_FLAT_PHONG, IT),
     KY_VARIANT(false, KY_DIRECT_BOTH_MIS, false, false, KY_FEAT_SINGLE_ENV, IT),
     KY_VARIANT(false, -1, false, false, 0, IT),
 #else
+    KY_VARIANT_SHAPES(false, KY_DIRECT_BOTH_MIS, false, false, KY_FEAT_CORNELL | KY_FEAT_SMALL_TABLES | KY_FEAT_BOXES | KY_FEAT_AXIS_ALIGNED | KY_FEAT_FLAT_PHONG, IT, KY_SH_CORNELL_LAMP),
     KY_VARIANT(false, KY_DIRECT_BOTH_MIS, false, false, KY_FEAT_CORNELL | KY_FEAT_SMALL_TABLES | KY_FEAT_BOXES | KY_FEAT_AXIS_ALIGNED | KY_FEAT_FLAT_PHONG, IT),
     KY_VARIANT(false, KY_DIRECT_BOTH_MIS, false, false, KY_FEAT_CORNELL | KY_FEAT_SMALL_TABLES | KY_FEAT_BOXES, IT),
     KY_VARIANT(false, KY_DIRECT_BOTH_MIS, false, false, KY_FEAT_CORNELL | KY_FEAT_SMALL_TABLES | KY_FEAT_AXIS_ALIGNED, IT),
     KY_VARIANT(false, KY_DIRECT_BOTH_MIS, false, false, KY_FEAT_CORNELL | KY_FEAT_SMALL_TABLES, IT),
     KY_VARIANT(false, KY_DIRECT_BOTH_MIS, false, false, KY_FEAT_CORNELL, IT),
+    KY_VARIANT_SHAPES(false, KY_DIRECT_BOTH_MIS, false, false, KY_FEAT_SINGLE_DELTA | KY_FEAT_BOXES | KY_FEAT_AXIS_ALIGNED | KY_FEAT_FLAT_PHONG, IT, KY_SH_CORNELL_POINT),
+    KY_VARIANT_SHAPES(false, KY_DIRECT_BOTH_MIS, false, false, KY_FEAT_SINGLE_DELTA | KY_FEAT_BOXES | KY_FEAT_AXIS_ALIGNED | KY_FEAT_FLAT_PHONG, IT, KY_SH_CORNELL_DIRECTION),
     KY_VARIANT(false, KY_DIRECT_BOTH_MIS, false, false, KY_FEAT_SINGLE_DELTA | KY_FEAT_BOXES | KY_FEAT_AXIS_ALIGNED | KY_FEAT_FLAT_PHONG, IT),
     KY_VARIANT(false, KY_DIRECT_BOTH_MIS, false, false, KY_FEAT_SINGLE_DELTA, IT),
+    KY_VARIANT_SHAPES(false, KY_DIRECT_BOTH_MIS, false, false, KY_FEAT_SINGLE_ENV | KY_FEAT_SMALL_TABLES | KY_FEAT_BOXES | KY_FEAT_AXIS_ALIGNED | KY_FEAT_FLAT_PHONG, IT, KY_SH_CORNELL_DIRECTION),
     KY_VARIANT(false, KY_DIRECT_BOTH_MIS, false, false, KY_FEAT_SINGLE_ENV | KY_FEAT_SMALL_TABLES | KY_FEAT_BOXES | KY_FEAT_AXIS_ALIGNED | KY_FEAT_FLAT_PHONG, IT),
     KY_VARIANT(false, KY_DIRECT_BOTH_MIS, false, false, KY_FEAT_SINGLE_ENV | KY_FEAT_SMALL_TABLES | KY_FEAT_AXIS_ALIGNED | KY_FEAT_FLAT_PHONG, IT),
     KY_VARIANT(false, KY_DIRECT_BOTH_MIS, false, false, KY_FEAT_SINGLE_ENV, IT),
@@ -304,6 +315,7 @@
             if (v.strategy != p->direct_sample || v.integrator != p->integrator) continue;
         }
         if ((v.feat & packed->feat) != v.feat) continue;
+        if (v.shapes != 0 && v.shapes != scene_shapes(*packed)) continue;
         if (v.queue && !(n_pix < (1 << 26) && deferred_rays)) continue;
         return &v;
     }
@@ -406,12 +418,13 @@
             if (!((feat & (KY_FEAT_SINGLE_AREA | KY_FEAT_SINGLE_DELTA)) || env_pair)) feat &= ~KY_FEAT_BOXES;
             const bool want_queue = (p->direct_sample == KY_DIRECT_BOTH_MIS || p->direct_sample == KY_DIRECT_LIGHT_MIS || p->direct_sample == KY_DIRECT_LIGHT) &&
                                     p->integrator == KY_INTEGRATOR_PATH_TRACING_ITERATION && sh.n_pix < (1 << 26) && !general && shadow_queue_wanted(scene);
+            const unsigned long long shapes = 0ull;
             const bool same = v->dbg == dbg && v->strategy == p->direct_sample && v->queue == want_queue && v->general == general && v->feat == feat &&
                               v->integrator == p->integrator && v->large == large_scene;
             if (!same) {
                 char expr[192];
-                snprintf(expr, sizeof expr, "%s, %d, %s, %s, %d, %d, %s", dbg ? "true" : "false", p->direct_sample, want_queue ? "true" : "false",
-                         general ? "true" : "false", feat, p->integrator, large_scene ? "true" : "false");
+                snprintf(expr, sizeof expr, "%s, %d, %s, %s, %d, %d, %s, %llu", dbg ? "true" : "false", p->direct_sample, want_queue ? "true" : "false",
+                         general ? "true" : "false", feat, p->integrator, large_scene ? "true" : "false", shapes);
                 DeviceCtx::JitKernel& k = c->jit[expr];
                 if (!k.fn && !k.failed) {
                     bool pending = false;
@@ -513,13 +526,17 @@
     if (!c) return name.c_str();
     std::lock_guard<std::mutex> lock(c->m);
     if (c->last_variant == -2) name = "render_kernel_q (queue engine)";
-    else if (c->last_variant == -3) name = c->last_jit + " (run-time instantiation; template arguments: DEBUG_SAMPLER, STRATEGY, QUEUE, GENERAL, FEAT, INTEGRATOR, LARGE)";
+    else if (c->last_variant == -3) name = c->last_jit + " (run-time instantiation; template arguments: DEBUG_SAMPLER, STRATEGY, QUEUE, GENERAL, FEAT, INTEGRATOR, LARGE, SHAPES)";
     else if (c->last_variant >= 0) {
         const Variant& v = g_variants[c->last_variant];
         char buf[160];
         snprintf(buf, sizeof buf, "render_kernel<%sstrategy %d%s%s%s, feat %d, integrator %d>", v.dbg ? "debug sampler, " : "", v.strategy, v.queue ? ", deferred shadow rays" : "",
                  v.general ? ", general shapes" : "", v.large ? ", scene-sized LDS block" : "", v.feat, v.integrator);
         name = buf;
+        if (v.shapes != 0) {
+            snprintf(buf, sizeof buf, " (shapes 0x%llx)", v.shapes);
+            name += buf;
+        }
     }
     name += c->last_note;
     return name.c_str();
diff --git a/ky_amd/csrc/ky_pack.cpp b/ky_amd/csrc/ky_pack.cpp
--- a/ky_amd/csrc/ky_pack.cpp
+++ b/ky_amd/csrc/ky_pack.cpp
@@ -439,6 +439,39 @@
     return g_boxes != 0;
 }
 
+static int g_shape_counts = -1;
+bool shape_counts_enabled() {
+    if (g_shape_counts < 0) {
+        const char* e = std::getenv("KYHIP_SHAPE_COUNTS");
+        g_shape_counts = (e && std::atoi(e) == 0) ? 0 : 1;
+    }
+    return g_shape_counts != 0;
+}
+
+static unsigned long long scene_shape_code(const DScene& d) {
+    if (!specialisation_enabled() || !shape_counts_enabled() || !(d.feat & KY_FEAT_AXIS_ALIGNED) || d.general || d.n_gen != 0) return 0;
+    const DTrav* tabs[4] = {&d.trav, &d.occ, &d.occ_front, &d.occ_behind};
+    for (const DTrav* t : tabs)
+        if (t->n_par != 0) return 0;
+    int table = 0;
+    bool two = false;
+    if (d.n_lights == 1) {
+        const int32_t tab = d.light[0].shadow_table;
+        const int32_t off = tab & ~1;
+        table = off == (int32_t)__builtin_offsetof(DScene, trav) ? KY_SH_TABLE_TRAV : off == (int32_t)__builtin_offsetof(DScene, occ) ? KY_SH_TABLE_OCC
+              : off == (int32_t)__builtin_offsetof(DScene, occ_front) ? KY_SH_TABLE_FRONT : -1;
+        if (table < 0) return 0;
+        two = (tab & 1) != 0;
+    }
+    const int n[KY_SH_FIELDS] = {d.boxtrav.n_box, d.boxtrav.n_aar_axis[0], d.boxtrav.n_aar_axis[1], d.boxtrav.n_aar_axis[2],
+                                 d.trav.n_aar_axis[0], d.trav.n_aar_axis[1], d.trav.n_aar_axis[2], d.n_sph,
+                                 d.occ.n_aar_axis[0], d.occ.n_aar_axis[1], d.occ.n_aar_axis[2], d.occ_front.n_aar_axis[0], d.occ_front.n_aar_axis[1],
+                                 d.occ_front.n_aar_axis[2], d.occ_behind.n_aar_axis[0], d.occ_behind.n_aar_axis[1], d.occ_behind.n_aar_axis[2]};
+    for (int f = 0; f < KY_SH_FIELDS; ++f)
+        if (n[f] < 0 || n[f] > KY_SH_MAX) return 0;
+    return shape_code(n[0], n[1], n[2], n[3], n[4], n[5], n[6], n[7], n[8], n[9], n[10], n[11], n[12], n[13], n[14], n[15], n[16], table, two);
+}
+
 int pack_scene(const ky_scene* in, DScene* out) {
     if (!in) return fail(KY_ERR_INVALID_VALUE, "scene is NULL");
     if (in->surface_count < 0 || in->shape_count < 0 || in->material_count < 0 || in->light_count < 0)
@@ -662,6 +695,9 @@
             if (in->lights[i].kind == KY_LIGHT_AREA) { any_area = true; own = own && out->light[i].pdf_from_carrier != 0; }
         if (carriers && any_area && own) out->feat |= KY_FEAT_OWN_CARRIER;
     }
+    const unsigned long long code = scene_shape_code(*out);
+    out->shapes[0] = (uint32_t)code;
+    out->shapes[1] = (uint32_t)(code >> 32);
     return KY_OK;
 }
 
@@ -720,7 +756,7 @@
         in->shape_count > KYHIP_MAX_SHAPES || in->material_count > KYHIP_MAX_MATERIALS || in->light_count > KYHIP_MAX_LIGHTS)
         return false;
     auto put = [&](const void* p, size_t n) { const unsigned char* b = (const unsigned char*)p; out.insert(out.end(), b, b + n); };
-    const int32_t head[6] = {in->shape_count, in->material_count, in->light_count, in->surface_count, in->environment_light, (specialisation_enabled() ? 1 : 0) | (boxes_enabled() ? 2 : 0)};
+    const int32_t head[6] = {in->shape_count, in->material_count, in->light_count, in->surface_count, in->environment_light, (specialisation_enabled() ? 1 : 0) | (boxes_enabled() ? 2 : 0) | (shape_counts_enabled() ? 4 : 0)};
     put(head, sizeof head);
     put(&in->camera, sizeof in->camera);
     if (in->shape_count) put(in->shapes, sizeof(ky_shape) * (size_t)in->shape_count);
@@ -830,6 +866,7 @@
 void set_engine_raw(int v) { g_engine = v; }
 void set_specialise_raw(int v) { g_specialise = v; }
 void set_boxes_raw(int v) { g_boxes = v; }
+void set_shape_counts_raw(int v) { g_shape_counts = v; }
 void set_shadow_queue_raw(int v) { g_shadow_queue = v; }
 }
 
@@ -855,6 +892,11 @@
 int kyhip_set_boxes(int on) {
     const int prev = boxes_enabled() ? 1 : 0;
     if (on == 0 || on == 1) kyh::set_boxes_raw(on);
+    return prev;
+}
+int kyhip_set_shape_counts(int on) {
+    const int prev = shape_counts_enabled() ? 1 : 0;
+    if (on == 0 || on == 1) kyh::set_shape_counts_raw(on);
     return prev;
 }
 int kyhip_set_shadow_queue(int mode) {
@@ -913,6 +955,13 @@
     std::vector<DScene> packed(1);
     const int rc = pack_scene(scene, &packed[0]);
     return rc != KY_OK ? rc : packed[0].feat;
+}
+
+int64_t kyhip_scene_shapes(const ky_scene* scene) {
+    if (!scene) return fail(KY_ERR_INVALID_VALUE, "bad arguments");
+    std::vector<DScene> packed(1);
+    const int rc = pack_scene(scene, &packed[0]);
+    return rc != KY_OK ? rc : (int64_t)scene_shapes(packed[0]);
 }
 
 int kyhip_scene_boxes(const ky_scene* scene, int* box_face, int n) {
diff --git a/ky_amd/csrc/ky_render.hpp b/ky_amd/csrc/ky_render.hpp
--- a/ky_amd/csrc/ky_render.hpp
+++ b/ky_amd/csrc/ky_render.hpp
@@ -48,7 +48,7 @@
     int x0, y0, pix0, s_begin, s_end;
 };
 
-template <bool DEBUG_SAMPLER, int STRATEGY, bool QUEUE, bool GENERAL, int FEAT, int INTEGRATOR, bool LARGE>
+template <bool DEBUG_SAMPLER, int STRATEGY, bool QUEUE, bool GENERAL, int FEAT, int INTEGRATOR, bool LARGE, unsigned long long SHAPES = 0>
 constexpr int ky_waves_per_eu() {
     return STRATEGY >= 0 ? (QUEUE ? (FEAT ? KY_WAVES_PER_EU_QUEUE_FEAT : KY_WAVES_PER_EU_QUEUE)
                                   : ((FEAT == 0 && STRATEGY == KY_DIRECT_BOTH_MIS) ? ((GENERAL || INTEGRATOR == KY_INTEGRATOR_PATH_TRACING_RECURSION) ? KY_WAVES_PER_EU_NO_FACTS_GENERAL : KY_WAVES_PER_EU_NO_FACTS)
@@ -56,14 +56,16 @@
                          : KY_WAVES_PER_EU_GENERIC;
 }
 
-template <bool DEBUG_SAMPLER, int STRATEGY, bool QUEUE = false, bool GENERAL = false, int FEAT = 0, int INTEGRATOR = KY_INTEGRATOR_PATH_TRACING_ITERATION, bool LARGE = false>
+template <bool DEBUG_SAMPLER, int STRATEGY, bool QUEUE = false, bool GENERAL = false, int FEAT = 0, int INTEGRATOR = KY_INTEGRATOR_PATH_TRACING_ITERATION, bool LARGE = false,
+          unsigned long long SHAPES = 0>
 KY_DEV void render_kernel_body(const DScene* __restrict__ S_, RenderConst rc, ShardConst sh, unsigned* __restrict__ counter, unsigned long long* __restrict__ accum,
                                unsigned* __restrict__ flags, float4* __restrict__ queue_mem) {
     static_assert(!QUEUE || ((STRATEGY == KY_DIRECT_BOTH_MIS || STRATEGY == KY_DIRECT_LIGHT_MIS || STRATEGY == KY_DIRECT_LIGHT) && INTEGRATOR == KY_INTEGRATOR_PATH_TRACING_ITERATION),
                   "the deferred shadow rays belong to the iterative integrator's strategies with a light-sampling half");
     static_assert(FEAT == 0 || (STRATEGY >= 0 && !GENERAL && !DEBUG_SAMPLER), "scene facts are instantiated for kernels with a fixed strategy only");
     static_assert(STRATEGY >= 0 || INTEGRATOR == KY_INTEGRATOR_PATH_TRACING_ITERATION, "the run-time-dispatched kernel reads the integrator from rc");
-    const SceneRef S{S_, GENERAL, FEAT, LARGE};
+    static_assert(SHAPES == 0 || (FEAT != 0 && !GENERAL), "shape counts are instantiated for kernels with scene facts only");
+    const SceneRef S{S_, GENERAL, FEAT, LARGE, SHAPES};
     __shared__ ItemSlot ring[4][KY_RING];
     __shared__ int c_xy[256], c_pix[256];
     __shared__ unsigned c_se[256];
@@ -233,9 +235,10 @@
     KY_CLK(-2);
 }
 
-template <bool DEBUG_SAMPLER, int STRATEGY, bool QUEUE = false, bool GENERAL = false, int FEAT = 0, int INTEGRATOR = KY_INTEGRATOR_PATH_TRACING_ITERATION, bool LARGE = false>
+template <bool DEBUG_SAMPLER, int STRATEGY, bool QUEUE = false, bool GENERAL = false, int FEAT = 0, int INTEGRATOR = KY_INTEGRATOR_PATH_TRACING_ITERATION, bool LARGE = false,
+          unsigned long long SHAPES = 0>
 __global__ __launch_bounds__(256, (ky_waves_per_eu<DEBUG_SAMPLER, STRATEGY, QUEUE, GENERAL, FEAT, INTEGRATOR, LARGE>())) void render_kernel(
     const DScene* __restrict__ S_, RenderConst rc, ShardConst sh, unsigned* __restrict__ counter, unsigned long long* __restrict__ accum, unsigned* __restrict__ flags,
     float4* __restrict__ queue_mem) {
-    render_kernel_body<DEBUG_SAMPLER, STRATEGY, QUEUE, GENERAL, FEAT, INTEGRATOR, LARGE>(S_, rc, sh, counter, accum, flags, queue_mem);
+    render_kernel_body<DEBUG_SAMPLER, STRATEGY, QUEUE, GENERAL, FEAT, INTEGRATOR, LARGE, SHAPES>(S_, rc, sh, counter, accum, flags, queue_mem);
 }
diff --git a/ky_amd/csrc/ky_scene.hpp b/ky_amd/csrc/ky_scene.hpp
--- a/ky_amd/csrc/ky_scene.hpp
+++ b/ky_amd/csrc/ky_scene.hpp
@@ -123,7 +123,8 @@
     float cam_up[3], pad1;
     DTrav trav;
     DTrav occ;
-    int32_t ts_light, feat, ts_pad[2];
+    int32_t ts_light, feat;
+    uint32_t shapes[2];
     float ts_plane[4];
     DTrav occ_front, occ_behind;
     DBoxTrav boxtrav;
@@ -136,6 +137,7 @@
     DMat mat[KYHIP_MAX_MATERIALS];
     DLight light[KYHIP_MAX_LIGHTS];
 };
+KY_HD inline unsigned long long scene_shapes(const DScene& d) { return ((unsigned long long)d.shapes[1] << 32) | d.shapes[0]; }
 static_assert(__builtin_offsetof(DScene, light) % 16 == 0 && __builtin_offsetof(DScene, trav) % 16 == 0 && __builtin_offsetof(DScene, boxtrav) % 16 == 0 &&
               __builtin_offsetof(DBoxTrav, box) % 16 == 0, "16-byte scalar loads of light, table and box records");
 
@@ -155,6 +157,18 @@
     KY_FEAT_X_PLANKS = 4096,
     KY_FEAT_SMALL_TABLES = 128
 };
+enum : int { KY_SH_BOX = 0, KY_SH_BOX_AAR = 1, KY_SH_TRAV = 4, KY_SH_SPH = 7, KY_SH_OCC = 8, KY_SH_FRONT = 11, KY_SH_BEHIND = 14, KY_SH_FIELDS = 17, KY_SH_MAX = 7 };
+enum : int { KY_SH_TABLE_SHIFT = 3 * KY_SH_FIELDS, KY_SH_TABLE_TRAV = 1, KY_SH_TABLE_OCC = 2, KY_SH_TABLE_FRONT = 3 };
+constexpr unsigned long long KY_SH_TWO_STAGE = 1ull << (KY_SH_TABLE_SHIFT + 2), KY_SH_VALID = 1ull << 60;
+KY_HD constexpr int shape_count(unsigned long long code, int field) { return (int)((code >> (3 * field)) & 7u); }
+KY_HD constexpr int shape_table(unsigned long long code) { return (int)((code >> KY_SH_TABLE_SHIFT) & 3u); }
+KY_HD constexpr unsigned long long shape_code(int box, int bx, int by, int bz, int tx, int ty, int tz, int sph, int ox, int oy, int oz, int fx, int fy, int fz,
+                                              int hx, int hy, int hz, int table, bool two_stage) {
+    unsigned long long c = KY_SH_VALID | ((unsigned long long)table << KY_SH_TABLE_SHIFT) | (two_stage ? KY_SH_TWO_STAGE : 0ull);
+    const int n[KY_SH_FIELDS] = {box, bx, by, bz, tx, ty, tz, sph, ox, oy, oz, fx, fy, fz, hx, hy, hz};
+    for (int f = 0; f < KY_SH_FIELDS; ++f) c |= (unsigned long long)n[f] << (3 * f);
+    return c;
+}
 constexpr int KY_FEAT_SINGLE_LIGHT = KY_FEAT_SINGLE_AREA | KY_FEAT_SINGLE_DELTA | KY_FEAT_SINGLE_ENV;
 
 constexpr int KY_LDS_SURFACES = 64, KY_LDS_MATERIALS = 32;
```

Measured after the change: 22560, median of 6. +1.5%, better.
